# sandialabs/PyNucleus

Measured on AMD Instinct MI355X. Metric: element-pairs/sec assembled (2D P1 fractional s=0.5, dense) + % fp64 roofline, higher is better.
Workload: dtype f64; 1 GPU; 2D unit disc (uniform_disc refined 7x, 98304 cells), P1, 48769 DoFs, fractional s=0.5, horizon=inf, dense getDense incl. zeroExterior; 4831887360 element pairs/step; noRef=7, num_dofs=48769, num_cells=98304, parallelism=block rows of the upper triangle dealt over 1 GPU(s), row-owned one-sided slabs

## Files before the change

include/pnl_hip.h:

```cpp
#ifndef PNL_HIP_H
#define PNL_HIP_H
#include <stdint.h>

#ifdef __cplusplus
extern "C" {
#endif

typedef struct pnl_context pnl_context;

enum pnl_status {
    PNL_OK = 0,
    PNL_ERR_INVALID = -1,
    PNL_ERR_UNSUPPORTED = -2,
    PNL_ERR_HIP = -3,
    PNL_ERR_STATE = -4,
    PNL_ERR_ORDER = -5
};

enum pnl_kernel_type { PNL_FRACTIONAL = 0, PNL_INDICATOR = 1, PNL_PERIDYNAMIC = 2, PNL_GAUSSIAN = 3, PNL_EXPONENTIAL = 4,
                       PNL_GAUSSIAN_BOUNDARY = 5, PNL_EXPONENTIAL_BOUNDARY = 6 };

typedef struct {
    int32_t ktype;
    int32_t interaction;
// ... 85 lines not shown
    const int32_t *d_cell, *d_pair;
    int32_t n_sing[3];
    int32_t n_btouch;
    const int32_t *sing_items[3];
    const int32_t *pair_foff, *fvid;
    const int32_t *bt_slot, *bt_cell, *bt_facet;
} pnl_cluster_plan;
int pnl_assemble_clusters_tiled(pnl_context *ctx, const pnl_cluster_plan *plan, int cluster_boundary, double *data_dev,
                                double *diag_dev);
typedef struct {
    int32_t nnodes, nleaves, nfar, m, nlevels, nq;
    const double *box;
    const int32_t *parent, *level;
    const int32_t *leaf_node, *leaf_dof_off, *leaf_dofs, *leaf_cell_off, *leaf_cells;
    const int32_t *far;
    const double *transfer;
    const double *qbary, *qw, *qphi;
    const int32_t *far_class;
    int32_t partial_leaves;
} pnl_h2_plan;
int pnl_h2_setup(pnl_context *ctx, const pnl_h2_plan *plan);
int pnl_h2_matvec(pnl_context *ctx, const double *x_dev, double *y_dev);
int pnl_h2_upward(pnl_context *ctx, const double *x_dev, double *cup_dev);
int pnl_h2_interact(pnl_context *ctx, const double *cup_dev, double *cdown_dev);
int pnl_h2_downward(pnl_context *ctx, double *cdown_dev, double *y_dev);
int pnl_h2_sizes(pnl_context *ctx, int32_t *out2);
int pnl_h2_get(pnl_context *ctx, int which, double *dst_host);
int pnl_h2_set(pnl_context *ctx, int which, const double *src_host);

int pnl_spmv(pnl_context *ctx, const double *data_dev, const double *diag_dev, const double *x_dev, double *y_dev);

typedef struct pnl_order_function {
    int32_t type, normalized;
    double p[6];
    int32_t scal_n, pad;
    double scal_mid, scal_half;
    double scal_cheb[32];
} pnl_order_function;

int pnl_set_order_function(pnl_context *ctx, const pnl_order_function *f, const double *cell_smax, const double *facet_smax,
                           double c0, double bc0, double sing_fac, double bsing_fac);
int pnl_set_order_vertex_values(pnl_context *ctx, int nv, const double *values_host);
int pnl_upload_pointwise_rules(pnl_context *ctx, int which, int panel, int nkeys, int M, int rows, const double *nodes,
                               const double *w, const double *phi0, const double *phi1);
int pnl_assemble_dense_pointwise(pnl_context *ctx, double *A, int64_t ldA, int zero_exterior, int cell_begin, int cell_end,
                                 int npairs, const int32_t *pairs, int nbpairs, const int32_t *bpairs);
int pnl_assemble_pairs_masked_pointwise(pnl_context *ctx, int np, const int32_t *pairs, const uint64_t *masks, const int32_t *rule,
                                        double *data);
int pnl_assemble_boundary_masked_pointwise(pnl_context *ctx, int ni, const int32_t *cells, const int32_t *facets, const uint32_t *masks,
                                           const int32_t *rule, const double *sv, double fac, double *data, double *diag);

int pnl_get_counters(pnl_context *ctx, int64_t *out, int n);
int pnl_get_phase_ms(pnl_context *ctx, float *out, int n);
enum pnl_kernel_slot { PNL_K_TILE_GENERAL = 0, PNL_K_TILE_UNIFORM2, PNL_K_TILE_UNIFORM3, PNL_K_TILE_UNIFORM4, PNL_K_FOLD_MIRROR,
                       PNL_K_WORKLIST, PNL_NUM_KERNEL_SLOTS };
int pnl_get_kernel_ms(pnl_context *ctx, float *out, int n);

typedef struct pnl_tree pnl_tree;
typedef struct pnl_nfplan pnl_nfplan;
int pnl_tree_build(int N, int dim, const double *boxes, const int64_t *d2c_ptr, const int32_t *d2c_idx, int nc, double eta,
                   int min_size, int max_levels, int do_admissibility, pnl_tree **out);
int pnl_tree_build_blocks(int N, int dim, const double *boxes, const int64_t *d2c_ptr, const int32_t *d2c_idx, int nc, double eta,
                          int min_size, int max_levels, int do_admissibility, const int32_t *dof_block, int mixed_block,
                          pnl_tree **out);
int pnl_tree_build_refined(int N, int dim, const double *boxes, const int64_t *d2c_ptr, const int32_t *d2c_idx, int nc, double eta,
                           int min_size, int max_levels, int do_admissibility, const int32_t *dof_block, int mixed_block, int ref_type,
                           pnl_tree **out);
int pnl_tree_build_horizon(int N, int dim, const double *boxes, const int64_t *d2c_ptr, const int32_t *d2c_idx, int nc, double eta,
                           int min_size, int max_levels, int do_admissibility, const int32_t *dof_block, int mixed_block, int ref_type,
                           double horizon, pnl_tree **out);
int pnl_tree_build_device(int N, int dim, const double *boxes, const int64_t *d2c_ptr, const int32_t *d2c_idx, int nc, double eta,
                          int min_size, int max_levels, int do_admissibility, int ref_type, pnl_tree **out);
void pnl_tree_destroy(pnl_tree *T);
int pnl_tree_sizes(const pnl_tree *T, int64_t *out3);
int pnl_tree_get(const pnl_tree *T, int32_t *range, int32_t *parent, int32_t *children, int32_t *level, double *box, int32_t *perm,
                 int32_t *near, int32_t *far);
int pnl_tree_node_cells(const pnl_tree *T, int n, const int32_t *node_ids, int64_t *off, int32_t *cells);
int pnl_h2_transfer_matrices(int nnodes, int dim, int m, const double *box, const int32_t *parent, double *out);
int pnl_nfplan_build(int dim, int nv, const double *vertices, int nc, const int32_t *cells, int dpe, int N, const int32_t *dofs,
                     int nnodes, const int64_t *node_off, const int32_t *node_dofs, const int64_t *node_cell_off,
                     const int32_t *node_cells, int npairs, const int32_t *pair_nodes, int tile, int max_chunk_dofs,
                     pnl_nfplan **out);
void pnl_nfplan_destroy(pnl_nfplan *P);
int pnl_nfplan_sizes(const pnl_nfplan *P, int64_t *out9);
int pnl_nfplan_get(const pnl_nfplan *P, int which, void *dst);

typedef struct pnl_pattern pnl_pattern;
int pnl_horizon_pattern(int dim, int nv, const double *vertices, int nc, const int32_t *cells, int dpe, int N, const int32_t *dofs,
                        double delta, int strict_lower, pnl_pattern **out);
int pnl_near_pattern(const pnl_tree *T, int npairs, const int32_t *pairs, int strict_lower, pnl_pattern **out);
int64_t pnl_pattern_set_max_nnz(int64_t max_nnz);
int64_t pnl_pattern_nnz(const pnl_pattern *P);
int pnl_pattern_get(const pnl_pattern *P, int32_t *indptr, int32_t *indices);
void pnl_pattern_destroy(pnl_pattern *P);

int pnl_set_row_slab(pnl_context *ctx, int nrows, const int32_t *rowdofs_host, int ncols, const int32_t *coldofs_host);
int pnl_diag_blocks_size(pnl_context *ctx);
int pnl_get_diag_blocks(pnl_context *ctx, double *dst_dev);
int pnl_slab_matvec(pnl_context *ctx, const double *slab_dev, int64_t ld, const double *diag_blocks_dev, const double *x_dev,
                    double *y_dev);
int pnl_slab_diagonal(pnl_context *ctx, const double *slab_dev, int64_t ld, const double *diag_blocks_dev, double *diag_dev);

int pnl_gemv(pnl_context *ctx, const double *A_dev, int64_t ldA, int n, const double *x_dev, double *y_dev,
             int symmetric_half);
int pnl_cg_jacobi(pnl_context *ctx, const double *A_dev, int64_t ldA, int n, const double *b_dev, double *x_dev,
                  double tol, int maxiter, int *iters, double *residual);
// ... 77 lines not shown
```

pynucleus_amd/_lib.py:

```python
import ctypes as C
import os
import numpy as np

_HERE = os.path.dirname(os.path.abspath(__file__))
LIB_PATH = os.environ.get('PNL_LIB', os.path.join(_HERE, 'libpnl_hip.so'))

PNL_OK = 0
PNL_ERR_INVALID = -1
PNL_ERR_UNSUPPORTED = -2
PNL_ERR_HIP = -3
PNL_ERR_STATE = -4
PNL_ERR_ORDER = -5
PNL_INTERIOR = 0
PNL_BOUNDARY = 1
PNL_FLAG_NO_MIRROR = 1
PNL_FLAG_SYMMETRIC_FLUSH = 2
PNL_NUM_COUNTERS = 134

EXPORTS = ['pnl_create', 'pnl_destroy', 'pnl_error_string', 'pnl_version', 'pnl_set_stream', 'pnl_synchronize',
           'pnl_upload_mesh', 'pnl_upload_dofmap', 'pnl_set_kernel', 'pnl_set_order_formula', 'pnl_upload_distant_rules',
           'pnl_upload_singular_rule', 'pnl_upload_boundary', 'pnl_assemble_dense', 'pnl_dense_overwrites', 'pnl_block_row_costs', 'pnl_tile_cells',
           'pnl_assemble_dense_tiles', 'pnl_get_counters', 'pnl_get_phase_ms', 'pnl_get_kernel_ms', 'pnl_tree_build', 'pnl_tree_build_blocks', 'pnl_tree_build_refined', 'pnl_tree_build_horizon', 'pnl_tree_build_device', 'pnl_tree_destroy', 'pnl_tree_sizes', 'pnl_tree_get', 'pnl_tree_node_cells', 'pnl_h2_transfer_matrices', 'pnl_nfplan_build', 'pnl_nfplan_destroy', 'pnl_nfplan_sizes', 'pnl_nfplan_get', 'pnl_horizon_pattern', 'pnl_near_pattern', 'pnl_pattern_set_max_nnz', 'pnl_set_option', 'pnl_set_cell_order', 'pnl_set_interaction_transform', 'pnl_set_order_vertex_values', 'pnl_h2_get', 'pnl_h2_set', 'pnl_pattern_nnz', 'pnl_pattern_get', 'pnl_pattern_destroy', 'pnl_set_row_slab', 'pnl_diag_blocks_size', 'pnl_get_diag_blocks', 'pnl_slab_matvec', 'pnl_slab_diagonal', 'pnl_gemv', 'pnl_cg_jacobi',
           'pnl_inv_diagonal', 'pnl_set_classes', 'pnl_select_class', 'pnl_upload_sparsity', 'pnl_upload_sparsity_device', 'pnl_assemble_pairs_masked', 'pnl_assemble_boundary_masked', 'pnl_assemble_clusters_tiled', 'pnl_h2_setup', 'pnl_h2_matvec', 'pnl_h2_upward', 'pnl_h2_interact', 'pnl_h2_downward', 'pnl_h2_sizes', 'pnl_spmv',
           'pnl_assemble_pairs_in_horizon', 'pnl_assemble_pairs_in_horizon_range', 'pnl_set_nonsymmetric', 'pnl_set_order_function', 'pnl_upload_pointwise_rules', 'pnl_assemble_dense_pointwise',
           'pnl_assemble_pairs_masked_pointwise', 'pnl_assemble_boundary_masked_pointwise',
           'pnl_gemv_axpby', 'pnl_csr_matvec', 'pnl_mg_create', 'pnl_mg_destroy', 'pnl_mg_cycle', 'pnl_mg_solve', 'pnl_mg_cg', 'pnl_theta_step', 'pnl_selftest',
           'pnl_potrf', 'pnl_potrs', 'pnl_getrf', 'pnl_getrs',
           'pnl_csr_cg_jacobi', 'pnl_fe_space_create', 'pnl_fe_space_destroy', 'pnl_assemble_nonlinearity', 'pnl_imex_create',
           'pnl_imex_destroy', 'pnl_imex_sweep']

PNL_FUN_BRUSSELATOR, PNL_FUN_CUBIC = 0, 1
PNL_IMEX_CG_MG, PNL_IMEX_CHOL = 0, 1
PNL_IMEX_MAX_STAGES, PNL_IMEX_MAX_COMP = 4, 2


def source_sha16():
    import glob
    import hashlib
    root = os.path.dirname(_HERE)
    files = sorted(glob.glob(os.path.join(_HERE, 'csrc', '*.h'))+glob.glob(os.path.join(_HERE, 'csrc', '*.hip'))
                   +[os.path.join(root, 'include', 'pnl_hip.h'), os.path.join(_HERE, 'csrc', 'Makefile')])
    h = hashlib.sha256()
    for fn in files:
        with open(fn, 'rb') as f:
            h.update(os.path.basename(fn).encode()+b'\0'+f.read())
    return h.hexdigest()[:16]


class pnl_kernel(C.Structure):
    _fields_ = [('ktype', C.c_int32), ('interaction', C.c_int32), ('exponent', C.c_double), ('scale', C.c_double),
                ('horizon2', C.c_double)]


class pnl_order_formula(C.Structure):
    _fields_ = [('c0', C.c_double), ('a', C.c_double), ('b', C.c_double), ('e', C.c_double), ('den0', C.c_double),
                ('clip_num', C.c_int32), ('pad', C.c_int32)]


class pnl_mg_level_desc(C.Structure):
    _fields_ = [('n', C.c_int32), ('pad', C.c_int32), ('A_dev', C.c_void_p), ('ldA', C.c_int64), ('diag_dev', C.c_void_p),
                ('R_indptr_dev', C.c_void_p), ('R_indices_dev', C.c_void_p), ('R_data_dev', C.c_void_p),
                ('P_indptr_dev', C.c_void_p), ('P_indices_dev', C.c_void_p), ('P_data_dev', C.c_void_p),
                ('kind', C.c_int32), ('pad2', C.c_int32), ('near_indptr_dev', C.c_void_p), ('near_indices_dev', C.c_void_p),
                ('near_data_dev', C.c_void_p)]


class pnl_order_function(C.Structure):
    _fields_ = [('type', C.c_int32), ('normalized', C.c_int32), ('p', C.c_double*6), ('scal_n', C.c_int32), ('pad', C.c_int32),
                ('scal_mid', C.c_double), ('scal_half', C.c_double), ('scal_cheb', C.c_double*32)]


class pnl_cluster_plan(C.Structure):
    _fields_ = ([(n, C.c_int32) for n in ('npairs', 'nnodes', 'nchunks', 'chunk_stride', 'ntiles', 'num_dslots', 'nfacets', 'tile')] +
                [(n, C.c_void_p) for n in ('pair_nodes', 'node_off', 'node_dofs', 'chunk_cells', 'chunk_ndof', 'chunk_dofs', 'chunk_slot',
                                           'tile_chunkA', 'tile_chunkB', 'tile_pair', 'tile_flags', 'tile_dslotA', 'tile_dslotB',
# ... 11 lines not shown

class pnl_imex_desc(C.Structure):
    _fields_ = ([(n, C.c_int32) for n in ('s', 'ncomp', 'n', 'fun', 'nparams', 'solver', 'maxiter', 'mass_maxiter')] +
                [('AE', C.c_double*(PNL_IMEX_MAX_STAGES**2)), ('AI', C.c_double*(PNL_IMEX_MAX_STAGES**2)),
                 ('bE', C.c_double*PNL_IMEX_MAX_STAGES), ('bI', C.c_double*PNL_IMEX_MAX_STAGES),
                 ('mass_scale', C.c_double*PNL_IMEX_MAX_COMP), ('params', C.c_double*4),
                 ('dt', C.c_double), ('tol', C.c_double), ('mass_tol', C.c_double),
                 ('S_dev', C.c_void_p), ('ldS', C.c_int64), ('M_indptr_dev', C.c_void_p), ('M_indices_dev', C.c_void_p),
                 ('M_data_dev', C.c_void_p), ('space', C.c_void_p), ('mg', C.c_void_p*PNL_IMEX_MAX_COMP),
                 ('chol_dev', C.c_void_p*PNL_IMEX_MAX_COMP), ('ldchol', C.c_int64*PNL_IMEX_MAX_COMP)])


class PnlError(RuntimeError):
    pass


_LIB = None


def load():
    global _LIB
    if _LIB is not None:
        return _LIB
    if not os.path.exists(LIB_PATH):
        raise PnlError('{} is missing: the HIP extension has not been built (run __graft_entry__.build()); '
                       'there is no CPU fallback for the assembly path'.format(LIB_PATH))
    import torch
    L = C.CDLL(LIB_PATH)
    vp, i32, i64, dbl = C.c_void_p, C.c_int, C.c_int64, C.c_double
    L.pnl_create.argtypes = [i32, C.POINTER(vp)]
    L.pnl_destroy.argtypes = [vp]
    L.pnl_destroy.restype = None
    L.pnl_error_string.argtypes = [vp]
    L.pnl_error_string.restype = C.c_char_p
    L.pnl_version.restype = C.c_char_p
    L.pnl_set_stream.argtypes = [vp, vp]
    L.pnl_synchronize.argtypes = [vp]
    L.pnl_upload_mesh.argtypes = [vp, i32, i32, vp, i32, vp, vp, vp, dbl]
    L.pnl_upload_dofmap.argtypes = [vp, i32, i32, i32, i32, vp, vp]
    L.pnl_set_kernel.argtypes = [vp, i32, C.POINTER(pnl_kernel)]
    L.pnl_selftest.argtypes = [i32, i32, i32, i32, vp, i32, vp, vp]
    L.pnl_set_order_formula.argtypes = [vp, i32, C.POINTER(pnl_order_formula)]
    L.pnl_upload_distant_rules.argtypes = [vp, i32, vp, vp, vp, vp, vp, vp, vp]
    L.pnl_upload_singular_rule.argtypes = [vp, i32, i32, i32, i32, vp, vp, vp, dbl]
    L.pnl_upload_boundary.argtypes = [vp, i32, vp]
    L.pnl_assemble_dense.argtypes = [vp, vp, i64, i32, i32, i32, i32]
    L.pnl_dense_overwrites.argtypes = [vp, i32, i32, i32]
    L.pnl_block_row_costs.argtypes = [vp, vp, i32]
    L.pnl_tile_cells.argtypes = [vp]
    L.pnl_assemble_dense_tiles.argtypes = [vp, vp, i64, i32, i32, vp, i32, i32, i32]
    L.pnl_get_counters.argtypes = [vp, vp, i32]
    L.pnl_get_phase_ms.argtypes = [vp, vp, i32]
    L.pnl_get_kernel_ms.argtypes = [vp, vp, i32]
    L.pnl_set_row_slab.argtypes = [vp, i32, vp, i32, vp]
    L.pnl_tree_build.argtypes = [i32, i32, vp, vp, vp, i32, dbl, i32, i32, i32, C.POINTER(vp)]
    L.pnl_tree_build_blocks.argtypes = [i32, i32, vp, vp, vp, i32, dbl, i32, i32, i32, vp, i32, C.POINTER(vp)]
    L.pnl_tree_build_refined.argtypes = [i32, i32, vp, vp, vp, i32, dbl, i32, i32, i32, vp, i32, i32, C.POINTER(vp)]
    L.pnl_tree_build_horizon.argtypes = [i32, i32, vp, vp, vp, i32, dbl, i32, i32, i32, vp, i32, i32, dbl, C.POINTER(vp)]
    L.pnl_tree_build_device.argtypes = [i32, i32, vp, vp, vp, i32, dbl, i32, i32, i32, i32, C.POINTER(vp)]
    L.pnl_tree_destroy.argtypes = [vp]
    L.pnl_tree_destroy.restype = None
    L.pnl_tree_sizes.argtypes = [vp, vp]
    L.pnl_tree_get.argtypes = [vp, vp, vp, vp, vp, vp, vp, vp, vp]
    L.pnl_tree_node_cells.argtypes = [vp, i32, vp, vp, vp]
    L.pnl_h2_transfer_matrices.argtypes = [i32, i32, i32, vp, vp, vp]
    L.pnl_nfplan_build.argtypes = [i32, i32, vp, i32, vp, i32, i32, vp, i32, vp, vp, vp, vp, i32, vp, i32, i32, C.POINTER(vp)]
    L.pnl_nfplan_destroy.argtypes = [vp]
    L.pnl_nfplan_destroy.restype = None
    L.pnl_nfplan_sizes.argtypes = [vp, vp]
    L.pnl_nfplan_get.argtypes = [vp, i32, vp]
    L.pnl_horizon_pattern.argtypes = [i32, i32, vp, i32, vp, i32, i32, vp, dbl, i32, C.POINTER(vp)]
    L.pnl_near_pattern.argtypes = [vp, i32, vp, i32, C.POINTER(vp)]
    L.pnl_pattern_nnz.argtypes = [vp]
    L.pnl_pattern_set_max_nnz.argtypes = [i64]
    L.pnl_set_option.argtypes = [C.c_char_p, C.c_char_p]
    L.pnl_set_cell_order.argtypes = [vp, i32, vp]
    L.pnl_set_interaction_transform.argtypes = [vp, i32, vp]
    L.pnl_set_order_vertex_values.argtypes = [vp, i32, vp]
    L.pnl_h2_get.argtypes = [vp, i32, vp]
    L.pnl_h2_set.argtypes = [vp, i32, vp]
    L.pnl_pattern_get.argtypes = [vp, vp, vp]
    L.pnl_pattern_destroy.argtypes = [vp]
    L.pnl_diag_blocks_size.argtypes = [vp]
    L.pnl_get_diag_blocks.argtypes = [vp, vp]
    L.pnl_slab_matvec.argtypes = [vp, vp, i64, vp, vp, vp]
    L.pnl_slab_diagonal.argtypes = [vp, vp, i64, vp, vp]
    L.pnl_gemv.argtypes = [vp, vp, i64, i32, vp, vp, i32]
    L.pnl_cg_jacobi.argtypes = [vp, vp, i64, i32, vp, vp, dbl, i32, C.POINTER(C.c_int), C.POINTER(C.c_double)]
    L.pnl_inv_diagonal.argtypes = [vp, vp, i64, i32, vp]
    L.pnl_gemv_axpby.argtypes = [vp, vp, i64, i32, i32, vp, dbl, dbl, vp, vp]
    L.pnl_csr_matvec.argtypes = [vp, i32, vp, vp, vp, vp, dbl, dbl, vp]
    L.pnl_mg_create.argtypes = [vp, i32, C.POINTER(pnl_mg_level_desc), vp, dbl, i32, i32, C.POINTER(C.c_void_p)]
    L.pnl_mg_destroy.argtypes = [vp]
    L.pnl_mg_cycle.argtypes = [vp, vp, vp, i32]
    L.pnl_mg_solve.argtypes = [vp, vp, vp, dbl, i32, i32, C.POINTER(C.c_int), C.POINTER(C.c_double), i32]
    L.pnl_mg_cg.argtypes = [vp, vp, i64, vp, vp, dbl, i32, i32, C.POINTER(C.c_int), C.POINTER(C.c_double), i32]
    L.pnl_theta_step.argtypes = [vp, vp, i64, vp, vp, vp, dbl, dbl, vp, vp, dbl, i32, C.POINTER(C.c_int), C.POINTER(C.c_double)]
    L.pnl_potrf.argtypes = [vp, vp, i64, i32, C.POINTER(C.c_int)]
    L.pnl_potrs.argtypes = [vp, vp, i64, i32, vp, i64, i32]
    L.pnl_getrf.argtypes = [vp, vp, i64, i32, vp, C.POINTER(C.c_int)]
    L.pnl_getrs.argtypes = [vp, vp, i64, i32, vp, vp, i64, i32]
    L.pnl_csr_cg_jacobi.argtypes = [vp, i32, vp, vp, vp, dbl, vp, vp, dbl, i32, i32, C.POINTER(C.c_int), C.POINTER(C.c_double)]
    L.pnl_fe_space_create.argtypes = [vp, i32, i32, i32, i32, vp, vp, vp, vp, C.POINTER(vp)]
    L.pnl_fe_space_destroy.argtypes = [vp]
    L.pnl_assemble_nonlinearity.argtypes = [vp, i32, vp, i32, i32, vp, i64, i32, dbl, dbl, vp, i64]
    L.pnl_imex_create.argtypes = [vp, C.POINTER(pnl_imex_desc), C.POINTER(vp)]
# ... 307 lines not shown
        P.chunk_slot = ptr(plan.chunk_slot, np.int16)
        for s in range(3):
            P.n_sing[s] = plan.sing_items[s].shape[0]
            P.sing_items[s] = ptr(plan.sing_items[s], np.int32)
        P.n_btouch = plan.bt_cell.shape[0]
        self.check(self.L.pnl_assemble_clusters_tiled(self.h, C.byref(P), int(bool(cluster_boundary)), C.c_void_p(data_ptr),
                                                      C.c_void_p(diag_ptr) if diag_ptr else None))

    def spmv(self, data_ptr, diag_ptr, x_ptr, y_ptr):
        self.check(self.L.pnl_spmv(self.h, C.c_void_p(data_ptr), C.c_void_p(diag_ptr) if diag_ptr else None, C.c_void_p(x_ptr),
                                   C.c_void_p(y_ptr)))

    def counters(self):
        out = np.zeros(PNL_NUM_COUNTERS, dtype=np.int64)
        self.check(self.L.pnl_get_counters(self.h, out.ctypes.data, PNL_NUM_COUNTERS))
        hist = {q: int(out[8+q]) for q in range(120) if out[8+q]}
        sing = {-1-k: int(out[128+k]) for k in range(3)}
        return dict(numCellPairs=int(out[0]), numAssembledCellPairs=int(out[1]), numIntegrations=int(out[2]),
                    numBoundaryPairs=int(out[3]), numBoundaryIntegrations=int(out[4]), orders=hist, singular=sing,
                    uniformTilePairs=int(out[6]), uniformTilePairsByOrder={2+k: int(out[131+k]) for k in range(3)})

    def phase_ms(self):
        out = np.zeros(7, dtype=np.float32)
        self.check(self.L.pnl_get_phase_ms(self.h, out.ctypes.data, 7))
        return dict(tiles=float(out[0]), tiles_uniform=float(out[6]), worklist=float(out[1]), singular=float(out[2]),
                    boundary=float(out[3]), scatter_mirror=float(out[4]), total=float(out[5]))

    def set_row_slab(self, rowdofs, coldofs):
        rd = np.ascontiguousarray(rowdofs, dtype=np.int32)
        cd = np.ascontiguousarray(coldofs, dtype=np.int32)
        self.check(self.L.pnl_set_row_slab(self.h, int(rd.shape[0]), rd.ctypes.data if rd.shape[0] else None, int(cd.shape[0]),
                                           cd.ctypes.data if cd.shape[0] else None))

    def diag_blocks_size(self):
        n = self.L.pnl_diag_blocks_size(self.h)
        self.check(min(n, 0))
        return n

    def get_diag_blocks(self, dst_ptr):
        self.check(self.L.pnl_get_diag_blocks(self.h, C.c_void_p(dst_ptr)))

    def slab_matvec(self, slab_ptr, ld, dblocks_ptr, x_ptr, y_ptr):
        self.check(self.L.pnl_slab_matvec(self.h, C.c_void_p(slab_ptr), int(ld), C.c_void_p(dblocks_ptr), C.c_void_p(x_ptr), C.c_void_p(y_ptr)))

    def slab_diagonal(self, slab_ptr, ld, dblocks_ptr, diag_ptr):
        self.check(self.L.pnl_slab_diagonal(self.h, C.c_void_p(slab_ptr), int(ld), C.c_void_p(dblocks_ptr), C.c_void_p(diag_ptr)))

    def kernel_ms(self):
        out = np.zeros(6, dtype=np.float32)
        self.check(self.L.pnl_get_kernel_ms(self.h, out.ctypes.data, 6))
        return dict(tile_general=float(out[0]), tile_uniform2=float(out[1]), tile_uniform3=float(out[2]), tile_uniform4=float(out[3]),
                    fold_mirror=float(out[4]), worklist=float(out[5]))

    def gemv(self, A_ptr, ldA, n, x_ptr, y_ptr, symmetric_half=False):
        self.check(self.L.pnl_gemv(self.h, C.c_void_p(A_ptr), int(ldA), int(n), C.c_void_p(x_ptr), C.c_void_p(y_ptr),
                                   int(symmetric_half)))

    def cg_jacobi(self, A_ptr, ldA, n, b_ptr, x_ptr, tol, maxiter):
        it, res = C.c_int(0), C.c_double(0.)
        self.check(self.L.pnl_cg_jacobi(self.h, C.c_void_p(A_ptr), int(ldA), int(n), C.c_void_p(b_ptr), C.c_void_p(x_ptr),
                                        float(tol), int(maxiter), C.byref(it), C.byref(res)))
        return it.value, res.value

    def gemv_axpby(self, A_ptr, ldA, nrows, ncols, x_ptr, alpha, beta, b_ptr, y_ptr):
        self.check(self.L.pnl_gemv_axpby(self.h, C.c_void_p(A_ptr), int(ldA), int(nrows), int(ncols), C.c_void_p(x_ptr), float(alpha),
                                         float(beta), C.c_void_p(b_ptr) if b_ptr else None, C.c_void_p(y_ptr)))

    def csr_matvec(self, nrows, indptr_ptr, indices_ptr, data_ptr, x_ptr, alpha, beta, y_ptr):
        self.check(self.L.pnl_csr_matvec(self.h, int(nrows), C.c_void_p(indptr_ptr), C.c_void_p(indices_ptr), C.c_void_p(data_ptr),
                                         C.c_void_p(x_ptr), float(alpha), float(beta), C.c_void_p(y_ptr)))

    def mg_create(self, descs, coarse_inverse_ptr, omega, presmooth, postsmooth):
        arr = (pnl_mg_level_desc*len(descs))(*descs)
        out = C.c_void_p()
        self.check(self.L.pnl_mg_create(self.h, len(descs), arr, C.c_void_p(coarse_inverse_ptr), float(omega), int(presmooth), int(postsmooth),
                                        C.byref(out)))
        return out

    def mg_destroy(self, mg):
        self.L.pnl_mg_destroy(mg)

    def mg_cycle(self, mg, b_ptr, x_ptr, x_is_zero):
        self.check(self.L.pnl_mg_cycle(mg, C.c_void_p(b_ptr), C.c_void_p(x_ptr), int(bool(x_is_zero))))

    def mg_solve(self, mg, b_ptr, x_ptr, tol, maxiter, x_is_zero):
        it = C.c_int(0)
        res = (C.c_double*(maxiter+2))()
        self.check(self.L.pnl_mg_solve(mg, C.c_void_p(b_ptr), C.c_void_p(x_ptr), float(tol), int(maxiter), int(bool(x_is_zero)), C.byref(it),
                                       res, maxiter+2))
        return it.value, list(res[:it.value+1])

    def mg_cg(self, mg, A_ptr, ldA, b_ptr, x_ptr, tol, maxiter, x_is_zero):
        it = C.c_int(0)
        res = (C.c_double*(maxiter+2))(*([float('nan')]*(maxiter+2)))
        self.check(self.L.pnl_mg_cg(mg, C.c_void_p(A_ptr) if A_ptr else None, int(ldA), C.c_void_p(b_ptr), C.c_void_p(x_ptr), float(tol),
                                    int(maxiter), int(bool(x_is_zero)), C.byref(it), res, maxiter+2))
        out = list(res)
        while len(out) > 1 and out[-1] != out[-1]:
            out.pop()
        return it.value, out

    def theta_step(self, mg, S_ptr, ldS, M_indptr_ptr, M_indices_ptr, M_data_ptr, dt, theta, forcing_ptr, u_ptr, tol, maxiter):
        it, res = C.c_int(0), C.c_double(0.)
        self.check(self.L.pnl_theta_step(mg, C.c_void_p(S_ptr), int(ldS), C.c_void_p(M_indptr_ptr), C.c_void_p(M_indices_ptr),
                                         C.c_void_p(M_data_ptr), float(dt), float(theta), C.c_void_p(forcing_ptr) if forcing_ptr else None,
                                         C.c_void_p(u_ptr), float(tol), int(maxiter), C.byref(it), C.byref(res)))
# ... 69 lines not shown
```

pynucleus_amd/csrc/pnl_context.h:

```cpp
#pragma once
#include <hip/hip_runtime.h>
#include <algorithm>
#include <cmath>
#include <cstdarg>
#include <cstdio>
#include <cstring>
#include <string>
#include <vector>
#include "pnl_hip.h"
#include "pnl_device.h"

constexpr int TILE_P1 = 64;
constexpr int TILE_P2 = 32;

struct DevBuf {
    void *p = nullptr;
    size_t bytes = 0;
    ~DevBuf() { release(); }
    void release() { if (p) { (void)hipFree(p); p = nullptr; bytes = 0; } }
};

struct pnl_context {
    int device = 0;
    hipStream_t own_stream = nullptr, stream = nullptr;
    static constexpr int NAUX = 4;
    hipStream_t aux[NAUX] = {};
    hipEvent_t ev_fork = nullptr, ev_join[NAUX] = {};
    hipEvent_t ev_fold = nullptr;
    hipEvent_t ev_bnd = nullptr;
    bool fold_event_set = false;
    std::string err;
    int dim = 0, nv = 0, nc = 0, dpe = 0, dpv = 0, dped = 0, N = 0, nb = 0, qmax = -1;
    int nreal = 0;
    std::vector<int> cell_orig;
    std::vector<int> real_from;
    double H0 = 0.;
    std::vector<double> vertices, vol, h;
    std::vector<int32_t> cells, dofs, perm_table, bcells;
    struct ClassData {
        pnl_kernel kern[2];
        pnl_order_formula form[2];
        bool have_kernel[2] = {false, false}, have_form[2] = {false, false};
        bool have_sing[2][3] = {{false, false, false}, {false, false, false}};
        DevBuf b_sn[3], b_sw[3], b_sp[3], b_bn[2], b_bw[2], b_bp[2], b_spairs[3], b_bpairs[2], b_spairs1[3];
        int sM[3] = {0, 0, 0}, sRows[3] = {0, 0, 0}, bM[2] = {0, 0};
        double sFac = 0., bFac = 0.;
        int n_spairs[3] = {0, 0, 0}, n_bpairs[2] = {0, 0};
        int n_spairs1[3] = {0, 0, 0};
        ClassData() { std::memset(kern, 0, sizeof(kern)); std::memset(form, 0, sizeof(form)); }
    };
    std::vector<ClassData*> cls;
    int cur = 0;
    ClassData &C() { return *cls[cur]; }
    int nlab = 0;
    bool nonsym = false;
    int orient = 0;
    std::vector<int32_t> cell_labels, facet_labels, cls_of;
    bool have_mesh = false, have_dofs = false, have_rules = false, have_boundary = false;
    bool dirty = true;
    DevProblem P;
    DevBuf b_cellv, b_ccen, b_cvol, b_ch, b_clog, b_cvid, b_cdof, b_cslot, b_blk_ndof, b_blk_dofs, b_perm, b_off, b_bary, b_w, b_phi,
        b_foff, b_fbary, b_fw, b_bvid, b_bv, b_bgeo, b_counters, b_D, b_tiles,
        b_vec[6], b_clabel, b_blabel, b_clsof, b_scal, b_wl, b_wlcount, b_tilectr, b_ttn, b_ttoff, b_tttab, b_ttwphi, b_wlsorted, b_wlaux,
        b_vertices, b_sp_indptr, b_sp_indices, b_mp_pairs, b_mp_masks, b_mp_wl, b_mp_sorted, b_mp_aux, b_bi_cells, b_bi_facets,
        b_bi_masks, b_cp[28], b_cpD, b_wlds, b_wlpair, b_h2[20];
    DevBuf b_kcls, b_fcls, b_uni, b_tilecls, b_ttwphif;
    DevBuf b_scolbase, b_srowoff, b_cpoff, b_cpslot, b_cprow, b_foldtab, b_bkcls, b_bfcls, b_bdefer, b_multitiles, b_slotA, b_candtiles, b_candq;
    int slot_S = 0, n_multitiles = 0;
    long long slot_total = 0;
    DevBuf b_rowmap, b_rowdof, b_colmap, b_coldof;
    DevBuf b_cholinfo;
    DevBuf b_luwork, b_lutmp;
    std::vector<int32_t> slab_rowdofs, slab_coldofs;
    int slab_rows = 0, slab_cols = 0;
    bool slot_full_list = false;
    bool slot_used = false;
    std::vector<DevKernel> kcls_host;
    std::vector<DevKernel> bkcls_host;
    std::vector<DevFormula> bfcls_host;
    std::vector<DevFormula> fcls_host;
    int uni_off[5] = {-1, -1, -1, -1, -1}, uni_np[5] = {0, 0, 0, 0, 0};
    bool uni_struct[5] = {false, false, false, false, false};
    H2Dev h2;
    bool have_h2 = false;
    bool have_tile_order = false;
    struct TileOrderJob *tile_job = nullptr;
    DevBuf b_cellv_t, b_cdof_t, b_cslot_t, b_Dt;
    PwDev pw;
    bool have_pw = false, have_pw_rules[2][3] = {{false, false, false}, {false, false, false}};
    int pw_nkeys[2] = {0, 0};
    std::vector<double> pw_cell_smax, pw_facet_smax;
    std::vector<double> pw_vertex_s;
    DevBuf b_pw_cellsv;
    DevBuf b_pw_csm, b_pw_fsm, b_pw_rule[2][3][4], b_pw_pairs, b_pw_bpairs;
    std::vector<std::vector<int>> h2_levels;
    long long h2_vtot = 0;
    std::vector<size_t> h2_level_off;
    std::vector<int32_t> rule_off, frule_off;
    int sp_nnz = -1;
    unsigned wl_cap = 0;
    int tile = TILE_P1, nblocks = 0, ncp = 0, nU = 0;
    std::vector<int2> spairs_host[3];
    std::vector<int2> tiles_cached;
    size_t tiles_cap = 0;
    int n_mixed = 0, n_pure = 0, tile_off = 0, tiles_cb = -1, tiles_ce = -1;
    std::vector<int> cls_tile_off, cls_n_mixed, cls_n_pure;
    std::vector<int> cls_n_uni[3];
    bool single_launch = false;
    int sl_off[4] = {0, 0, 0, 0}, sl_n[4] = {0, 0, 0, 0};
    unsigned wl_cap_each = 0;
    int wl_slots = 1;
    std::vector<pnl_order_formula> tiles_forms;
    pnl_order_formula tiles_form;
    bool tiles_filter = true;
    bool use_pure = true;
    struct PowTab { double exponent, scale; DevBuf buf; };
    std::vector<PowTab*> powtabs;
    struct BlockAgg { double cx, cy, rad, hmax, hmin, Lmin, Lmax; bool full; double tcx, tcy, trad; };
    bool have_xform = false;
    double xform[4] = {1., 0., 0., 1.};
    std::vector<BlockAgg> blocks;
    hipEvent_t ev[8] = {nullptr, nullptr, nullptr, nullptr, nullptr, nullptr, nullptr, nullptr};
    hipEvent_t kev[PNL_NUM_KERNEL_SLOTS][2] = {};
    bool kev_set[PNL_NUM_KERNEL_SLOTS] = {};
    bool pure_launched = false;
    bool symflush = false;
    bool ev_valid = false;
    unsigned long long visited_pairs = 0;
    bool visited_is_assembled = false;
    bool tiles_launched = false;
    int ablate = 0;
    bool tile_cell_filter = true;
    bool wl_lane = true;
};

inline int fail(pnl_context *ctx, int code, const char *fmt, ...) {
    char buf[512];
    va_list ap;
    va_start(ap, fmt);
    vsnprintf(buf, sizeof(buf), fmt, ap);
    va_end(ap);
    if (ctx) ctx->err = buf;
    return code;
}

#define HIPCHK(ctx, call)                                                                            \
    do {                                                                                             \
        hipError_t e_ = (call);                                                                      \
        if (e_ != hipSuccess) return fail(ctx, PNL_ERR_HIP, "%s failed: %s", #call, hipGetErrorString(e_)); \
    } while (0)

template <class T>
int upload(pnl_context *ctx, DevBuf &b, const T *src, size_t n) {
    const size_t bytes = std::max<size_t>(n*sizeof(T), 16);
    if (b.bytes < bytes) {
        b.release();
        HIPCHK(ctx, hipMalloc(&b.p, bytes));
        b.bytes = bytes;
    }
    if (n) HIPCHK(ctx, hipMemcpyAsync(b.p, src, n*sizeof(T), hipMemcpyHostToDevice, ctx->stream));
    HIPCHK(ctx, hipStreamSynchronize(ctx->stream));
    return PNL_OK;
}

inline int ensure(pnl_context *ctx, DevBuf &b, size_t bytes) {
    bytes = std::max<size_t>(bytes, 16);
    if (b.bytes < bytes) {
        b.release();
        HIPCHK(ctx, hipMalloc(&b.p, bytes));
        b.bytes = bytes;
    }
    return PNL_OK;
}

inline DevKernel to_dev(const pnl_kernel &k, int dim) {
    DevKernel d;
    d.ktype = k.ktype;
// ... 31 lines not shown
    W.type = f.type; W.normalized = f.normalized;
    for (int i = 0; i < 6; i++) W.p[i] = f.p[i];
    if (f.scal_n < 0 || f.scal_n > 32 || (f.scal_n > 0 && !(f.scal_half > 0.))) return false;
    W.scal_n = f.scal_n; W.scal_mid = f.scal_mid; W.scal_inv_half = f.scal_n > 0 ? 1./f.scal_half : 0.;
    for (int i = 0; i < 32; i++) W.scal_cheb[i] = i < f.scal_n ? f.scal_cheb[i] : 0.;
    return true;
}

inline DevFormula to_dev(const pnl_order_formula &f) {
    DevFormula d;
    d.c0 = f.c0; d.a = f.a; d.b = f.b; d.e = f.e; d.den0 = f.den0; d.clip = f.clip_num; d.pad = 0;
    return d;
}

const char *pnl_tune(const char *name);
inline int pnl_grid_cap(int grid) {
    const char *e = pnl_tune("PNL_TILE_WGS");
    const int cap = e ? atoi(e) : 0;
    return cap > 0 ? std::max(1, std::min(grid, cap)) : grid;
}

inline int acc_stride_of(int nU, size_t fixed_bytes = 0) {
    int st = nU+1;
    const int m = pnl_tune("PNL_ACC_PAD") ? atoi(pnl_tune("PNL_ACC_PAD")) : 32;
    if (m > 1) {
        int padded = st;
        while (padded % m != 1) padded++;
        if (fixed_bytes+sizeof(double)*(size_t)(nU+1)*padded <= 80*1024) st = padded;
        else if (st % 2 == 0 && fixed_bytes+sizeof(double)*(size_t)(nU+1)*(st+1) <= 80*1024) st++;
    }
    return st;
}

inline DevProblem tile_problem(const pnl_context *ctx) {
    DevProblem Pt = ctx->P;
    if (ctx->have_tile_order) {
        Pt.cellv = (const double*)ctx->b_cellv_t.p; Pt.cdof = (const int*)ctx->b_cdof_t.p; Pt.cslot = (const short*)ctx->b_cslot_t.p;
    }
    return Pt;
}

inline DevProblem with_mixed_rules(const pnl_context *ctx, DevProblem Pt) {
    Pt.uni = (const double*)ctx->b_uni.p;
    Pt.mix_struct = 0;
    const bool generic = pnl_tune("PNL_MIXED_GENERIC") != nullptr;
    for (int q = 0; q < 5; q++) {
        Pt.uni_off[q] = ctx->uni_off[q] >= 0 ? ctx->uni_off[q] : 0;
        if (q >= 2 && q <= ctx->qmax && ctx->dim == 2 && ctx->dpe == 3 && ctx->uni_off[q] >= 0 && ctx->uni_struct[q] && !generic)
            Pt.mix_struct |= 1 << q;
    }
    return Pt;
}

inline void kt_begin(pnl_context *ctx, int slot) { (void)hipEventRecord(ctx->kev[slot][0], ctx->stream); }
inline void kt_end(pnl_context *ctx, int slot) { (void)hipEventRecord(ctx->kev[slot][1], ctx->stream); ctx->kev_set[slot] = true; }

int pnl_tile_order_ready(pnl_context *ctx);

int pnl_assembly_prepare(pnl_context *ctx);
int pnl_assembly_ready(pnl_context *ctx);
void pnl_refresh_tables(pnl_context *ctx);
int pnl_make_tiles(pnl_context *ctx, std::vector<int2> &tiles, int cell_begin, int cell_end);
int pnl_upload_tiles(pnl_context *ctx, std::vector<int2> &tiles, int cell_begin, int cell_end);
int pnl_tile_order_range(pnl_context *ctx, const DevFormula &qo, int ncand, signed char *host_out);
struct WlBins { unsigned *hist, *offs, *coff, *cursor; };
int pnl_wl_sort(pnl_context *ctx, const int4 *wl, const unsigned *count, unsigned cap, unsigned *aux_base, int4 *sorted, WlBins &B);
void pnl_scatter_diag(pnl_context *ctx, const DevProblem &P, const double *D, double *A, int64_t ldA);
int pnl_tile_uniform_order(const pnl_context *ctx, const pnl_order_formula &F, int ta, int tb, int qlimit);
int pnl_sparse_ready(pnl_context *ctx, double *data, double *diag, SparseOut &S);

int pnl_pw_prepare(pnl_context *ctx, int need_boundary);
int pnl_pw_h2_interp(pnl_context *ctx);

int pnl_launch_gemv_symmetric(pnl_context *ctx, const double *A, long long ldA, int n, const double *x, double alpha, double beta,
                              const double *b, double *y);
int pnl_launch_slab_two_sided(pnl_context *ctx, const double *slab, long long ld, int nrows, int ncols, const int *rowdof, const int *coldof,
                              const double *x, double *y);

int pnl2_launch_uniform(pnl_context *ctx, int kt, const DevProblem &Pt, const int2 *tiles, const int *tile_cls, int ntiles, int q,
                        double *A, int64_t ldA, double *Dglob, const SlotOut &SO);
int pnl2_launch_p2(pnl_context *ctx, int kt, const int2 *tiles, const int *tile_cls, int ntiles, double *A, int64_t ldA,
                   int cell_begin, int cell_end, unsigned wl_cap_each, const SlotOut &SO);
int pnl2_zero_slot_tiles(pnl_context *ctx, const SlotOut &SO);
int pnl2_fold_mirror(pnl_context *ctx, const SlotOut &SO, double *A, int64_t ldA);
inline SlotOut slot_out(const pnl_context *ctx) {
    SlotOut SO;
    SO.A2 = (double*)ctx->b_slotA.p; SO.rowoff = (const long long*)ctx->b_srowoff.p; SO.colbase = (const int*)ctx->b_scolbase.p;
    SO.S = ctx->slot_S; SO.nU = ctx->nU;
    return SO;
}
```

pynucleus_amd/csrc/pnl_hip.hip:

```cpp
#include <hip/hip_runtime.h>
#include <algorithm>
#include <cmath>
#include <cstdio>
#include <cstring>
#include <string>
#include <vector>
#include "pnl_hip.h"
#include "pnl_kernels.h"
#include "pnl_bndtile.h"
#include "pnl_context.h"
#include "pnl_launch.h"

namespace {

__global__ void __launch_bounds__(PNL_NTHREADS)
k_mirror(double *__restrict__ A, long long ldA, int N) {
    __shared__ double t1[32][33], t2[32][33];
    const int nb = (N+31)/32;
    int bid = blockIdx.x;
    int bi = 0;
    {
        double fb = ((2.*nb+1.)-sqrt((2.*nb+1.)*(2.*nb+1.)-8.*bid))*0.5;
        bi = (int)fb;
        while (bi > 0 && (long long)bi*nb-(long long)bi*(bi-1)/2 > bid) bi--;
// ... 75 lines not shown
        }
    }
    void use(int k) {
        if (!on) return;
        const int j = k < (int)slot.size() ? slot[k] : k % pnl_context::NAUX;
        if (!used[j]) { (void)hipStreamWaitEvent(ctx->aux[j], start, 0); used[j] = true; }
        ctx->stream = ctx->aux[j];
    }
    void join() {
        if (!on) return;
        ctx->stream = main;
        for (int j = 0; j < pnl_context::NAUX; j++)
            if (used[j]) {
                (void)hipEventRecord(ctx->ev_join[j], ctx->aux[j]);
                (void)hipStreamWaitEvent(main, ctx->ev_join[j], 0);
                used[j] = false;
            }
        on = false;
    }
    ~ClassFork() { join(); }
};

template <int DIM, int DPE, int KT>
int run_worklist(pnl_context *ctx, const int4 *wl, const unsigned *wlc, unsigned cap, double *A, int64_t ldA, bool sym, int region = 0,
                 int nregions = 1) {
    int rc;
    if ((rc = ensure(ctx, ctx->b_wlsorted, (size_t)cap*nregions*sizeof(int4)))) return rc;
    if ((rc = ensure(ctx, ctx->b_wlaux, sizeof(unsigned)*(4*(PNL_WL_BINS+1))*nregions))) return rc;
    const int4 *wlsorted = (const int4*)ctx->b_wlsorted.p+(size_t)region*cap;
    WlBins B;
    if ((rc = pnl_wl_sort(ctx, wl, wlc, cap, (unsigned*)ctx->b_wlaux.p+(size_t)region*4*(PNL_WL_BINS+1), (int4*)wlsorted, B))) return rc;
    int dbg = 0;
#ifdef PNL_DEBUG_ABLATE
    dbg = pnl_tune("PNL_WL_DBG") ? atoi(pnl_tune("PNL_WL_DBG")) : 0;
#endif
    const int nmin = ctx->wl_lane ? PNL_WL_LANE_MAXPTS+1 : 0;
    return worklist_eval<DIM, DPE, KT, false>(ctx, "PNL_WL_LDS_KB", 18, wlsorted, B, A, ldA, (double*)ctx->b_D.p, SparseOut{}, ClusterTiles{},
                                              PNL_WL_BINS-1, nmin | (sym ? 1 << 16 : 0), ctx->wl_lane, dbg | (sym ? 8 : 0));
}

int ensure_worklist(pnl_context *ctx, double pairs, int regions) {
    const double frac = pnl_tune("PNL_WL_FRAC") ? atof(pnl_tune("PNL_WL_FRAC")) : 0.05;
    const double floor_entries = pnl_tune("PNL_WL_FRAC") ? 64. : (double)(1 << 20);
    const size_t each = (size_t)std::min<double>(std::max<double>(pairs*frac, floor_entries), 400e6);
    int rc;
    if ((rc = ensure(ctx, ctx->b_wl, each*(size_t)regions*sizeof(int4)))) return rc;
    ctx->wl_cap = (unsigned)std::min<size_t>(ctx->b_wl.bytes/sizeof(int4), 0xffffffffu);
    ctx->wl_cap_each = (unsigned)each;
    if ((rc = ensure(ctx, ctx->b_tilectr, sizeof(unsigned)))) return rc;
    return PNL_OK;
}

template <int DIM, int DPE, int TILE, int KT>
int launch_tiles(pnl_context *ctx, int wl_slot, double *A, int64_t ldA, int cell_begin, int cell_end, const SlotOut &SO = SlotOut{}) {
    using S = TileSmem<DIM, DPE, TILE, KT == 0>;
    HIPCHK(ctx, hipEventRecord(ctx->ev[7], ctx->stream));
    ctx->pure_launched = false;
    if (TILE == 64 && DPE <= 3) {
        int rc;
        if (DIM == 2 && DPE == 3 && !pnl_tune("PNL_PURE_V1") && ctx->uni_off[2] >= 0 && ctx->uni_np[2] == 3)
            rc = pnl2_launch_uniform(ctx, KT, tile_problem(ctx), (const int2*)ctx->b_tiles.p+ctx->tile_off+ctx->n_mixed, nullptr, ctx->n_pure, 2,
                                     A, ldA, (double*)(ctx->have_tile_order ? ctx->b_Dt.p : ctx->b_D.p), SO);
        else rc = launch_pure<DIM, (DPE <= 3 ? DPE : 3), KT>(ctx, A, ldA, SO);
        if (rc) return rc;
        ctx->pure_launched = ctx->n_pure > 0;
        if (DIM == 2 && DPE == 3) {
            int off = ctx->tile_off+ctx->n_mixed+ctx->n_pure;
            for (int q = 3; q <= 4; q++) {
                const int n = ctx->cls_n_uni[q-2][ctx->cur];
                if ((rc = pnl2_launch_uniform(ctx, KT, tile_problem(ctx), (const int2*)ctx->b_tiles.p+off, nullptr, n, q, A, ldA,
                                              (double*)(ctx->have_tile_order ? ctx->b_Dt.p : ctx->b_D.p), SO))) return rc;
                ctx->pure_launched = ctx->pure_launched || n > 0;
                off += n;
            }
        }
        HIPCHK(ctx, hipEventRecord(ctx->ev[7], ctx->stream));
    }
    const int ntiles = ctx->n_mixed;
    const int acc_stride = acc_stride_of(ctx->nU, S::fixed_bytes);
    const size_t lds = S::fixed_bytes+sizeof(double)*(size_t)(ctx->nU+1)*acc_stride;
    if (lds > 160*1024)
        return fail(ctx, PNL_ERR_UNSUPPORTED, "a block of %d cells touches %d DoFs: LDS sub-block of %zu bytes exceeds 160 KiB "
                    "(cells must be numbered with spatial locality)", TILE, ctx->nU, lds);
    unsigned *wlc = (unsigned*)ctx->b_wlcount.p+wl_slot;
    HIPCHK(ctx, hipMemsetAsync(ctx->b_tilectr.p, 0, sizeof(unsigned), ctx->stream));
    auto kfun = k_tile_distant<DIM, DPE, TILE, KT, false>;
    const int grid_mult = pnl_tune("PNL_GRID_MULT") ? atoi(pnl_tune("PNL_GRID_MULT")) : 1;
    const PersistentGrid g = persistent_grid(ctx, kfun, tile_threads(DPE, KT), lds, ntiles, 2, grid_mult);
    if (g.rc) return g.rc;
    if (pnl_tune("PNL_VERBOSE")) fprintf(stderr, "[pnl] tiles=%d nU=%d lds=%zu bytes, occupancy API: %d blocks/CU\n", ntiles, ctx->nU, lds, g.per_cu);
    SlotOut SOk = SO;
    SOk.nU = ctx->nU;
    kt_begin(ctx, PNL_K_TILE_GENERAL);
    if (g.grid > 0)
        hipLaunchKernelGGL(kfun, dim3(g.grid), dim3(tile_threads(DPE, KT)), lds, ctx->stream, with_mixed_rules(ctx, tile_problem(ctx)), (const int2*)ctx->b_tiles.p+ctx->tile_off, A,
                           (long long)ldA, (double*)(ctx->have_tile_order ? ctx->b_Dt.p : ctx->b_D.p), cell_begin, cell_end, acc_stride, (int4*)ctx->b_wl.p,
                           wlc, ctx->wl_cap_each, ctx->ablate | (ctx->symflush ? 256 : 0), ntiles, ClusterTiles{},
                           (unsigned*)ctx->b_tilectr.p, SOk);
    kt_end(ctx, PNL_K_TILE_GENERAL);
    HIPCHK(ctx, hipGetLastError());
    HIPCHK(ctx, hipEventRecord(ctx->ev[6], ctx->stream));
    if (SO.A2) {
        int rc = pnl2_fold_mirror(ctx, SO, A, ldA);
        if (rc) return rc;
        HIPCHK(ctx, hipEventRecord(ctx->ev_fold, ctx->stream));
        ctx->fold_event_set = true;
    }
    return run_worklist<DIM, DPE, KT>(ctx, (const int4*)ctx->b_wl.p, wlc, ctx->wl_cap_each, A, ldA, ctx->symflush || SO.A2 != nullptr);
}

template <int DIM, int DPE, int KT>
int launch_singular(pnl_context *ctx, double *A, int64_t ldA, int cell_begin, int cell_end) {
    for (int s = 0; s < DIM+1; s++) {
        const int np = ctx->orient ? ctx->C().n_spairs1[s] : ctx->C().n_spairs[s];
        if (!np) continue;
        if (!ctx->C().have_sing[0][s]) return fail(ctx, PNL_ERR_STATE, "singular rule for %d common vertices not uploaded", s+1);
        const int wpb = PNL_SING_THREADS/64;
        int rc = with_slot<DIM>(s, [&](auto slot) {
            constexpr int SLOT = decltype(slot)::value;
            const int2 *pairs = (const int2*)(ctx->orient ? ctx->C().b_spairs1[SLOT].p : ctx->C().b_spairs[SLOT].p);
            return launch_singular_pairs<DIM, DPE, SLOT, KT, false>(ctx, (np+wpb-1)/wpb, pairs, np, A, ldA, cell_begin, cell_end, SparseOut{},
                                                                    nullptr, nullptr, ClusterTiles{});
        });
        if (rc) return rc;
    }
    return PNL_OK;
}

template <int DIM, int DPE, int KT>
int launch_boundary(pnl_context *ctx, int cell_begin, int cell_end, int what = 3, const DevKernel *bkcls = nullptr,
                    const DevFormula *bfcls = nullptr, bool all_fast = false) {
    if (ctx->nb == 0 || cell_end <= cell_begin) return PNL_OK;
    const int ncell = cell_end-cell_begin;
    const int gx = (ncell+PNL_NTHREADS-1)/PNL_NTHREADS;
    int per = pnl_tune("PNL_BND_PER") ? atoi(pnl_tune("PNL_BND_PER")) : 32;
    while (per > 1 && (long long)gx*((ctx->nb+per-1)/per) < 4096) per >>= 1;
    const int chunks = (ctx->nb+per-1)/per;
    if (what & 1) {
        const int defer = pnl_tune("PNL_BND_DEFER") ? atoi(pnl_tune("PNL_BND_DEFER")) : 48;
        const bool use_list = defer > 0;
        const unsigned cap = (unsigned)std::min<long long>(std::max<long long>(65536, 64ll*ctx->nb), 1ll << 24);
        int *dcells = nullptr, *dfacets = nullptr, *dcls = nullptr;
        unsigned *dslots = nullptr, *dcount = nullptr;
        if (use_list) {
            int rc;
            if ((rc = ensure(ctx, ctx->b_bdefer, sizeof(int)*(size_t)cap*(3+DIM)+sizeof(unsigned)))) return rc;
            dcells = (int*)ctx->b_bdefer.p; dfacets = dcells+cap; dslots = (unsigned*)(dfacets+(size_t)cap*DIM); dcls = (int*)(dslots+cap);
            dcount = (unsigned*)(dcls+cap);
            HIPCHK(ctx, hipMemsetAsync(dcount, 0, sizeof(unsigned), ctx->stream));
        }
        const bool fast = bkcls ? all_fast : (ctx->P.bkn.fast != 0);
        bool tiled = false;
        if constexpr (DIM == 2) {
// ... 95 lines not shown
        if (var && (rc = pnl2_zero_slot_tiles(ctx, SO))) return rc;
    }
    HIPCHK(ctx, hipEventRecord(ctx->ev[7], ctx->stream));
    ctx->pure_launched = false;
    for (int q = 2; q <= 4; q++) {
        const int n = ctx->sl_n[q-1];
        if ((rc = pnl2_launch_uniform(ctx, kt, ctx->P, tiles+ctx->sl_off[q-1], tcls ? tcls+ctx->sl_off[q-1] : nullptr, n, q, A, ldA,
                                      (double*)ctx->b_D.p, SO))) return rc;
        ctx->pure_launched = ctx->pure_launched || n > 0;
    }
    if (ctx->pure_launched) HIPCHK(ctx, hipEventRecord(ctx->ev[7], ctx->stream));
    if ((rc = pnl2_launch_p2(ctx, kt, tiles+ctx->sl_off[0], tcls ? tcls+ctx->sl_off[0] : nullptr, ctx->sl_n[0], A, ldA, cell_begin, cell_end,
                             ctx->wl_cap_each, SO))) return rc;
    HIPCHK(ctx, hipEventRecord(ctx->ev[6], ctx->stream));
    if (ctx->slot_used) {
        if ((rc = pnl2_fold_mirror(ctx, SO, A, ldA))) return rc;
        HIPCHK(ctx, hipEventRecord(ctx->ev_fold, ctx->stream));
        ctx->fold_event_set = true;
    }
    const bool sym = ctx->symflush || ctx->slot_used;
    {
        ClassFork fork(ctx, ncls);
        if (ncls > pnl_context::NAUX && (int)ctx->cls_n_mixed.size() == ncls) fork.plan(ctx->cls_n_mixed);
        for (int k = 0; k < ncls; k++) {
            ctx->cur = k;
            pnl_refresh_tables(ctx);
            fork.use(k);
            const int4 *wl = (const int4*)ctx->b_wl.p+(size_t)k*ctx->wl_cap_each;
            const unsigned *wlc = (const unsigned*)ctx->b_wlcount.p+k;
            rc = with_kt(ctx->P.k.fast, [&](auto kt) {
                return run_worklist<DIM, DPE, decltype(kt)::value>(ctx, wl, wlc, ctx->wl_cap_each, A, ldA, sym, k, ncls);
            });
            if (rc) { ctx->cur = 0; return rc; }
        }
    }
    ctx->cur = 0;
    return PNL_OK;
}

bool slot_eligible(const pnl_context *ctx, int cell_begin, int cell_end, int flags) {
    const bool elem = ctx->dpe == 6 || (ctx->dpe == 3 && ctx->cls.size() == 1 && !ctx->nonsym && ctx->use_pure && !pnl_tune("PNL_NO_SLOT_P1"));
    return ctx->dim == 2 && elem && ctx->slot_full_list && ctx->slab_rows == 0 && cell_begin == 0 && cell_end == ctx->nc &&
           !(flags & (PNL_FLAG_NO_MIRROR | PNL_FLAG_SYMMETRIC_FLUSH));
}

#ifndef PNL_BND_MODE_DEFAULT
#define PNL_BND_MODE_DEFAULT 3
#endif
template <int DIM, int DPE, int TILE>
int assemble_impl(pnl_context *ctx, double *A, int64_t ldA, int zero_exterior, int ntiles, int cell_begin, int cell_end, int flags) {
    int rc;
    const int ncls = (int)ctx->cls.size();
    ctx->symflush = (flags & PNL_FLAG_SYMMETRIC_FLUSH) != 0;
    for (bool &b : ctx->kev_set) b = false;
    HIPCHK(ctx, hipMemsetAsync(ctx->b_counters.p, 0, sizeof(unsigned long long)*PNL_NCOUNTERS, ctx->stream));
    HIPCHK(ctx, hipMemsetAsync(ctx->b_D.p, 0, sizeof(double)*(size_t)ctx->ncp*(DPE*(DPE+1)/2), ctx->stream));
    if (ctx->have_tile_order) HIPCHK(ctx, hipMemsetAsync(ctx->b_Dt.p, 0, sizeof(double)*(size_t)ctx->ncp*(DPE*(DPE+1)/2), ctx->stream));
    HIPCHK(ctx, hipEventRecord(ctx->ev[0], ctx->stream));
    ctx->tiles_launched = ntiles > 0;
    ctx->fold_event_set = false;
    const bool bnd_one_pass = zero_exterior && ncls > 1 && ctx->nlab > 0 && !pnl_tune("PNL_BND_PER_CLASS");
    bool bnd_all_fast = true;
    if (bnd_one_pass) {
        std::vector<DevKernel> &bk = ctx->bkcls_host;
        std::vector<DevFormula> &bf = ctx->bfcls_host;
        bk.resize(ncls); bf.resize(ncls);
        for (int k = 0; k < ncls; k++) {
            ctx->cur = k;
            pnl_refresh_tables(ctx);
            bk[k] = ctx->P.bkn; bf[k] = ctx->P.bqo;
            bnd_all_fast = bnd_all_fast && ctx->P.bkn.fast;
        }
        ctx->cur = 0;
        if ((rc = ensure(ctx, ctx->b_bkcls, sizeof(DevKernel)*ncls))) return rc;
        if ((rc = ensure(ctx, ctx->b_bfcls, sizeof(DevFormula)*ncls))) return rc;
        HIPCHK(ctx, hipMemcpyAsync(ctx->b_bkcls.p, bk.data(), sizeof(DevKernel)*ncls, hipMemcpyHostToDevice, ctx->stream));
        HIPCHK(ctx, hipMemcpyAsync(ctx->b_bfcls.p, bf.data(), sizeof(DevFormula)*ncls, hipMemcpyHostToDevice, ctx->stream));
    }
    auto boundary_term = [&](hipEvent_t chain) -> int {
        int rcb;
        ClassFork fork(ctx, chain ? ncls : 1, chain);
        if (chain && ncls > pnl_context::NAUX && (int)ctx->cls_n_mixed.size() == ncls) fork.plan(ctx->cls_n_mixed);
        for (int k = 0; k < ncls; k++) {
            ctx->cur = k;
            pnl_refresh_tables(ctx);
            if (!ctx->have_boundary || !ctx->C().have_kernel[1] || !ctx->C().have_form[1]) {
                ctx->cur = 0;
                return fail(ctx, PNL_ERR_STATE, "zero_exterior needs boundary facets, boundary kernel and order formula");
            }
            if (chain) fork.use(k);
            if (bnd_one_pass && k == 0 &&
                (rcb = launch_boundary<DIM, DPE, 0>(ctx, cell_begin, cell_end, 1, (const DevKernel*)ctx->b_bkcls.p, (const DevFormula*)ctx->b_bfcls.p,
                                                    bnd_all_fast))) { ctx->cur = 0; return rcb; }
            if (chain) fork.use(k);
            if ((rcb = launch_boundary<DIM, DPE, 0>(ctx, cell_begin, cell_end, bnd_one_pass ? 2 : 3))) { ctx->cur = 0; return rcb; }
        }
        ctx->cur = 0;
        return PNL_OK;
    };
    const int bnd_mode = !zero_exterior ? -1 : pnl_tune("PNL_BND_MODE") ? atoi(pnl_tune("PNL_BND_MODE")) : PNL_BND_MODE_DEFAULT;
    bool bnd_side = false;
    auto boundary_side = [&](hipEvent_t after) -> int {
        hipStream_t const caller = ctx->stream;
        hipStream_t const side = ctx->aux[1];
        HIPCHK(ctx, hipStreamWaitEvent(side, after, 0));
        ctx->stream = side;
        const int rcb = boundary_term(nullptr);
        ctx->stream = caller;
        if (rcb) return rcb;
        HIPCHK(ctx, hipEventRecord(ctx->ev_join[1], side));
        bnd_side = true;
        return PNL_OK;
    };
// ... 16 lines not shown
                { ctx->cur = 0; ctx->orient = 0; return rc; }
        } else {
        SlotOut SO{};
        ctx->slot_used = false;
        if (slot_eligible(ctx, cell_begin, cell_end, flags) && slot_storage_ready(ctx)) { SO = slot_out(ctx); ctx->slot_used = true; }
        for (int ko = 0; ko < ncls*norient; ko++) {
            const int k = ko/norient;
            ctx->cur = k; ctx->orient = ko%norient;
            pnl_refresh_tables(ctx);
            ctx->tile_off = ctx->cls_tile_off[k]; ctx->n_mixed = ctx->cls_n_mixed[k]; ctx->n_pure = ctx->cls_n_pure[k];
            if (ctx->n_mixed+ctx->n_pure+ctx->cls_n_uni[1][k]+ctx->cls_n_uni[2][k] == 0) continue;
            const int tb0 = ctx->tile_cell_filter ? cell_begin : 0, tb1 = ctx->tile_cell_filter ? cell_end : ctx->nc;
            if (ctx->P.k.fast && ctx->P.k.qm == 6 && DPE == 3 && !pnl_tune("PNL_NO_KT2")) rc = launch_tiles<DIM, DPE, TILE, (DPE == 3 ? 2 : 1)>(ctx, ko, A, ldA, tb0, tb1, SO);
            else rc = with_kt(ctx->P.k.fast, [&](auto kt) { return launch_tiles<DIM, DPE, TILE, decltype(kt)::value>(ctx, ko, A, ldA, tb0, tb1, SO); });
            if (rc) { ctx->cur = 0; ctx->orient = 0; return rc; }
        }
        }
    }
    ctx->orient = 0;
    HIPCHK(ctx, hipEventRecord(ctx->ev[1], ctx->stream));
    if (ntiles > 0 && ctx->slot_used) {
    } else if (!(flags & (PNL_FLAG_NO_MIRROR | PNL_FLAG_SYMMETRIC_FLUSH))) {
        const long long nb = (ctx->N+31)/32;
        hipLaunchKernelGGL(k_mirror, dim3((unsigned)(nb*(nb+1)/2)), dim3(PNL_NTHREADS), 0, ctx->stream, A, (long long)ldA, ctx->N);
        HIPCHK(ctx, hipGetLastError());
    }
    HIPCHK(ctx, hipEventRecord(ctx->ev[2], ctx->stream));
    hipStream_t const main_stream = ctx->stream;
    bool fold_like = ctx->fold_event_set;
    if (!fold_like && ncls*norient == 1 && zero_exterior && !pnl_tune("PNL_NO_OVERLAP")) {
        HIPCHK(ctx, hipEventRecord(ctx->ev_fold, ctx->stream));
        fold_like = true;
    }
    const bool overlap = fold_like && ncls*norient == 1 && !pnl_tune("PNL_NO_OVERLAP");
    struct StreamGuard { pnl_context *c; hipStream_t s; ~StreamGuard() { c->stream = s; } } stream_guard{ctx, main_stream};
    if (overlap) { HIPCHK(ctx, hipStreamWaitEvent(ctx->aux[0], ctx->ev_fold, 0)); ctx->stream = ctx->aux[0]; }
    hipEvent_t const chain = (ctx->fold_event_set && !overlap && !pnl_tune("PNL_NO_OVERLAP")) ? ctx->ev_fold : nullptr;
    {
        ClassFork fork(ctx, ncls*norient, chain);
        if (norient == 1 && ncls > pnl_context::NAUX && (int)ctx->cls_n_mixed.size() == ncls) fork.plan(ctx->cls_n_mixed);
        for (int ko = 0; ko < ncls*norient; ko++) {
            ctx->cur = ko/norient; ctx->orient = ko%norient;
            pnl_refresh_tables(ctx);
            fork.use(ko);
            rc = with_kt(ctx->P.k.fast, [&](auto kt) { return launch_singular<DIM, DPE, decltype(kt)::value>(ctx, A, ldA, cell_begin, cell_end); });
            if (rc) { ctx->cur = 0; ctx->orient = 0; return rc; }
        }
    }
    ctx->orient = 0;
    if (overlap) {
        HIPCHK(ctx, hipEventRecord(ctx->ev_join[0], ctx->aux[0]));
        ctx->stream = main_stream;
    } else HIPCHK(ctx, hipEventRecord(ctx->ev[3], ctx->stream));
    if (bnd_mode == 3 && ctx->fold_event_set) rc = boundary_side(ctx->ev[6]);
    else if (bnd_mode == 1 || ((bnd_mode == 0 || bnd_mode == 3) && overlap)) rc = boundary_side(bnd_mode == 1 ? ctx->ev_bnd : ctx->ev_fold);
    else if (bnd_mode == 0 || bnd_mode == 3) rc = boundary_term(chain);
    if (rc) return rc;
    ctx->cur = 0;
    if (overlap) {
        HIPCHK(ctx, hipStreamWaitEvent(main_stream, ctx->ev_join[0], 0));
        ctx->stream = main_stream;
        HIPCHK(ctx, hipEventRecord(ctx->ev[3], ctx->stream));
    }
    if (bnd_side) HIPCHK(ctx, hipStreamWaitEvent(main_stream, ctx->ev_join[1], 0));
    HIPCHK(ctx, hipEventRecord(ctx->ev[4], ctx->stream));
    if (ctx->slab_rows == 0) {
        scatter_diag<DPE>(ctx, ctx->P, (const double*)ctx->b_D.p, A, ldA);
        if (ctx->have_tile_order) scatter_diag<DPE>(ctx, tile_problem(ctx), (const double*)ctx->b_Dt.p, A, ldA);
        HIPCHK(ctx, hipGetLastError());
    }
    HIPCHK(ctx, hipEventRecord(ctx->ev[5], ctx->stream));
    ctx->ev_valid = true;
    return PNL_OK;
}

template <int DIM, int DPE>
int boundary_masked_impl(pnl_context *ctx, int ni, double fac, const SparseOut &S) {
    const int grid = std::min((ni+3)/4, 256*8);
    const int *cells = (const int*)ctx->b_bi_cells.p, *facets = (const int*)ctx->b_bi_facets.p;
    const unsigned *masks = (const unsigned*)ctx->b_bi_masks.p;
    with_kt(ctx->P.bkn.fast, [&](auto kt) {
        hipLaunchKernelGGL((k_boundary_items<DIM, DPE, decltype(kt)::value>), dim3(grid), dim3(PNL_NTHREADS), 0, ctx->stream, ctx->P,
                           (const double*)ctx->b_vertices.p, cells, facets, masks, ni, fac, S, (double*)nullptr, (const unsigned*)nullptr,
                           (const int*)nullptr, (const DevKernel*)nullptr, (const DevFormula*)nullptr);
        return PNL_OK;
    });
    HIPCHK(ctx, hipGetLastError());
    return PNL_OK;
}

template <int DIM, int DPE, int TILE, int KT>
int clusters_tiled_impl(pnl_context *ctx, const pnl_cluster_plan *pl, ClusterTiles CT, int cluster_boundary, const int *d_cell,
                        const int *d_pair, const int2 *sing_dev[3], const int *sing_pair_dev[3], const int *pair_foff, const int *fvid,
                        const double *fgeo, int maxf, const int *bt_cell, const int *bt_facet, const unsigned *bt_slot) {
    using S = TileSmem<DIM, DPE, TILE, KT == 0>;
    constexpr int ND = DPE*(DPE+1)/2;
    int rc;
    const int acc_stride = pl->chunk_stride+1;
    const size_t lds = S::fixed_bytes+sizeof(double)*(size_t)(pl->chunk_stride+1)*acc_stride;
    if (lds > 160*1024) return fail(ctx, PNL_ERR_UNSUPPORTED, "cluster chunk with %d DoFs: LDS sub-block of %zu bytes exceeds 160 KiB", pl->chunk_stride, lds);
    HIPCHK(ctx, hipMemsetAsync(ctx->b_counters.p, 0, sizeof(unsigned long long)*PNL_NCOUNTERS, ctx->stream));
    HIPCHK(ctx, hipMemsetAsync(CT.D, 0, sizeof(double)*(size_t)std::max(pl->num_dslots, 1)*ND, ctx->stream));
    HIPCHK(ctx, hipEventRecord(ctx->ev[0], ctx->stream));
    HIPCHK(ctx, hipEventRecord(ctx->ev[7], ctx->stream));
    ctx->pure_launched = false;
    {
        const double pairs = (double)pl->ntiles*TILE*TILE;
        const size_t want = (size_t)std::min<double>(std::max<double>(pairs*0.25, 1<<20), 400e6);
        if (ctx->wl_cap < want) {
// ... 444 lines not shown
```

pynucleus_amd/csrc/pnl_setup.hip:

```cpp
#include <hip/hip_runtime.h>
#include <algorithm>
#include <cmath>
#include <cstdio>
#include <cstring>
#include <deque>
#include <map>
#include <mutex>
#include <string>
#include <thread>
#include <vector>
#include "pnl_hip.h"
#include "pnl_context.h"

template <class F>
static void host_threads(F body) {
    const int nthr = (int)std::max(1u, std::min(8u, std::thread::hardware_concurrency()));
    std::vector<std::thread> pool;
    for (int th = 0; th < nthr; th++) pool.emplace_back([&body, th, nthr]() { body(th, nthr); });
    for (auto &t : pool) t.join();
}

struct TileOrderJob {
    std::vector<int> cells, lperm;
    int nc = 0, T = 0, nblocks = 0, ncp = 0, dim = 0, dpe = 0;
// ... 367 lines not shown
        block_aggregates(ctx, F, clog);
    }
    if ((rc = upload(ctx, ctx->b_cvid, F.cvid.data(), F.cvid.size()))) return rc;
    if ((rc = upload(ctx, ctx->b_cdof, F.cdof.data(), F.cdof.size()))) return rc;
    if ((rc = upload(ctx, ctx->b_cslot, F.cslot.data(), F.cslot.size()))) return rc;
    if ((rc = upload(ctx, ctx->b_blk_ndof, F.blk_ndof.data(), F.blk_ndof.size()))) return rc;
    if ((rc = upload(ctx, ctx->b_blk_dofs, F.blk_dofs.data(), F.blk_dofs.size()))) return rc;
    return PNL_OK;
}

static int upload_slot_tables(pnl_context *ctx, const CellTables &F) {
    int rc;
    const int nblocks = F.nblocks;
    const std::vector<std::vector<int>> &lists = F.lists;
    const std::vector<int32_t> &blk_ndof = F.blk_ndof;
    std::vector<int32_t> colbase(nblocks+1, 0);
    for (int b = 0; b < nblocks; b++) colbase[b+1] = colbase[b]+((blk_ndof[b]+7) & ~7);
    const int S = colbase[nblocks];
    std::vector<long long> rowoff(nblocks, 0);
    long long run = 0;
    for (int a = 0; a < nblocks; a++) { rowoff[a] = run; run += (long long)blk_ndof[a]*(S-colbase[a]); }
    ctx->slot_S = S; ctx->slot_total = run;
    std::vector<int32_t> cpoff(ctx->N+1, 0);
    for (int b = 0; b < nblocks; b++) for (int g : lists[b]) cpoff[g+1]++;
    for (int g = 0; g < ctx->N; g++) cpoff[g+1] += cpoff[g];
    std::vector<int2> cp(cpoff[ctx->N]);
    std::vector<int32_t> fillp(cpoff.begin(), cpoff.end()-1);
    std::vector<long long> cprow(cp.size());
    for (int b = 0; b < nblocks; b++)
        for (size_t r = 0; r < lists[b].size(); r++) {
            const int k = fillp[lists[b][r]]++;
            cp[k] = make_int2(b, colbase[b]+(int)r);
            cprow[k] = rowoff[b]+(long long)r*(S-colbase[b])-colbase[b];
        }
    if ((rc = upload(ctx, ctx->b_cprow, cprow.data(), cprow.size()))) return rc;
    if ((rc = upload(ctx, ctx->b_scolbase, colbase.data(), colbase.size()))) return rc;
    if ((rc = upload(ctx, ctx->b_srowoff, rowoff.data(), rowoff.size()))) return rc;
    if ((rc = upload(ctx, ctx->b_cpoff, cpoff.data(), cpoff.size()))) return rc;
    if ((rc = upload(ctx, ctx->b_cpslot, cp.data(), cp.size()))) return rc;
    const int nranges = (ctx->N+31)/32;
    std::vector<FoldEntry> tab((size_t)nranges*(PNL_FOLD_TAB+1));
    for (int q = 0; q < nranges; q++) {
        FoldEntry *e = &tab[(size_t)q*(PNL_FOLD_TAB+1)];
        const int g0 = cpoff[q*32], g1 = cpoff[std::min(ctx->N, q*32+32)];
        e[0].off = g1-g0; e[0].ar = 0; e[0].cy = 0;
        if (g1-g0 > PNL_FOLD_TAB) continue;
        for (int I = q*32; I < std::min(ctx->N, q*32+32); I++)
            for (int g = cpoff[I]; g < cpoff[I+1]; g++) {
                FoldEntry &x = e[1+g-g0];
                x.off = cprow[g]; x.ar = (cp[g].x << 5) | (I-q*32); x.cy = cp[g].y;
            }
    }
    if ((rc = upload(ctx, ctx->b_foldtab, tab.data(), tab.size()))) return rc;
    return PNL_OK;
}

static void fill_problem(pnl_context *ctx, const CellTables &F) {
    const int dim = F.dim, dpe = F.dpe, nc = F.nc, ncp = F.ncp, nblocks = F.nblocks, nU = ctx->nU, nlab = ctx->nlab;
    DevProblem &P = ctx->P;
    P.dim = dim; P.dpe = dpe; P.nc = nc; P.ncp = ncp; P.N = ctx->N; P.dpv = ctx->dpv; P.dped = ctx->dped; P.nb = ctx->nb;
    P.H0 = ctx->H0;
    P.cellv = (const double*)ctx->b_cellv.p; P.ccen = (const double*)ctx->b_ccen.p;
    P.cvol = (const double*)ctx->b_cvol.p; P.ch = (const double*)ctx->b_ch.p; P.clog = (const double*)ctx->b_clog.p;
    P.cvid = (const int*)ctx->b_cvid.p; P.cdof = (const int*)ctx->b_cdof.p; P.cslot = (const short*)ctx->b_cslot.p;
    P.blk_ndof = (const int*)ctx->b_blk_ndof.p; P.blk_dofs = (const int*)ctx->b_blk_dofs.p;
    P.blk_stride = nU; P.nblocks = nblocks;
    P.perm_table = (const int*)ctx->b_perm.p;
    P.bvid = (const int*)ctx->b_bvid.p; P.bv = (const double*)ctx->b_bv.p; P.bgeo = (const double*)ctx->b_bgeo.p;
    P.counters = (unsigned long long*)ctx->b_counters.p;
    P.nlab = nlab; P.cur_class = -1; P.orient = 0; P.pad2 = 0; P.idfac = 1.;
    P.clabel = (const int*)ctx->b_clabel.p; P.blabel = (const int*)ctx->b_blabel.p; P.cls_of = (const int*)ctx->b_clsof.p;
}

static int finalize(pnl_context *ctx) {
    if (!ctx->dirty) return PNL_OK;
    if (!ctx->have_mesh || !ctx->have_dofs) return fail(ctx, PNL_ERR_STATE, "mesh and DoF map must be uploaded first");
    const int dim = ctx->dim, nV = dim+1, nc = ctx->nc, dpe = ctx->dpe;
    if (!((dim == 2 && (dpe == 1 || dpe == 3 || dpe == 6)) || (dim == 1 && dpe >= 1 && dpe <= 4)))
        return fail(ctx, PNL_ERR_UNSUPPORTED, "unsupported (dim=%d, dofs_per_element=%d)", dim, dpe);
    const int T = ctx->tile = (dpe == 6 || (dim == 1 && dpe >= 3)) ? TILE_P2 : TILE_P1;
    const int nblocks = ctx->nblocks = (nc+T-1)/T;
    const int ncp = ctx->ncp = nblocks*T;
    CellTables F;
    F.dim = dim; F.nV = nV; F.nc = nc; F.dpe = dpe; F.T = T; F.nblocks = nblocks; F.ncp = ncp;
    const bool reorder = dpe == nV && dim == 2 && !pnl_tune("PNL_NO_REORDER");
    tile_order_drop(ctx);
    if (reorder) start_tile_order_search(ctx, F);
    int rc;
    if ((rc = padded_cell_tables(ctx, F))) return rc;
    block_dofs(ctx, F);
    ctx->have_tile_order = false;
    if (reorder) { ctx->tile_job->cellv = F.cellv; ctx->tile_job->cdof = F.cdof; ctx->tile_job->cslot = F.cslot; }
    if ((rc = touching_cell_pairs(ctx, F))) return rc;
    if (ctx->nlab > 0 && (int)ctx->cell_labels.size() != nc) return fail(ctx, PNL_ERR_STATE, "cell labels do not match the mesh");
    if ((rc = upload_touching_pairs(ctx))) return rc;
    if ((rc = boundary_facets(ctx, F))) return rc;
    if ((rc = upload_cell_tables(ctx, F))) return rc;
    if ((rc = upload_slot_tables(ctx, F))) return rc;
    if ((rc = upload(ctx, ctx->b_perm, ctx->perm_table.data(), ctx->perm_table.size()))) return rc;
    const bool fresh_counters = !ctx->b_counters.p;
    if ((rc = ensure(ctx, ctx->b_counters, sizeof(unsigned long long)*PNL_NCOUNTERS))) return rc;
    if (fresh_counters) HIPCHK(ctx, hipMemset(ctx->b_counters.p, 0, sizeof(unsigned long long)*PNL_NCOUNTERS));
    if ((rc = ensure(ctx, ctx->b_D, sizeof(double)*(size_t)ncp*(dpe*(dpe+1)/2)))) return rc;
    fill_problem(ctx, F);
    ctx->dirty = false;
    return PNL_OK;
// ... 59 lines not shown
        if (!c->have_kernel[0] || !c->have_form[0] || !ctx->have_rules)
            return fail(ctx, PNL_ERR_STATE, "kernel, order formula and distant rules must be set (for every class) before assembling");
    return PNL_OK;
}

int pnl_assembly_ready(pnl_context *ctx) {
    int rc;
    if ((rc = check_ready(ctx))) return rc;
    return finalize(ctx);
}
int pnl_assembly_prepare(pnl_context *ctx) {
    int rc;
    if ((rc = pnl_assembly_ready(ctx))) return rc;
    pnl_refresh_tables(ctx);
    return PNL_OK;
}

int pnl_tile_uniform_order(const pnl_context *ctx, const pnl_order_formula &F, int ta, int tb, int qlimit) {
    if (ta == tb) return 0;
    const auto &A = ctx->blocks[ta], &B = ctx->blocks[tb];
    if (!A.full || !B.full || !(F.e >= 0.) || !(F.den0 > 0.)) return 0;
    const double dx = A.cx-B.cx, dy = A.cy-B.cy, dc = std::sqrt(dx*dx+dy*dy);
    const double dmin = dc-A.rad-B.rad, dmax = dc+A.rad+B.rad;
    if (!(dmin > A.hmax+B.hmax)) return 0;
    typedef pnl_context::BlockAgg Agg;
    auto upper = [&](const Agg &S, const Agg &O, double q) {
        const double l_self = std::log(dmin/S.hmax), n_other = std::log(dmin/O.hmax);
        const double aL = std::max(F.a*O.Lmin, F.a*O.Lmax);
        const double bL = std::max(F.b*std::max(S.Lmin, O.Lmin), F.b*std::max(S.Lmax, O.Lmax));
        const double num = F.c0+aL+bL-F.e*n_other, den = l_self+F.den0;
        return num <= q*den*(1.-1e-9)-1e-9;
    };
    auto lower = [&](const Agg &S, const Agg &O, double q) {
        const double l_self = std::log(dmax/S.hmin), n_other = std::log(dmax/O.hmin);
        const double aL = std::min(F.a*O.Lmin, F.a*O.Lmax);
        const double bL = std::min(F.b*std::max(S.Lmin, O.Lmin), F.b*std::max(S.Lmax, O.Lmax));
        const double num = F.c0+aL+bL-F.e*n_other, den = l_self+F.den0;
        return den > 0. && num >= q*den*(1.+1e-9)+1e-9;
    };
    for (int q = 2; q <= qlimit; q++)
        if (upper(A, B, q) && upper(B, A, q)) {
            if (q == 2) return 2;
            return (lower(A, B, q-1) || lower(B, A, q-1)) ? q : 0;
        }
    return 0;
}

namespace {
std::mutex g_opt_mutex;
std::map<std::string, const std::string*> g_options;
std::deque<std::string> g_option_values;
const char *const k_product_options[] = {"PNL_WL_FRAC", "PNL_FH_NOTILES", "PNL_NO_POWTAB", "PNL_VERBOSE", "PNL_PLAN_TIMING", "PNL_PLAN_THREADS", "PNL_BND_OLD",
                                         "PNL_NO_OVERLAP", "PNL_NO_FORK",
                                         "PNL_TILE_WGS", "PNL_UNI_GENERIC", "PNL_MIXED_GENERIC"};
}

const char *pnl_tune(const char *name) {
    {
        std::lock_guard<std::mutex> lk(g_opt_mutex);
        auto it = g_options.find(name);
        if (it != g_options.end()) return it->second->c_str();
    }
#ifdef PNL_TUNING
    return getenv(name);
#else
    return nullptr;
#endif
}

extern "C" {

const char *pnl_version(void) {
#ifdef PNL_TUNING
    return "pnl_hip 0.1 (gfx950, tuning build)";
#else
    return "pnl_hip 0.1 (gfx950)";
#endif
}

int pnl_set_option(const char *name, const char *value) {
    if (!name) return PNL_ERR_INVALID;
#ifndef PNL_TUNING
    bool known = false;
    for (const char *k : k_product_options) known = known || std::strcmp(k, name) == 0;
    if (!known) return PNL_ERR_UNSUPPORTED;
#endif
    std::lock_guard<std::mutex> lk(g_opt_mutex);
    if (value) {
        const std::string *v = nullptr;
        for (const std::string &have : g_option_values) if (have == value) { v = &have; break; }
        if (!v) { g_option_values.emplace_back(value); v = &g_option_values.back(); }
        g_options[name] = v;
    } else g_options.erase(name);
    return PNL_OK;
}

int pnl_create(int device_id, pnl_context **out) {
    if (!out) return PNL_ERR_INVALID;
    *out = nullptr;
    int ndev = 0;
    hipError_t e0;
    auto hiperr = [](const char *what, hipError_t e) { fprintf(stderr, "[pnl] pnl_create: %s failed: %s\n", what, hipGetErrorString(e)); return PNL_ERR_HIP; };
    if ((e0 = hipGetDeviceCount(&ndev)) != hipSuccess || ndev <= 0) return hiperr("hipGetDeviceCount", e0);
    if (device_id < 0 || device_id >= ndev) return PNL_ERR_INVALID;
    if ((e0 = hipSetDevice(device_id)) != hipSuccess) return hiperr("hipSetDevice", e0);
    pnl_context *ctx = new pnl_context();
    ctx->device = device_id;
    if ((e0 = hipStreamCreate(&ctx->own_stream)) != hipSuccess) { delete ctx; return hiperr("hipStreamCreate", e0); }
    ctx->stream = ctx->own_stream;
    for (auto &st : ctx->aux)
        if ((e0 = hipStreamCreateWithFlags(&st, hipStreamNonBlocking)) != hipSuccess) { delete ctx; return hiperr("hipStreamCreateWithFlags", e0); }
    if (hipEventCreateWithFlags(&ctx->ev_fork, hipEventDisableTiming) != hipSuccess) { delete ctx; return PNL_ERR_HIP; }
    if (hipEventCreateWithFlags(&ctx->ev_fold, hipEventDisableTiming) != hipSuccess) { delete ctx; return PNL_ERR_HIP; }
    if (hipEventCreateWithFlags(&ctx->ev_bnd, hipEventDisableTiming) != hipSuccess) { delete ctx; return PNL_ERR_HIP; }
    for (auto &e : ctx->ev_join)
        if (hipEventCreateWithFlags(&e, hipEventDisableTiming) != hipSuccess) { delete ctx; return PNL_ERR_HIP; }
    for (auto &e : ctx->ev)
        if (hipEventCreate(&e) != hipSuccess) { delete ctx; return PNL_ERR_HIP; }
    for (auto &pr : ctx->kev)
        for (auto &e : pr)
            if (hipEventCreate(&e) != hipSuccess) { delete ctx; return PNL_ERR_HIP; }
    std::memset(&ctx->P, 0, sizeof(ctx->P));
#ifdef PNL_DEBUG_ABLATE
    if (const char *e = pnl_tune("PNL_ABLATE")) ctx->ablate = atoi(e);
#endif
    if (const char *e = pnl_tune("PNL_WL_LANE")) ctx->wl_lane = atoi(e) != 0;
    if (const char *e = pnl_tune("PNL_PURE")) ctx->use_pure = atoi(e) != 0;
    ctx->cls.push_back(new pnl_context::ClassData());
    *out = ctx;
    return PNL_OK;
}

void pnl_destroy(pnl_context *ctx) {
    if (!ctx) return;
    (void)hipSetDevice(ctx->device);
    (void)hipStreamSynchronize(ctx->stream);
    for (auto &e : ctx->ev)
        if (e) (void)hipEventDestroy(e);
    for (auto &pr : ctx->kev)
        for (auto &e : pr)
            if (e) (void)hipEventDestroy(e);
    tile_order_drop(ctx);
    for (auto &st : ctx->aux) if (st) { (void)hipStreamSynchronize(st); (void)hipStreamDestroy(st); }
    if (ctx->ev_fork) (void)hipEventDestroy(ctx->ev_fork);
    if (ctx->ev_fold) (void)hipEventDestroy(ctx->ev_fold);
    if (ctx->ev_bnd) (void)hipEventDestroy(ctx->ev_bnd);
    for (auto *t : ctx->powtabs) delete t;
    ctx->powtabs.clear();
    for (auto &e : ctx->ev_join) if (e) (void)hipEventDestroy(e);
    if (ctx->own_stream) (void)hipStreamDestroy(ctx->own_stream);
    for (auto *c : ctx->cls) delete c;
    delete ctx;
}

const char *pnl_error_string(pnl_context *ctx) { return ctx ? ctx->err.c_str() : "null context"; }

int pnl_set_stream(pnl_context *ctx, void *hip_stream) {
    if (!ctx) return PNL_ERR_INVALID;
    ctx->stream = hip_stream ? (hipStream_t)hip_stream : ctx->own_stream;
    return PNL_OK;
}

static int check_overflow(pnl_context *ctx) {
    if (ctx->b_wlcount.p && ctx->wl_cap_each > 0) {
        unsigned wl[PNL_WL_SLOTS];
        const int n = std::max(1, std::min(ctx->wl_slots, PNL_WL_SLOTS));
        HIPCHK(ctx, hipMemcpy(wl, ctx->b_wlcount.p, sizeof(unsigned)*n, hipMemcpyDeviceToHost));
        for (int i = 0; i < n; i++)
            if (wl[i] > ctx->wl_cap_each)
                return fail(ctx, PNL_ERR_STATE, "work list overflow (pass %d): %u entries needed, capacity %u; the assembled operator is "
                            "incomplete", i, wl[i], ctx->wl_cap_each);
    }
    if (ctx->b_counters.p) {
        unsigned long long ov = 0;
        HIPCHK(ctx, hipMemcpy(&ov, (const unsigned long long*)ctx->b_counters.p+5, sizeof(ov), hipMemcpyDeviceToHost));
        if (ov) return fail(ctx, PNL_ERR_ORDER, "%llu pairs need a quadrature order beyond the uploaded tables (qmax=%d); the assembled "
                            "operator is incomplete", ov, ctx->qmax);
        HIPCHK(ctx, hipMemcpy(&ov, (const unsigned long long*)ctx->b_counters.p+7, sizeof(ov), hipMemcpyDeviceToHost));
        if (ov) return fail(ctx, PNL_ERR_STATE, "%llu entries of touching pairs have no row in the slab (pnl_set_row_slab needs the DoFs of the "
                            "cells touching the rank's cells)", ov);
    }
    return PNL_OK;
}

int pnl_synchronize(pnl_context *ctx) {
    if (!ctx) return PNL_ERR_INVALID;
    HIPCHK(ctx, hipStreamSynchronize(ctx->stream));
    return check_overflow(ctx);
}

int pnl_upload_mesh(pnl_context *ctx, int dim, int nv, const double *vertices, int nc, const int32_t *cells,
                    const double *vol, const double *h, double H0) {
    if (!ctx) return PNL_ERR_INVALID;
    if (dim != 1 && dim != 2) return fail(ctx, PNL_ERR_UNSUPPORTED, "dim=%d is not implemented", dim);
// ... 241 lines not shown
    if (!ctx->have_dofs) return fail(ctx, PNL_ERR_STATE, "upload the DoF map first");
    const int slot = -panel-1;
    const int nslots = which == PNL_INTERIOR ? ctx->dim+1 : ctx->dim;
    if (which < 0 || which > 1 || slot < 0 || slot >= nslots || M <= 0 || rows <= 0 || !nodes || !w || !psi)
        return fail(ctx, PNL_ERR_INVALID, "bad singular-rule arguments");
    const int dim = ctx->dim, dpe = ctx->dpe, dpv = ctx->dpv, dped = ctx->dped, nV = dim+1;
    int rc;
    if (which == PNL_INTERIOR) {
        const int common = slot+1;
        const int expect = common == nV ? dpe : (common == 1 ? 2*dpe-dpv : 2*dpe-2*dpv-dped);
        if (rows != expect) return fail(ctx, PNL_ERR_INVALID, "singular rule has %d rows, expected %d", rows, expect);
        if ((rc = upload(ctx, ctx->C().b_sn[slot], nodes, (size_t)2*nV*M))) return rc;
        if ((rc = upload(ctx, ctx->C().b_sw[slot], w, (size_t)M))) return rc;
        if ((rc = upload(ctx, ctx->C().b_sp[slot], psi, (size_t)rows*M))) return rc;
        ctx->C().sM[slot] = M; ctx->C().sRows[slot] = rows; ctx->C().sFac = facv;
    } else {
        if (rows != dpe) return fail(ctx, PNL_ERR_INVALID, "boundary singular rule has %d rows, expected %d", rows, dpe);
        if ((rc = upload(ctx, ctx->C().b_bn[slot], nodes, (size_t)(nV+dim)*M))) return rc;
        if ((rc = upload(ctx, ctx->C().b_bw[slot], w, (size_t)M))) return rc;
        if ((rc = upload(ctx, ctx->C().b_bp[slot], psi, (size_t)rows*M))) return rc;
        ctx->C().bM[slot] = M; ctx->C().bFac = facv;
    }
    ctx->C().have_sing[which][slot] = true;
    return PNL_OK;
}

int pnl_upload_boundary(pnl_context *ctx, int nb, const int32_t *bcells) {
    if (!ctx) return PNL_ERR_INVALID;
    if (!ctx->have_mesh) return fail(ctx, PNL_ERR_STATE, "upload the mesh first");
    if (nb < 0 || (nb > 0 && !bcells)) return fail(ctx, PNL_ERR_INVALID, "bad boundary arguments");
    ctx->nb = nb;
    ctx->bcells.assign(bcells, bcells+(size_t)nb*ctx->dim);
    ctx->have_boundary = true;
    ctx->dirty = true;
    return PNL_OK;
}

int pnl_tile_cells(pnl_context *ctx) {
    if (!ctx) return PNL_ERR_INVALID;
    int rc = finalize(ctx);
    return rc ? rc : ctx->tile;
}

}

struct TilePlan {
    int T, ncls, L, qlimit, cell_begin, cell_end;
    bool filter, p1, p2, allow, q2ok;
    std::vector<pnl_order_formula> forms;
    std::vector<std::vector<int>> blk_labels;
    std::vector<std::vector<int2>> mixed, uni[3];
};

static bool tiles_resident(const pnl_context *ctx, const std::vector<int2> &tiles, const TilePlan &R) {
    const std::vector<pnl_order_formula> &forms = R.forms;
    return tiles.size() == ctx->tiles_cached.size() && ctx->b_tiles.p && ctx->tiles_cb == R.cell_begin && ctx->tiles_ce == R.cell_end &&
        forms.size() == ctx->tiles_forms.size() && std::memcmp(forms.data(), ctx->tiles_forms.data(), sizeof(pnl_order_formula)*R.ncls) == 0 &&
        ctx->tiles_filter == ctx->tile_cell_filter &&
        (tiles.empty() || std::memcmp(tiles.data(), ctx->tiles_cached.data(), tiles.size()*sizeof(int2)) == 0);
}

static int tile_orders(pnl_context *ctx, const TilePlan &R, const std::vector<int2> &tiles, int k, std::vector<signed char> &qof) {
    const int T = R.T, L = R.L, qlimit = R.qlimit, cell_begin = R.cell_begin, cell_end = R.cell_end;
    const bool filter = R.filter, allow = R.allow, q2ok = R.q2ok;
    const std::vector<std::vector<int>> &blk_labels = R.blk_labels;
    host_threads([&](int th, int nthr) {
        const size_t i0 = tiles.size()*th/nthr, i1 = tiles.size()*(th+1)/nthr;
        for (size_t i = i0; i < i1; i++) {
            const int2 &t = tiles[i];
            bool single = true;
            if (L > 0) {
                bool has = false;
                for (int la : blk_labels[t.x]) for (int lb : blk_labels[t.y])
                    has = has || ctx->cls_of[(size_t)la*L+lb] == k || ctx->cls_of[(size_t)lb*L+la] == k;
                if (!has) { qof[i] = -1; continue; }
                single = blk_labels[t.x].size() == 1 && blk_labels[t.y].size() == 1;
            }
            int q = (allow && single) ? pnl_tile_uniform_order(ctx, R.forms[k], t.x, t.y, qlimit) : 0;
            if (q == 2 && !q2ok) q = 0;
            if (q && filter && !(t.x*T >= cell_begin && (t.x+1)*T <= cell_end)) q = 0;
            qof[i] = (signed char)q;
        }
    });
    if (!(allow && ctx->dim == 2 && (T == 64 || T == 32) && !pnl_tune("PNL_NO_EXACT_TILES"))) return PNL_OK;
    std::vector<int2> cand;
    std::vector<size_t> cand_idx;
    for (size_t i = 0; i < tiles.size(); i++) {
        const int2 &t = tiles[i];
        if (qof[i] != 0 || t.x == t.y || !ctx->blocks[t.x].full || !ctx->blocks[t.y].full) continue;
        if (L > 0 && !(blk_labels[t.x].size() == 1 && blk_labels[t.y].size() == 1)) continue;
        if (filter && !(t.x*T >= cell_begin && (t.x+1)*T <= cell_end)) continue;
        cand.push_back(t); cand_idx.push_back(i);
    }
    if (cand.empty()) return PNL_OK;
    int rc;
    if ((rc = upload(ctx, ctx->b_candtiles, cand.data(), cand.size()))) return rc;
    if ((rc = ensure(ctx, ctx->b_candq, cand.size()))) return rc;
    std::vector<signed char> cq(cand.size());
    if ((rc = pnl_tile_order_range(ctx, to_dev(R.forms[k]), (int)cand.size(), cq.data()))) return rc;
    size_t moved = 0;
    for (size_t c = 0; c < cand.size(); c++) {
        const int q = cq[c];
        if (q < 2 || q > qlimit || (q == 2 && !q2ok)) continue;
        qof[cand_idx[c]] = (signed char)q; moved++;
    }
    if (pnl_tune("PNL_VERBOSE")) fprintf(stderr, "[pnl] exact order range: %zu of %zu open tiles are uniform\n", moved, cand.size());
    return PNL_OK;
}

static void tile_lists_per_class(pnl_context *ctx, const TilePlan &R, std::vector<int2> &all) {
    const std::vector<std::vector<int2>> &mixed = R.mixed, *uni = R.uni;
    for (int k = 0; k < R.ncls; k++) {
        ctx->cls_tile_off[k] = (int)all.size(); ctx->cls_n_mixed[k] = (int)mixed[k].size();
        all.insert(all.end(), mixed[k].begin(), mixed[k].end());
        for (int u = 0; u < 3; u++) { ctx->cls_n_uni[u][k] = (int)uni[u][k].size(); all.insert(all.end(), uni[u][k].begin(), uni[u][k].end()); }
        ctx->cls_n_pure[k] = ctx->cls_n_uni[0][k];
    }
}

static int tile_lists_single_launch(pnl_context *ctx, const TilePlan &R, const std::vector<int2> &tiles, std::vector<int2> &all) {
    const int ncls = R.ncls;
    const std::vector<std::vector<int2>> &mixed = R.mixed, *uni = R.uni;
    std::vector<int32_t> allcls;
    const int norient = ctx->nonsym ? 2 : 1;
    ctx->sl_off[0] = 0;
    const bool one_visit = norient == 1 && ncls > 1 && ncls <= 28 && !pnl_tune("PNL_P2_VISIT_PER_CLASS");
    std::vector<unsigned> tile_mask;
    if (one_visit) {
        tile_mask.assign((size_t)ctx->nblocks*ctx->nblocks, 0u);
        for (int k = 0; k < ncls; k++)
            for (const int2 &t : mixed[k]) tile_mask[(size_t)t.x*ctx->nblocks+t.y] |= 1u << k;
        for (const int2 &t : tiles) {
            const unsigned m = tile_mask[(size_t)t.x*ctx->nblocks+t.y];
            if (m & (m-1u)) { all.push_back(t); allcls.push_back((int)((1u << 29) | m)); }
        }
    }
    for (int k = 0; k < ncls; k++) {
        ctx->cls_n_mixed[k] = (int)mixed[k].size();
        for (int o = 0; o < norient; o++)
            for (const int2 &t : mixed[k]) {
                if (one_visit) { const unsigned m = tile_mask[(size_t)t.x*ctx->nblocks+t.y]; if (m & (m-1u)) continue; }
                all.push_back(t); allcls.push_back(2*k+o);
            }
    }
    ctx->sl_n[0] = (int)all.size();
    for (int u = 0; u < 3; u++) {
        ctx->sl_off[u+1] = (int)all.size();
        for (int k = 0; k < ncls; k++) {
            ctx->cls_n_uni[u][k] = (int)uni[u][k].size();
            for (const int2 &t : uni[u][k]) { all.push_back(t); allcls.push_back(2*k); }
        }
        ctx->sl_n[u+1] = (int)all.size()-ctx->sl_off[u+1];
    }
    for (int k = 0; k < ncls; k++) ctx->cls_n_pure[k] = ctx->cls_n_uni[0][k];
    std::vector<long long> keys(all.size());
    for (size_t i = 0; i < all.size(); i++) keys[i] = (long long)all[i].x*ctx->nblocks+all[i].y;
    std::vector<long long> sorted(keys);
    std::sort(sorted.begin(), sorted.end());
    std::vector<int2> multi;
// ... 4 lines not shown
    for (size_t i = 0; i < multi.size(); i++) mk[i] = (long long)multi[i].x*ctx->nblocks+multi[i].y;
    for (size_t i = 0; i < all.size(); i++)
        if (std::binary_search(mk.begin(), mk.end(), keys[i])) allcls[i] |= (1 << 30);
    ctx->n_multitiles = (int)multi.size();
    int rc;
    if ((rc = upload(ctx, ctx->b_multitiles, multi.data(), multi.size()))) return rc;
    return upload(ctx, ctx->b_tilecls, allcls.data(), allcls.size());
}

int pnl_upload_tiles(pnl_context *ctx, std::vector<int2> &tiles, int cell_begin, int cell_end) {
    TilePlan R;
    const int ncls = R.ncls = (int)ctx->cls.size();
    R.cell_begin = cell_begin; R.cell_end = cell_end;
    R.forms = std::vector<pnl_order_formula>(ncls);
    for (int k = 0; k < ncls; k++) R.forms[k] = ctx->cls[k]->form[0];
    if (tiles_resident(ctx, tiles, R)) return PNL_OK;
    const int T = R.T = ctx->tile;
    R.filter = ctx->tile_cell_filter;
    R.p1 = T == 64 && (ctx->dpe == 3 || ctx->dpe == 2); R.p2 = ctx->dim == 2 && ctx->dpe == 6;
    R.allow = ctx->use_pure && (R.p1 || R.p2) && ctx->qmax >= 2 && !ctx->nonsym;
    int qlimit = 2;
    if (ctx->dim == 2) for (int q = 3; q <= 4 && ctx->uni_off[q] >= 0 && ctx->uni_np[q] == 6 && q <= ctx->qmax; q++) qlimit = q;
    R.q2ok = R.p1 ? true : (ctx->uni_off[2] >= 0 && ctx->uni_np[2] == 3);
    if (pnl_tune("PNL_UNI_QMAX")) qlimit = std::min(qlimit, std::max(2, atoi(pnl_tune("PNL_UNI_QMAX"))));
    R.qlimit = qlimit;
    const int L = R.L = ctx->nlab;
    std::vector<std::vector<int>> &blk_labels = R.blk_labels;
    if (L > 0) {
        blk_labels.resize(ctx->nblocks);
        for (int b = 0; b < ctx->nblocks; b++) {
            auto &v = blk_labels[b];
            for (int c = b*T; c < std::min((b+1)*T, ctx->nc); c++) v.push_back(ctx->cell_labels[c]);
            std::sort(v.begin(), v.end());
            v.erase(std::unique(v.begin(), v.end()), v.end());
        }
    }
    ctx->cls_tile_off.assign(ncls, 0); ctx->cls_n_mixed.assign(ncls, 0); ctx->cls_n_pure.assign(ncls, 0);
    for (int u = 0; u < 3; u++) ctx->cls_n_uni[u].assign(ncls, 0);
    std::vector<std::vector<int2>> &mixed = R.mixed, *uni = R.uni;
    mixed.resize(ncls);
    for (int u = 0; u < 3; u++) uni[u].resize(ncls);
    std::vector<signed char> qof(tiles.size());
    int rc;
    for (int k = 0; k < ncls; k++) {
        if ((rc = tile_orders(ctx, R, tiles, k, qof))) return rc;
        for (size_t i = 0; i < tiles.size(); i++) {
            const int q = qof[i];
            if (q < 0) continue;
            (q ? uni[q-2][k] : mixed[k]).push_back(tiles[i]);
        }
    }
    std::vector<int2> all;
    ctx->single_launch = R.p2;
    if (!R.p2) tile_lists_per_class(ctx, R, all);
    else if ((rc = tile_lists_single_launch(ctx, R, tiles, all))) return rc;
    if (pnl_tune("PNL_VERBOSE")) {
        size_t nm = 0, nu[3] = {0, 0, 0};
        for (int k = 0; k < ncls; k++) { nm += mixed[k].size(); for (int u = 0; u < 3; u++) nu[u] += uni[u][k].size(); }
        fprintf(stderr, "[pnl] tiles: %zu mixed, uniform order 2/3/4: %zu / %zu / %zu (qlimit %d)\n", nm, nu[0], nu[1], nu[2], qlimit);
    }
    if ((rc = upload(ctx, ctx->b_tiles, all.data(), all.size()))) return rc;
    ctx->tile_off = 0; ctx->n_mixed = ctx->cls_n_mixed[0]; ctx->n_pure = ctx->cls_n_pure[0];
    ctx->tiles_cached = tiles; ctx->tiles_cb = cell_begin; ctx->tiles_ce = cell_end; ctx->tiles_forms = R.forms;
    ctx->tiles_filter = ctx->tile_cell_filter;
    return PNL_OK;
}

int pnl_make_tiles(pnl_context *ctx, std::vector<int2> &tiles, int cell_begin, int cell_end) {
    const int T = ctx->tile, nbk = ctx->nblocks;
    const int a0 = cell_begin/T, a1 = (cell_end+T-1)/T;
    for (int d = 0; d < nbk; d++)
        for (int a = a0; a < a1 && a+d < nbk; a++) tiles.push_back(make_int2(a, a+d));
    return PNL_OK;
}

extern "C" {

int pnl_block_row_costs(pnl_context *ctx, double *out, int n) {
    if (!ctx || !out) return PNL_ERR_INVALID;
    int rc;
    if ((rc = check_ready(ctx))) return rc;
    if ((rc = finalize(ctx))) return rc;
    if (n != ctx->nblocks) return fail(ctx, PNL_ERR_INVALID, "pnl_block_row_costs: %d blocks expected", ctx->nblocks);
    const int T = ctx->tile, nb = ctx->nblocks;
    const bool p1 = T == 64 && (ctx->dpe == 3 || ctx->dpe == 2), p2 = ctx->dim == 2 && ctx->dpe == 6;
    const bool allow = ctx->use_pure && (p1 || p2) && ctx->qmax >= 2 && !ctx->nonsym && ctx->cls.size() == 1;
    int qlimit = 2;
    if (ctx->dim == 2) for (int q = 3; q <= 4 && ctx->uni_off[q] >= 0 && ctx->uni_np[q] == 6 && q <= ctx->qmax; q++) qlimit = q;
    const pnl_order_formula F = ctx->cls[0]->form[0];
    const double w_uni3 = p2 ? 1.75 : 2.7, w_mixed = p2 ? 2.5 : 4.0, w_cells = p2 ? 30. : 57.;
    host_threads([&](int t, int nthreads) {
        for (int a = t; a < nb; a += nthreads) {
            double c = w_cells;
            for (int b = a; b < nb; b++) {
                const int q = allow ? pnl_tile_uniform_order(ctx, F, a, b, qlimit) : 0;
                c += q == 2 ? 1. : (q ? w_uni3 : w_mixed);
            }
            out[a] = c;
        }
    });
    return PNL_OK;
}

int pnl_set_order_function(pnl_context *ctx, const pnl_order_function *f, const double *cell_smax, const double *facet_smax,
                           double c0, double bc0, double sing_fac, double bsing_fac) {
    if (!ctx || !f || !cell_smax) return fail(ctx, PNL_ERR_INVALID, "bad order-function arguments");
    if (!ctx->have_mesh) return fail(ctx, PNL_ERR_STATE, "upload the mesh first");
    if (f->type < 1 || f->type > 5) return fail(ctx, PNL_ERR_UNSUPPORTED, "order function type %d is not implemented", f->type);
    if (ctx->have_dofs && !(ctx->dpe == ctx->dim+1 || (ctx->dim == 2 && ctx->dpe == 6) || (ctx->dim == 1 && ctx->dpe == 3)))
        return fail(ctx, PNL_ERR_UNSUPPORTED, "pointwise variable orders: P1 and P2 elements");
    if (!pw_set_function(ctx->pw, *f)) return fail(ctx, PNL_ERR_INVALID, "bad Chebyshev series of the scaling");
    ctx->pw.c0 = c0; ctx->pw.bc0 = bc0; ctx->pw.sfac = sing_fac; ctx->pw.bfac = bsing_fac;
    ctx->pw_cell_smax.assign(cell_smax, cell_smax+ctx->nc);
    ctx->pw_facet_smax.clear();
    if (facet_smax && ctx->have_boundary) ctx->pw_facet_smax.assign(facet_smax, facet_smax+ctx->nb);
    for (int w = 0; w < 2; w++) for (int s = 0; s < 3; s++) ctx->have_pw_rules[w][s] = false;
    ctx->pw_vertex_s.clear();
// ... 69 lines not shown
        for (int s = 0; s < ctx->dim; s++)
            if (!ctx->have_pw_rules[1][s]) return fail(ctx, PNL_ERR_STATE, "pointwise boundary rule for %d common vertices not uploaded", s+1);
    }
    std::vector<double> sm(ctx->ncp, 0.);
    std::copy(ctx->pw_cell_smax.begin(), ctx->pw_cell_smax.end(), sm.begin());
    if ((rc = upload(ctx, ctx->b_pw_csm, sm.data(), sm.size()))) return rc;
    if ((rc = upload(ctx, ctx->b_pw_fsm, ctx->pw_facet_smax.data(), ctx->pw_facet_smax.size()))) return rc;
    ctx->pw.cell_smax = (const double*)ctx->b_pw_csm.p; ctx->pw.facet_smax = (const double*)ctx->b_pw_fsm.p;
    DevProblem &P = ctx->P;
    P.qmax = ctx->qmax;
    P.off = (const int*)ctx->b_off.p; P.bary = (const double*)ctx->b_bary.p; P.w = (const double*)ctx->b_w.p;
    P.phi = (const double*)ctx->b_phi.p; P.foff = (const int*)ctx->b_foff.p; P.fbary = (const double*)ctx->b_fbary.p;
    P.fw = (const double*)ctx->b_fw.p;
    P.cur_class = -1;
    return PNL_OK;
}

extern "C" {

int pnl_get_counters(pnl_context *ctx, int64_t *out, int n) {
    if (!ctx || !out || n <= 0) return PNL_ERR_INVALID;
    if (!ctx->b_counters.p) return fail(ctx, PNL_ERR_STATE, "nothing assembled yet");
    unsigned long long tmp[PNL_NCOUNTERS];
    HIPCHK(ctx, hipStreamSynchronize(ctx->stream));
    HIPCHK(ctx, hipMemcpy(tmp, ctx->b_counters.p, sizeof(tmp), hipMemcpyDeviceToHost));
    tmp[0] = ctx->visited_is_assembled ? tmp[1] : ctx->visited_pairs;
    for (int i = 0; i < n && i < PNL_NCOUNTERS; i++) out[i] = (int64_t)tmp[i];
    return check_overflow(ctx);
}

int pnl_get_phase_ms(pnl_context *ctx, float *out, int n) {
    if (!ctx || !out || n <= 0) return PNL_ERR_INVALID;
    if (!ctx->ev_valid) return fail(ctx, PNL_ERR_STATE, "nothing assembled yet");
    HIPCHK(ctx, hipEventSynchronize(ctx->ev[5]));
    float t[7] = {0, 0, 0, 0, 0, 0, 0}, tmp;
    if (ctx->tiles_launched) {
        HIPCHK(ctx, hipEventElapsedTime(&t[0], ctx->ev[0], ctx->ev[6]));
        HIPCHK(ctx, hipEventElapsedTime(&t[1], ctx->ev[6], ctx->ev[1]));
        if (ctx->pure_launched && ctx->cls.size() == 1) {
            HIPCHK(ctx, hipEventElapsedTime(&t[6], ctx->ev[0], ctx->ev[7]));
            t[0] -= t[6];
        }
    }
    HIPCHK(ctx, hipEventElapsedTime(&tmp, ctx->ev[1], ctx->ev[2]));
    HIPCHK(ctx, hipEventElapsedTime(&t[2], ctx->ev[2], ctx->ev[3]));
    HIPCHK(ctx, hipEventElapsedTime(&t[3], ctx->ev[3], ctx->ev[4]));
    HIPCHK(ctx, hipEventElapsedTime(&t[4], ctx->ev[4], ctx->ev[5]));
    t[4] += tmp;
    HIPCHK(ctx, hipEventElapsedTime(&t[5], ctx->ev[0], ctx->ev[5]));
    for (int i = 0; i < n && i < 7; i++) out[i] = t[i];
    return PNL_OK;
}

int pnl_get_kernel_ms(pnl_context *ctx, float *out, int n) {
    if (!ctx || !out || n <= 0) return PNL_ERR_INVALID;
    if (!ctx->ev_valid) return fail(ctx, PNL_ERR_STATE, "nothing assembled yet");
    HIPCHK(ctx, hipEventSynchronize(ctx->ev[5]));
    for (int s = 0; s < n && s < PNL_NUM_KERNEL_SLOTS; s++) {
        out[s] = 0.f;
        if (ctx->kev_set[s]) HIPCHK(ctx, hipEventElapsedTime(&out[s], ctx->kev[s][0], ctx->kev[s][1]));
    }
    return PNL_OK;
}

}
```

pynucleus_amd/csrc/pnl_tile2.h:

```cpp
#pragma once
#include "pnl_common.h"

__host__ __device__ constexpr int uni_rule_size(int dpe, int np) { return 3*np+np+np*dpe+(dpe*(dpe+1)/2)*np; }


#ifndef PNL_FOLD_FLAT
#define PNL_FOLD_FLAT 1
#endif
template <bool NT>
__global__ void __launch_bounds__(256)
k_fold_mirror(const double *__restrict__ A2, const FoldEntry *__restrict__ tab, const int *__restrict__ cpoff, const int2 *__restrict__ cp,
              const long long *__restrict__ cprow, double *__restrict__ A, long long ldA, int N) {
    __shared__ double t1[32][33], t2[32][33];
    __shared__ FoldEntry s_tab[2][PNL_FOLD_TAB+1];
    const unsigned nb = (unsigned)(N+31)/32;
    const unsigned nbs = (nb+7)/8;
    const unsigned sbid = blockIdx.x >> 6, inner = blockIdx.x & 63;
    unsigned I;
    {
        const float t = 2.f*(float)nbs+1.f;
        const float fb = (t-sqrtf(fmaxf(t*t-8.f*(float)sbid, 0.f)))*0.5f;
        I = (unsigned)fmaxf(fb, 0.f);
        if (I >= nbs) I = nbs-1;
        while (I > 0 && I*nbs-I*(I-1)/2 > sbid) I--;
        while (I+1 < nbs && (I+1)*nbs-(I+1)*I/2 <= sbid) I++;
    }
    const unsigned J = I+(sbid-(I*nbs-I*(I-1)/2));
    const unsigned bi = 8*I+(inner >> 3), bj = 8*J+(inner & 7);
    if (bi > bj || bj >= nb) return;
    const int tid = threadIdx.x, tx = tid & 31, ty = tid >> 5;
    if (tid < 2*(PNL_FOLD_TAB+1)) {
        const int side = tid >= PNL_FOLD_TAB+1, k = tid-side*(PNL_FOLD_TAB+1);
        s_tab[side][k] = tab[(size_t)(side ? bj : bi)*(PNL_FOLD_TAB+1)+k];
    }
    for (int k = tid; k < 32*33; k += 256) { (&t1[0][0])[k] = 0.; (&t2[0][0])[k] = 0.; }
    __syncthreads();
    const int n0 = (int)s_tab[0][0].off, n1 = (int)s_tab[1][0].off;
    if (n0 <= PNL_FOLD_TAB && n1 <= PNL_FOLD_TAB) {
#if PNL_FOLD_FLAT
#pragma unroll
        for (int g = 0; g < 2; g++) {
            if (g && bi == bj) break;
            const int nr = g ? n1 : n0, nc = g ? n0 : n1;
            double *__restrict__ tf = g ? &t2[0][0] : &t1[0][0];
            const unsigned total = (unsigned)(nr*nc), inv = ((1u << 20)+(unsigned)nc-1u)/(unsigned)nc;
            for (unsigned base = 0; base < total; base += 8*256) {
                double v[8];
                int dst[8];
#pragma unroll
                for (int u = 0; u < 8; u++) {
                    const unsigned idx = base+256u*u+(unsigned)tid;
                    dst[u] = -1;
                    v[u] = 0.;
                    if (idx < total) {
                        const unsigned ci = (idx*inv) >> 20, cj = idx-ci*(unsigned)nc;
                        const FoldEntry rw = s_tab[g][1+ci], col = s_tab[1-g][1+cj];
                        if ((col.ar >> 5) >= (rw.ar >> 5)) { v[u] = A2[rw.off+col.cy]; dst[u] = (rw.ar & 31)*33+(col.ar & 31); }
                    }
                }
#pragma unroll
                for (int u = 0; u < 8; u++) if (dst[u] >= 0) lds_add_f64(tf+dst[u], v[u]);
            }
        }
#else
#pragma unroll
        for (int g = 0; g < 2; g++) {
            if (g && bi == bj) break;
            const int nr = g ? n1 : n0, nc = g ? n0 : n1;
            double *__restrict__ tf = g ? &t2[0][0] : &t1[0][0];
            for (int cj = tx; cj < nc; cj += 32) {
                const FoldEntry col = s_tab[1-g][1+cj];
                const int cb = col.ar >> 5, c = col.ar & 31;
                for (int ci0 = ty; ci0 < nr; ci0 += 48) {
                    double v[6];
                    int dst[6];
#pragma unroll
                    for (int u = 0; u < 6; u++) {
                        const int ci = ci0+8*u;
                        dst[u] = -1;
                        v[u] = 0.;
                        if (ci < nr) {
// ... 6 lines not shown
                }
            }
        }
#endif
    } else {
        auto gather = [&](int br, int bc, double (*t)[33]) {
            const int J = min(bc*32+tx, N), j0 = cpoff[J], j1 = cpoff[min(J+1, N)];
#pragma unroll 1
            for (int rr = 0; rr < 4; rr++) {
                const int r = ty+8*rr, I = min(br*32+r, N);
                double s = 0.;
                for (int ci = cpoff[I]; ci < cpoff[min(I+1, N)]; ci++) {
                    const int a = cp[ci].x;
                    const double *__restrict__ rowp = A2+cprow[ci];
                    for (int cj = j0; cj < j1; cj++) {
                        const int2 c2 = cp[cj];
                        if (c2.x >= a) s += rowp[c2.y];
                    }
                }
                t[r][tx] = s;
            }
        };
        gather((int)bi, (int)bj, t1);
        if (bi != bj) gather((int)bj, (int)bi, t2);
    }
    __syncthreads();
    for (int r = ty; r < 32; r += 8) {
        const int I = bi*32+r, J = bj*32+tx;
        if (I < N && J < N) {
            const double v = (bi != bj) ? t1[r][tx]+t2[tx][r] : ((r != tx) ? t1[r][tx]+t1[tx][r] : t1[r][tx]);
            if (NT) __builtin_nontemporal_store(v, A+(long long)I*ldA+J); else A[(long long)I*ldA+J] = v;
        }
        const int I2 = bj*32+r, J2 = bi*32+tx;
        if (bi != bj && I2 < N && J2 < N) {
            const double v = t2[r][tx]+t1[tx][r];
            if (NT) __builtin_nontemporal_store(v, A+(long long)I2*ldA+J2); else A[(long long)I2*ldA+J2] = v;
        }
    }
}

__global__ void __launch_bounds__(256)
k_zero_slot_tiles(const SlotOut SO, const int2 *__restrict__ tiles, const int *__restrict__ blk_ndof) {
    const int a = tiles[blockIdx.x].x, b = tiles[blockIdx.x].y;
    const int nA = blk_ndof[a], nBp = SO.colbase[b+1]-SO.colbase[b], W = SO.S-SO.colbase[a];
    double *__restrict__ base = SO.A2+SO.rowoff[a]+(SO.colbase[b]-SO.colbase[a]);
    for (int t = threadIdx.x; t < nA*nBp; t += 256) {
        const int r = t/nBp, c = t-r*nBp;
        base[(long long)r*W+c] = 0.;
    }
}

__host__ __device__ constexpr size_t uniform_fixed_lds(int dpe, int np, int tile, int nUe, bool dof_lists = true) {
    return dpe == 3 ? sizeof(double)*(size_t)(2*tile*(np*2+1)+2*tile+2*tile*(np|1)+(dpe*(dpe+1)/2)*np)
                      +sizeof(int)*(size_t)(2*tile*(dpe|1)+2*tile+(dof_lists ? 4*nUe : 0))
                    : sizeof(double)*(size_t)(tile*np*2+tile*6+2*tile+2*tile*np+(dpe*(dpe+1)/2)*np)
                      +sizeof(int)*(size_t)(2*tile*dpe+2*tile+(dof_lists ? 4*nUe : 0));
}

#ifndef PNL_U33K0_WAVES
#define PNL_U33K0_WAVES 3
#endif
template <int DPE, int NP, int KT, bool STRUCT = false>
__global__ void __launch_bounds__(256, (DPE == 3 && NP == 3) ? (KT == 0 ? PNL_U33K0_WAVES : (KT == 2 ? 4 : 2)) : ((DPE == 3 && NP == 6) ? 3 : 2))
k_tile_uniform(const DevProblem P, const int2 *__restrict__ tiles, const int *__restrict__ tile_cls, const DevKernel *__restrict__ kcls,
               int ntiles, double *__restrict__ A, long long ldA, double *__restrict__ Dglob, int acc_stride, int q_uniform,
               int flags, const double *__restrict__ rule_g, int nUe, const SlotOut SO) {
    const int flags_in = flags;
    constexpr int DIM = 2, NV = 3, NC = 6, ND = DPE*(DPE+1)/2, NT = 256, NW = NT/64;
    constexpr int TILE = DPE == 6 ? 32 : 64, HALVES = 64/TILE, JW = TILE/NW, ITER = JW/HALVES;
    constexpr int R_BARY = 0, R_W = 3*NP, R_WPH = R_W+NP, R_PP = R_WPH+NP*DPE;
    constexpr bool XPTS = DPE == 3;
    constexpr int PS = XPTS ? NP*DIM+1 : NP*DIM, RS = XPTS ? (NP|1) : NP, SS = XPTS ? (DPE|1) : DPE, XS = XPTS ? PS : NC;
    constexpr bool TRAVEL = (TILE == 64);
    const pnl_const_f64_ptr rule = (pnl_const_f64_ptr)(unsigned long long)rule_g;
#ifndef PNL_DEBUG_ABLATE
    flags &= 1;
#endif
    extern __shared__ double smem[];
    double *s_y = smem;
    double *s_x = s_y+TILE*PS;
    double *s_vola = s_x+TILE*XS;
    double *s_volb = s_vola+TILE;
    double *s_Ra = s_volb+TILE;
    double *s_Rb = s_Ra+TILE*RS;
    double *s_PP = s_Rb+TILE*RS;
    int *s_slotb = (int*)(s_PP+ND*NP);
    int *s_sa = s_slotb+TILE*SS;
    int *s_ha = s_sa+TILE*SS;
    int *s_hb = s_ha+TILE;
    int *s_dof = s_hb+TILE;
    const bool dof_lists = SO.A2 == nullptr;
    double *s_acc = (double*)(s_dof+(dof_lists ? 4*nUe : 0));
    const bool have_pow = KT == 0 && (flags_in & 8) != 0;
    double *s_pow = s_acc+(size_t)(nUe+1)*acc_stride;
    const int tid = threadIdx.x, lane = tid & 63, wave = tid >> 6;
    const int li = lane%TILE, half = lane/TILE;
    const int wv = __builtin_amdgcn_readfirstlane(wave);
    unsigned long long npairs = 0;
    const double *cur_ptab = nullptr;

    auto stage = [&](int t, int buf) {
        const int2 tl = tiles[t];
        const int nA = P.blk_ndof[tl.x], nB = P.blk_ndof[tl.y];
        if (tid < 2*TILE) {
            const bool bside = tid < TILE;
            const int l = bside ? tid : tid-TILE, c = (bside ? tl.y : tl.x)*TILE+l;
            double v[NC];
#pragma unroll
            for (int k = 0; k < NC; k++) v[k] = P.cellv[(size_t)k*P.ncp+c];
            const double vol = P.cvol[c];
            int sl[DPE], any = 0;
#pragma unroll
            for (int k = 0; k < DPE; k++) { sl[k] = P.cslot[(size_t)k*P.ncp+c]; any |= (sl[k] >= 0); }
            any |= (P.cvid[c] >= 0) ? 2 : 0;
            double *__restrict__ pts = (bside ? s_y : s_x)+l*PS;
            if (bside || XPTS) {
#pragma unroll
                for (int jp = 0; jp < NP; jp++)
#pragma unroll
                    for (int d = 0; d < DIM; d++) {
                        double sy = 0.;
#pragma unroll
                        for (int k = 0; k < NV; k++) sy = __builtin_fma(rule[R_BARY+3*jp+k], v[k*DIM+d], sy);
                        pts[jp*DIM+d] = sy;
                    }
            } else {
#pragma unroll
                for (int k = 0; k < NC; k++) s_x[l*XS+k] = v[k];
            }
            if (bside) {
                s_volb[l] = vol; s_hb[l] = any;
#pragma unroll
                for (int k = 0; k < DPE; k++) s_slotb[l*SS+k] = sl[k] >= 0 ? sl[k] : nUe;
            } else {
                s_vola[l] = vol; s_ha[l] = any;
#pragma unroll
                for (int k = 0; k < DPE; k++) s_sa[l*SS+k] = (sl[k] >= 0 ? sl[k] : nUe)*acc_stride;
            }
        }
        const int *__restrict__ dofA = P.blk_dofs+(size_t)tl.x*P.blk_stride;
        const int *__restrict__ dofB = P.blk_dofs+(size_t)tl.y*P.blk_stride;
        if (dof_lists) {
            for (int k = tid; k < nA; k += NT) s_dof[(buf*2+0)*nUe+k] = P.rowmap ? P.rowmap[dofA[k]] : dofA[k];
            for (int k = tid; k < nB; k += NT) s_dof[(buf*2+1)*nUe+k] = P.colmap ? P.colmap[dofB[k]] : dofB[k];
        }
        if (have_pow && tile_cls) {
            const double *pt = kcls[(tile_cls[t] & 0xffff) >> 1].ptab;
            if (pt != cur_ptab) { cur_ptab = pt; pnl_pow_tab_fill(s_pow, pt, tid, NT); }
        }
    };

    int tile_idx = blockIdx.x, buf = 0;
    if (tile_idx >= ntiles) return;
    for (int t = tid; t < ND*NP; t += NT) s_PP[t] = rule_g[R_PP+t];
    if (have_pow && !tile_cls) { cur_ptab = P.k.ptab; pnl_pow_tab_fill(s_pow, cur_ptab, tid, NT); }
    for (int t = tid; t < (nUe+1)*acc_stride; t += NT) s_acc[t] = 0.;
    for (int t = tid; t < 2*TILE*RS; t += NT) s_Ra[t] = 0.;
    stage(tile_idx, 0);
    lds_barrier();
#pragma unroll 1
    while (true) {
        const int2 tl = tiles[tile_idx];
        const int ta = tl.x, tb = tl.y;
        const int nA = P.blk_ndof[ta], nB = P.blk_ndof[tb];
        DevKernel kk = P.k;
        if (tile_cls) kk = kcls[(tile_cls[tile_idx] & 0xffff) >> 1];
        const double scale2 = 2.*kern_scale<KT>(kk);
        const double *__restrict__ ptab = (have_pow && kk.ptab) ? s_pow : nullptr;
        double *__restrict__ Ra = s_Ra;
        double xa[NP == 3 ? 3 : 1][DIM];
        double av[XPTS ? 1 : NC];
        if (XPTS && NP == 3) {
#pragma unroll
            for (int ip = 0; ip < (NP == 3 ? 3 : 1); ip++)
#pragma unroll
                for (int d = 0; d < DIM; d++) xa[ip][d] = s_x[li*XS+ip*DIM+d];
        }
        if (!XPTS) {
#pragma unroll
            for (int k = 0; k < NC; k++) av[XPTS ? 0 : k] = s_x[li*XS+k];
        }
        int sa[DPE];
#pragma unroll
        for (int k = 0; k < DPE; k++) sa[k] = s_sa[li*SS+k];
        const int fa = s_ha[li];
        const double vola = s_vola[li];
        kern_dispatch<KT>(kk, ptab, [&](auto ktag) {
        constexpr int KTE = decltype(ktag)::value;
        double racc[NP == 3 ? 3 : 1] = {};
        int j = (wave*JW+half+li) & (TILE-1);
        double y[NP][DIM], volb_j, cacc[TRAVEL ? NP : 1] = {};
        int fb, sbj[DPE];
        auto load_b = [&]() {
#pragma unroll
            for (int jp = 0; jp < NP; jp++)
#pragma unroll
                for (int d = 0; d < DIM; d++) y[jp][d] = s_y[j*PS+jp*DIM+d];
            fb = s_hb[j];
            volb_j = s_volb[j];
#pragma unroll
            for (int b = 0; b < DPE; b++) sbj[b] = s_slotb[j*SS+b];
        };
        if (TRAVEL) load_b();
#pragma unroll 1
        for (int jj = 0; jj < ITER; jj++) {
            if (!TRAVEL) { j = (wave*JW+jj*HALVES+half+li) & (TILE-1); load_b(); }
            else if (jj) {
                constexpr int ROT = 0x134;
                j = __builtin_amdgcn_update_dpp(0, j, ROT, 0xf, 0xf, true);
                fb = __builtin_amdgcn_update_dpp(0, fb, ROT, 0xf, 0xf, true);
// ... 81 lines not shown
                    }
                    const double s0 = (g[0]+g[1])+g[2], s1 = (g[3]+g[4])+g[NP-1];
                    const double A0 = rule[R_WPH+1], B0 = rule[R_WPH]-rule[R_WPH+1];
                    const double A1 = rule[R_WPH+3*DPE+1], B1 = rule[R_WPH+3*DPE]-rule[R_WPH+3*DPE+1];
                    r = __builtin_fma(rule[R_W], s0, rule[R_W+3]*s1);
                    const double base = __builtin_fma(A0, s0, A1*s1);
#pragma unroll
                    for (int b = 0; b < DPE; b++) u[b] = __builtin_fma(B0, g[b], __builtin_fma(B1, g[NP == 6 ? 3+b : 0], base));
                } else {
#pragma unroll
                for (int jp = 0; jp < NP; jp++) {
                    double d2 = 0.;
#pragma unroll
                    for (int d = 0; d < DIM; d++) { const double t = x[d]-y[jp][d]; d2 = __builtin_fma(t, t, d2); }
                    const double g = kern_eval<KTE>(kk, d2, ptab);
                    r = __builtin_fma(rule[R_W+jp], g, r);
                    c[jp] = __builtin_fma(wi, g, c[jp]);
#pragma unroll
                    for (int b = 0; b < DPE; b++) u[b] = __builtin_fma(g, rule[R_WPH+jp*DPE+b], u[b]);
                }
                }
                if (NP == 3) racc[NP == 3 ? ip : 0] = __builtin_fma(vv, r, racc[NP == 3 ? ip : 0]);
                else lds_add_f64(&Ra[li*RS+ip], vv*r);
#pragma unroll
                for (int a = 0; a < DPE; a++) {
                    const double pa = rule[R_WPH+ip*DPE+a];
#pragma unroll
                    for (int b = 0; b < DPE; b++) G[a][b] = __builtin_fma(pa, u[b], G[a][b]);
                }
            }
            if (!(flags & 4)) {
#pragma unroll
                for (int b = 0; b < DPE; b++) {
                    const int sb = sbj[b];
#pragma unroll
                    for (int a = 0; a < DPE; a++) lds_add_f64(&s_acc[sa[a]+sb], -vv*G[a][b]);
                }
            } else if (G[0][0]+G[1][2]+G[DPE-1][DPE-1] == 1.2345e300) s_acc[0] = vv;
#pragma unroll
            for (int jp = 0; jp < NP; jp++) {
                if (TRAVEL) cacc[TRAVEL ? jp : 0] = __builtin_fma(vv, c[jp], cacc[TRAVEL ? jp : 0]);
                else lds_add_f64(&s_Rb[j*RS+jp], vv*c[jp]);
            }
        }
        if (TRAVEL) {
#pragma unroll
            for (int jp = 0; jp < NP; jp++) lds_add_f64(&s_Rb[j*RS+jp], cacc[TRAVEL ? jp : 0]);
        }
        if (NP == 3) {
#pragma unroll
            for (int ip = 0; ip < (NP == 3 ? 3 : 1); ip++) lds_add_f64(&Ra[li*RS+ip], racc[ip]);
        }
        });
        lds_barrier();
        const int nxt = tile_idx+(int)gridDim.x;
        const bool more = nxt < ntiles;
        if (more) stage(nxt, buf^1);
        const int *__restrict__ dA = s_dof+(buf*2+0)*nUe, *__restrict__ dB = s_dof+(buf*2+1)*nUe;
        const bool sym = (flags & 1) != 0 && dof_lists;
        if (SO.A2) {
            const int ca = SO.colbase[ta], W = SO.S-ca;
            double *__restrict__ base = SO.A2+SO.rowoff[ta]+(SO.colbase[tb]-ca);
#pragma unroll 1
            for (int r = wv; r < nA; r += NW) {
                double *__restrict__ row = base+(long long)r*W;
                for (int cc = 2*lane; cc < nB; cc += 128) {
                    double2 v = make_double2(0., 0.);
                    if (cc < nB) { v.x = s_acc[r*acc_stride+cc]; s_acc[r*acc_stride+cc] = 0.; }
                    if (cc+1 < nB) { v.y = s_acc[r*acc_stride+cc+1]; s_acc[r*acc_stride+cc+1] = 0.; }
                    slot_store2(row+cc, v.x, v.y);
                }
            }
        } else if (!(flags & 2))
#pragma unroll 1
        for (int r = wv; r < nA; r += NW) {
            double *__restrict__ row = A+(long long)__builtin_amdgcn_readfirstlane(dA[r])*ldA;
            for (int cc = lane; cc < nB; cc += 64) {
                const double v = s_acc[r*acc_stride+cc];
                if (v != 0.) {
                    if (!sym) s_acc[r*acc_stride+cc] = 0.;
                    atomic_add_f64(&row[dB[cc]], v);
                }
            }
        }
        if (sym) lds_barrier();
        if (sym)
#pragma unroll 1
            for (int cc = wv; cc < nB; cc += NW) {
                double *__restrict__ row = A+(long long)__builtin_amdgcn_readfirstlane(dB[cc])*ldA;
                for (int r = lane; r < nA; r += 64) {
                    const double v = s_acc[r*acc_stride+cc];
                    if (v != 0.) {
                        s_acc[r*acc_stride+cc] = 0.;
                        atomic_add_f64(&row[dA[r]], v);
                    }
                }
            }
        if (flags & 2) for (int t = tid; t < (nUe+1)*acc_stride; t += NT) s_acc[t] = 0.;
        {
            constexpr int PARTS = NT/(2*TILE);
            static_assert(PARTS*2*TILE == NT && 64%PARTS == 0, "one (side, cell) per group of PARTS lanes");
            const int item = tid/PARTS, part = tid-item*PARTS, side = item/TILE, cl = item-side*TILE;
            double *__restrict__ R = (side ? s_Rb : s_Ra)+cl*RS;
            double Rv[NP];
#pragma unroll
            for (int ip = 0; ip < NP; ip++) Rv[ip] = R[ip];
#pragma unroll
            for (int ip = 0; ip < NP; ip++) if (ip%PARTS == part) R[ip] = 0.;
// ... 635 lines not shown
```

pynucleus_amd/csrc/pnl_tile2.hip:

```cpp
#include "pnl_context.h"
#include "pnl_tile2.h"

namespace {

template <int DPE, int NP, int KT, bool STRUCT = false>
int launch_uniform_t(pnl_context *ctx, const DevProblem &Pt, const int2 *tiles, const int *tile_cls, int ntiles, int q, double *A,
                     int64_t ldA, double *Dglob, const SlotOut &SO) {
    constexpr int TILE = DPE == 6 ? 32 : 64;
    const int nUe = (ctx->nU+1) & ~1;
    const size_t fixed = uniform_fixed_lds(DPE, NP, TILE, nUe, SO.A2 == nullptr);
    int acc_stride = nUe+1;
    while (acc_stride % 32 != 1) acc_stride++;
    if (fixed+sizeof(double)*(size_t)(nUe+1)*acc_stride > 80*1024) acc_stride = (nUe+1) | 1;
    size_t lds = fixed+sizeof(double)*(size_t)(nUe+1)*acc_stride;
    if (lds > 160*1024)
        return fail(ctx, PNL_ERR_UNSUPPORTED, "a block of %d cells touches %d DoFs: LDS sub-block of %zu bytes exceeds 160 KiB", TILE, ctx->nU, lds);
    const size_t cap_cu = (size_t)std::max(1, pnl_tune("PNL_UNI_PER_CU") ? atoi(pnl_tune("PNL_UNI_PER_CU")) : 4);
    auto kfun = k_tile_uniform<DPE, NP, KT, STRUCT>;
    HIPCHK(ctx, hipFuncSetAttribute((const void*)kfun, hipFuncAttributeMaxDynamicSharedMemorySize, (int)std::min<size_t>(160*1024, lds+sizeof(double)*PNL_POW_TAB_DOUBLES)));
    auto resident = [&](size_t bytes) -> int {
        int occ = 0;
        if (hipOccupancyMaxActiveBlocksPerMultiprocessor(&occ, (const void*)kfun, 256, bytes) != hipSuccess || occ < 1) {
            (void)hipGetLastError();
            occ = (int)std::min<size_t>(2, (160*1024)/bytes);
        }
        return std::max(1, std::min((int)cap_cu, occ));
    };
    int pow_flag = 0;
    if (KT == 0) {
        const size_t tab = sizeof(double)*PNL_POW_TAB_DOUBLES;
        const int per_cu0 = resident(lds);
        if (lds+tab <= 160*1024 && resident(lds+tab) == per_cu0) { lds += tab; pow_flag = 8; }
        else if (!pnl_tune("PNL_UNI_KEEP_STRIDE")) {
            const int odd = (nUe+1) | 1;
            const size_t alt = fixed+sizeof(double)*(size_t)(nUe+1)*odd+tab;
            if (alt <= 160*1024 && resident(alt) == per_cu0) { acc_stride = odd; lds = alt; pow_flag = 8; }
        }
    }
    HIPCHK(ctx, hipFuncSetAttribute((const void*)kfun, hipFuncAttributeMaxDynamicSharedMemorySize, (int)lds));
    const int per_cu = resident(lds);
    const int grid = pnl_grid_cap(std::min(ntiles, 256*per_cu));
    if (pnl_tune("PNL_VERBOSE"))
        fprintf(stderr, "[pnl] uniform tiles of order %d: %d, dpe=%d np=%d kt=%d struct=%d lds=%zu bytes (%d per CU), acc_stride=%d\n", q, ntiles, DPE,
                NP, KT, (int)STRUCT, lds, per_cu, acc_stride);
    int uni_abl = 0;
#ifdef PNL_DEBUG_ABLATE
    uni_abl = pnl_tune("PNL_UNI_ABL") ? atoi(pnl_tune("PNL_UNI_ABL")) : 0;
#endif
    kt_begin(ctx, PNL_K_TILE_UNIFORM2+(q-2));
    hipLaunchKernelGGL(kfun, dim3(grid), dim3(256), lds, ctx->stream, Pt, tiles, tile_cls, (const DevKernel*)ctx->b_kcls.p, ntiles, A,
                       (long long)ldA, Dglob, acc_stride, q, (ctx->symflush ? 1 : 0) | uni_abl | pow_flag, (const double*)ctx->b_uni.p+ctx->uni_off[q],
                       nUe, SO);
    kt_end(ctx, PNL_K_TILE_UNIFORM2+(q-2));
    HIPCHK(ctx, hipGetLastError());
    return PNL_OK;
}

template <int DPE, int NP>
int launch_uniform_kt(pnl_context *ctx, int kt, const DevProblem &Pt, const int2 *tiles, const int *tile_cls, int ntiles, int q,
                      double *A, int64_t ldA, double *Dglob, const SlotOut &SO) {
    if constexpr (DPE == 3) {
        if (ctx->uni_struct[q] && !pnl_tune("PNL_UNI_GENERIC")) {
            if (kt == 2) return launch_uniform_t<DPE, NP, 2, true>(ctx, Pt, tiles, tile_cls, ntiles, q, A, ldA, Dglob, SO);
            if (kt == 1) return launch_uniform_t<DPE, NP, 1, true>(ctx, Pt, tiles, tile_cls, ntiles, q, A, ldA, Dglob, SO);
            return launch_uniform_t<DPE, NP, 0, true>(ctx, Pt, tiles, tile_cls, ntiles, q, A, ldA, Dglob, SO);
        }
    }
    if (kt == 2) return launch_uniform_t<DPE, NP, 2>(ctx, Pt, tiles, tile_cls, ntiles, q, A, ldA, Dglob, SO);
    if (kt == 1) return launch_uniform_t<DPE, NP, 1>(ctx, Pt, tiles, tile_cls, ntiles, q, A, ldA, Dglob, SO);
    return launch_uniform_t<DPE, NP, 0>(ctx, Pt, tiles, tile_cls, ntiles, q, A, ldA, Dglob, SO);
}

template <int KT>
int launch_p2_t(pnl_context *ctx, const int2 *tiles, const int *tile_cls, int ntiles, double *A, int64_t ldA, int cell_begin,
                int cell_end, unsigned wl_cap_each, const SlotOut &SO) {
    using S = P2Smem;
    const int nUe = (ctx->nU+1) & ~1;
    int stride = nUe+1;
    while (stride % 32 != 1) stride++;
    size_t lds = S::fixed_bytes(nUe)+sizeof(double)*(size_t)(nUe+1)*stride;
    if (lds > 160*1024) { stride = (nUe+1) | 1; lds = S::fixed_bytes(nUe)+sizeof(double)*(size_t)(nUe+1)*stride; }
    if (lds > 160*1024)
        return fail(ctx, PNL_ERR_UNSUPPORTED, "a block of %d cells touches %d DoFs: LDS sub-block of %zu bytes exceeds 160 KiB "
                    "(cells must be numbered with spatial locality)", P2_TILE, ctx->nU, lds);
    auto kfun = k_tile_p2<KT>;
    HIPCHK(ctx, hipFuncSetAttribute((const void*)kfun, hipFuncAttributeMaxDynamicSharedMemorySize, (int)lds));
    const int grid = pnl_grid_cap(std::max(1, std::min((ntiles+1)/2, 256)));
    if (pnl_tune("PNL_VERBOSE")) fprintf(stderr, "[pnl] P2 general tiles=%d nU=%d kt=%d lds=%zu bytes acc_stride=%d\n", ntiles, ctx->nU, KT, lds, stride);
    kt_begin(ctx, PNL_K_TILE_GENERAL);
    hipLaunchKernelGGL(kfun, dim3(grid), dim3(P2_NT), lds, ctx->stream, ctx->P, tiles, tile_cls, (const DevKernel*)ctx->b_kcls.p,
                       (const DevFormula*)ctx->b_fcls.p, A, (long long)ldA, (double*)ctx->b_D.p, cell_begin, cell_end, stride,
                       (int4*)ctx->b_wl.p, (unsigned*)ctx->b_wlcount.p, wl_cap_each, ctx->symflush ? 256 : 0, ntiles,
                       (unsigned*)ctx->b_tilectr.p, nUe, SO);
    kt_end(ctx, PNL_K_TILE_GENERAL);
    HIPCHK(ctx, hipGetLastError());
    return PNL_OK;
}

}

int pnl2_launch_uniform(pnl_context *ctx, int kt, const DevProblem &Pt, const int2 *tiles, const int *tile_cls, int ntiles, int q,
                        double *A, int64_t ldA, double *Dglob, const SlotOut &SO) {
    if (ntiles <= 0) return PNL_OK;
    if (q < 2 || q > 4 || ctx->uni_off[q] < 0) return fail(ctx, PNL_ERR_STATE, "no uniform-tile rule for order %d", q);
    const int np = ctx->uni_np[q];
    if (ctx->dpe == 6 && np == 3) return launch_uniform_kt<6, 3>(ctx, kt, Pt, tiles, tile_cls, ntiles, q, A, ldA, Dglob, SO);
    if (ctx->dpe == 6 && np == 6) return launch_uniform_kt<6, 6>(ctx, kt, Pt, tiles, tile_cls, ntiles, q, A, ldA, Dglob, SO);
    if (ctx->dpe == 3 && np == 6) return launch_uniform_kt<3, 6>(ctx, kt, Pt, tiles, tile_cls, ntiles, q, A, ldA, Dglob, SO);
    if (ctx->dpe == 3 && np == 3) return launch_uniform_kt<3, 3>(ctx, kt, Pt, tiles, tile_cls, ntiles, q, A, ldA, Dglob, SO);
    return fail(ctx, PNL_ERR_UNSUPPORTED, "uniform tiles: dpe=%d with %d points", ctx->dpe, np);
}

int pnl2_launch_p2(pnl_context *ctx, int kt, const int2 *tiles, const int *tile_cls, int ntiles, double *A, int64_t ldA,
                   int cell_begin, int cell_end, unsigned wl_cap_each, const SlotOut &SO) {
    if (ntiles <= 0) return PNL_OK;
    if (kt == 2) return launch_p2_t<2>(ctx, tiles, tile_cls, ntiles, A, ldA, cell_begin, cell_end, wl_cap_each, SO);
    if (kt == 1) return launch_p2_t<1>(ctx, tiles, tile_cls, ntiles, A, ldA, cell_begin, cell_end, wl_cap_each, SO);
    return launch_p2_t<0>(ctx, tiles, tile_cls, ntiles, A, ldA, cell_begin, cell_end, wl_cap_each, SO);
}

int pnl2_zero_slot_tiles(pnl_context *ctx, const SlotOut &SO) {
    if (ctx->n_multitiles <= 0) return PNL_OK;
    hipLaunchKernelGGL(k_zero_slot_tiles, dim3(ctx->n_multitiles), dim3(256), 0, ctx->stream, SO, (const int2*)ctx->b_multitiles.p,
                       (const int*)ctx->b_blk_ndof.p);
    HIPCHK(ctx, hipGetLastError());
    return PNL_OK;
}

int pnl2_fold_mirror(pnl_context *ctx, const SlotOut &SO, double *A, int64_t ldA) {
    const long long nb = (ctx->N+31)/32, nbs = (nb+7)/8;
    if (nbs*(nbs+1)/2*64 >= (1ll << 31)) return fail(ctx, PNL_ERR_UNSUPPORTED, "fold pass: %d DoFs exceed the grid size", ctx->N);
    kt_begin(ctx, PNL_K_FOLD_MIRROR);
    hipLaunchKernelGGL(k_fold_mirror<true>, dim3((unsigned)(nbs*(nbs+1)/2*64)), dim3(256), 0, ctx->stream, (const double*)SO.A2, (const FoldEntry*)ctx->b_foldtab.p, (const int*)ctx->b_cpoff.p,
                       (const int2*)ctx->b_cpslot.p, (const long long*)ctx->b_cprow.p, A, (long long)ldA, ctx->N);
    kt_end(ctx, PNL_K_FOLD_MIRROR);
    HIPCHK(ctx, hipGetLastError());
    return PNL_OK;
}
```

Measured before the change: 55.00 billion element-pairs/s.

## Stage uniform tiles and overlap per-stage mirror folds on side streams

Splits the uniform-tile work into K stages and launches the mirror-fold kernel per stage on an auxiliary stream, limited to the images that stage completed. The worklist pass also moves to its own stream, so folding and worklist processing can overlap with later tile computation instead of running serially at the end. Uniform and general tile kernels now take tiles from an atomic ticket counter instead of a fixed stride, and the uniform grid can leave spare slots per CU for the concurrent streams. This adds event and stream synchronisation complexity, per-stage launch overhead, and risks contention between the overlapped kernels.

```diff
diff --git a/include/pnl_hip.h b/include/pnl_hip.h
--- a/include/pnl_hip.h
+++ b/include/pnl_hip.h
@@ -161,6 +161,8 @@
 
 int pnl_get_counters(pnl_context *ctx, int64_t *out, int n);
 int pnl_get_phase_ms(pnl_context *ctx, float *out, int n);
+int pnl_get_fold_stages(pnl_context *ctx, int64_t *out, int n);
+int pnl_get_fold_plan(pnl_context *ctx, int32_t *images, int64_t nimages, int8_t *tile_stage, int8_t *tile_order, int64_t ntiles);
 enum pnl_kernel_slot { PNL_K_TILE_GENERAL = 0, PNL_K_TILE_UNIFORM2, PNL_K_TILE_UNIFORM3, PNL_K_TILE_UNIFORM4, PNL_K_FOLD_MIRROR,
                        PNL_K_WORKLIST, PNL_NUM_KERNEL_SLOTS };
 int pnl_get_kernel_ms(pnl_context *ctx, float *out, int n);
diff --git a/pynucleus_amd/_lib.py b/pynucleus_amd/_lib.py
--- a/pynucleus_amd/_lib.py
+++ b/pynucleus_amd/_lib.py
@@ -20,7 +20,7 @@
 EXPORTS = ['pnl_create', 'pnl_destroy', 'pnl_error_string', 'pnl_version', 'pnl_set_stream', 'pnl_synchronize',
            'pnl_upload_mesh', 'pnl_upload_dofmap', 'pnl_set_kernel', 'pnl_set_order_formula', 'pnl_upload_distant_rules',
            'pnl_upload_singular_rule', 'pnl_upload_boundary', 'pnl_assemble_dense', 'pnl_dense_overwrites', 'pnl_block_row_costs', 'pnl_tile_cells',
-           'pnl_assemble_dense_tiles', 'pnl_get_counters', 'pnl_get_phase_ms', 'pnl_get_kernel_ms', 'pnl_tree_build', 'pnl_tree_build_blocks', 'pnl_tree_build_refined', 'pnl_tree_build_horizon', 'pnl_tree_build_device', 'pnl_tree_destroy', 'pnl_tree_sizes', 'pnl_tree_get', 'pnl_tree_node_cells', 'pnl_h2_transfer_matrices', 'pnl_nfplan_build', 'pnl_nfplan_destroy', 'pnl_nfplan_sizes', 'pnl_nfplan_get', 'pnl_horizon_pattern', 'pnl_near_pattern', 'pnl_pattern_set_max_nnz', 'pnl_set_option', 'pnl_set_cell_order', 'pnl_set_interaction_transform', 'pnl_set_order_vertex_values', 'pnl_h2_get', 'pnl_h2_set', 'pnl_pattern_nnz', 'pnl_pattern_get', 'pnl_pattern_destroy', 'pnl_set_row_slab', 'pnl_diag_blocks_size', 'pnl_get_diag_blocks', 'pnl_slab_matvec', 'pnl_slab_diagonal', 'pnl_gemv', 'pnl_cg_jacobi',
+           'pnl_assemble_dense_tiles', 'pnl_get_counters', 'pnl_get_phase_ms', 'pnl_get_kernel_ms', 'pnl_get_fold_stages', 'pnl_get_fold_plan', 'pnl_tree_build', 'pnl_tree_build_blocks', 'pnl_tree_build_refined', 'pnl_tree_build_horizon', 'pnl_tree_build_device', 'pnl_tree_destroy', 'pnl_tree_sizes', 'pnl_tree_get', 'pnl_tree_node_cells', 'pnl_h2_transfer_matrices', 'pnl_nfplan_build', 'pnl_nfplan_destroy', 'pnl_nfplan_sizes', 'pnl_nfplan_get', 'pnl_horizon_pattern', 'pnl_near_pattern', 'pnl_pattern_set_max_nnz', 'pnl_set_option', 'pnl_set_cell_order', 'pnl_set_interaction_transform', 'pnl_set_order_vertex_values', 'pnl_h2_get', 'pnl_h2_set', 'pnl_pattern_nnz', 'pnl_pattern_get', 'pnl_pattern_destroy', 'pnl_set_row_slab', 'pnl_diag_blocks_size', 'pnl_get_diag_blocks', 'pnl_slab_matvec', 'pnl_slab_diagonal', 'pnl_gemv', 'pnl_cg_jacobi',
            'pnl_inv_diagonal', 'pnl_set_classes', 'pnl_select_class', 'pnl_upload_sparsity', 'pnl_upload_sparsity_device', 'pnl_assemble_pairs_masked', 'pnl_assemble_boundary_masked', 'pnl_assemble_clusters_tiled', 'pnl_h2_setup', 'pnl_h2_matvec', 'pnl_h2_upward', 'pnl_h2_interact', 'pnl_h2_downward', 'pnl_h2_sizes', 'pnl_spmv',
            'pnl_assemble_pairs_in_horizon', 'pnl_assemble_pairs_in_horizon_range', 'pnl_set_nonsymmetric', 'pnl_set_order_function', 'pnl_upload_pointwise_rules', 'pnl_assemble_dense_pointwise',
            'pnl_assemble_pairs_masked_pointwise', 'pnl_assemble_boundary_masked_pointwise',
@@ -138,6 +138,8 @@
     L.pnl_get_counters.argtypes = [vp, vp, i32]
     L.pnl_get_phase_ms.argtypes = [vp, vp, i32]
     L.pnl_get_kernel_ms.argtypes = [vp, vp, i32]
+    L.pnl_get_fold_stages.argtypes = [vp, vp, i32]
+    L.pnl_get_fold_plan.argtypes = [vp, vp, C.c_int64, vp, vp, C.c_int64]
     L.pnl_set_row_slab.argtypes = [vp, i32, vp, i32, vp]
     L.pnl_tree_build.argtypes = [i32, i32, vp, vp, vp, i32, dbl, i32, i32, i32, C.POINTER(vp)]
     L.pnl_tree_build_blocks.argtypes = [i32, i32, vp, vp, vp, i32, dbl, i32, i32, i32, vp, i32, C.POINTER(vp)]
@@ -551,6 +553,20 @@
         return dict(tile_general=float(out[0]), tile_uniform2=float(out[1]), tile_uniform3=float(out[2]), tile_uniform4=float(out[3]),
                     fold_mirror=float(out[4]), worklist=float(out[5]))
 
+    def fold_stages(self):
+        out = np.zeros((17, 5), dtype=np.int64)
+        n = self.L.pnl_get_fold_stages(self.h, out.ctypes.data, 17)
+        self.check(min(n, 0))
+        return [dict(images=int(r[0]), uniform={2: int(r[1]), 3: int(r[2]), 4: int(r[3])}, mixed=int(r[4])) for r in out[:n]]
+
+    def fold_plan(self, nblocks):
+        nimg = sum(s['images'] for s in self.fold_stages())
+        images = np.zeros((nimg, 3), dtype=np.int32)
+        stage = np.zeros((nblocks, nblocks), dtype=np.int8)
+        order = np.zeros((nblocks, nblocks), dtype=np.int8)
+        self.check(self.L.pnl_get_fold_plan(self.h, images.ctypes.data, nimg, stage.ctypes.data, order.ctypes.data, nblocks*nblocks))
+        return images, stage, order
+
     def gemv(self, A_ptr, ldA, n, x_ptr, y_ptr, symmetric_half=False):
         self.check(self.L.pnl_gemv(self.h, C.c_void_p(A_ptr), int(ldA), int(n), C.c_void_p(x_ptr), C.c_void_p(y_ptr),
                                    int(symmetric_half)))
diff --git a/pynucleus_amd/csrc/pnl_context.h b/pynucleus_amd/csrc/pnl_context.h
--- a/pynucleus_amd/csrc/pnl_context.h
+++ b/pynucleus_amd/csrc/pnl_context.h
@@ -27,6 +27,8 @@
     hipStream_t aux[NAUX] = {};
     hipEvent_t ev_fork = nullptr, ev_join[NAUX] = {};
     hipEvent_t ev_fold = nullptr;
+    static constexpr int MAX_STAGES = 16;
+    hipEvent_t ev_stage[MAX_STAGES+1] = {};
     hipEvent_t ev_bnd = nullptr;
     bool fold_event_set = false;
     std::string err;
@@ -67,6 +69,17 @@
     DevBuf b_kcls, b_fcls, b_uni, b_tilecls, b_ttwphif;
     DevBuf b_scolbase, b_srowoff, b_cpoff, b_cpslot, b_cprow, b_foldtab, b_bkcls, b_bfcls, b_bdefer, b_multitiles, b_slotA, b_candtiles, b_candq;
     int slot_S = 0, n_multitiles = 0;
+    std::vector<int32_t> rng_blk_off, rng_blk;
+    DevBuf b_foldimg, b_unictr;
+    int stg_K = 0, stg_want = -1;
+    std::vector<int> stg_img_off;
+    std::vector<int> stg_uni_off[3];
+    std::vector<unsigned> stg_img;
+    std::vector<signed char> stg_tile_stage;
+    std::vector<unsigned char> stg_tile_q;
+    static constexpr int UNI_CTRS = 64;
+    int uni_ctr_next = 0, uni_ctr_fresh = 0;
+    bool stg_active = false;
     long long slot_total = 0;
     DevBuf b_rowmap, b_rowdof, b_colmap, b_coldof;
     DevBuf b_cholinfo;
@@ -121,8 +134,9 @@
     double xform[4] = {1., 0., 0., 1.};
     std::vector<BlockAgg> blocks;
     hipEvent_t ev[8] = {nullptr, nullptr, nullptr, nullptr, nullptr, nullptr, nullptr, nullptr};
-    hipEvent_t kev[PNL_NUM_KERNEL_SLOTS][2] = {};
-    bool kev_set[PNL_NUM_KERNEL_SLOTS] = {};
+    std::vector<hipEvent_t> kev[PNL_NUM_KERNEL_SLOTS];
+    int kev_n[PNL_NUM_KERNEL_SLOTS] = {};
+    bool kev_open[PNL_NUM_KERNEL_SLOTS] = {};
     bool pure_launched = false;
     bool symflush = false;
     bool ev_valid = false;
@@ -260,8 +274,22 @@
     return Pt;
 }
 
-inline void kt_begin(pnl_context *ctx, int slot) { (void)hipEventRecord(ctx->kev[slot][0], ctx->stream); }
-inline void kt_end(pnl_context *ctx, int slot) { (void)hipEventRecord(ctx->kev[slot][1], ctx->stream); ctx->kev_set[slot] = true; }
+inline void kt_begin(pnl_context *ctx, int slot) {
+    std::vector<hipEvent_t> &v = ctx->kev[slot];
+    const size_t k = 2*(size_t)ctx->kev_n[slot];
+    ctx->kev_open[slot] = false;
+    while (v.size() < k+2) {
+        hipEvent_t e = nullptr;
+        if (hipEventCreate(&e) != hipSuccess) { (void)hipGetLastError(); return; }
+        v.push_back(e);
+    }
+    ctx->kev_open[slot] = hipEventRecord(v[k], ctx->stream) == hipSuccess;
+}
+inline void kt_end(pnl_context *ctx, int slot) {
+    if (!ctx->kev_open[slot]) return;
+    ctx->kev_open[slot] = false;
+    if (hipEventRecord(ctx->kev[slot][2*(size_t)ctx->kev_n[slot]+1], ctx->stream) == hipSuccess) ctx->kev_n[slot]++;
+}
 
 int pnl_tile_order_ready(pnl_context *ctx);
 
@@ -286,11 +314,11 @@
                               const double *x, double *y);
 
 int pnl2_launch_uniform(pnl_context *ctx, int kt, const DevProblem &Pt, const int2 *tiles, const int *tile_cls, int ntiles, int q,
-                        double *A, int64_t ldA, double *Dglob, const SlotOut &SO);
+                        double *A, int64_t ldA, double *Dglob, const SlotOut &SO, int spare = 0);
 int pnl2_launch_p2(pnl_context *ctx, int kt, const int2 *tiles, const int *tile_cls, int ntiles, double *A, int64_t ldA,
                    int cell_begin, int cell_end, unsigned wl_cap_each, const SlotOut &SO);
 int pnl2_zero_slot_tiles(pnl_context *ctx, const SlotOut &SO);
-int pnl2_fold_mirror(pnl_context *ctx, const SlotOut &SO, double *A, int64_t ldA);
+int pnl2_fold_mirror(pnl_context *ctx, const SlotOut &SO, double *A, int64_t ldA, const unsigned *images = nullptr, int nimages = 0);
 inline SlotOut slot_out(const pnl_context *ctx) {
     SlotOut SO;
     SO.A2 = (double*)ctx->b_slotA.p; SO.rowoff = (const long long*)ctx->b_srowoff.p; SO.colbase = (const int*)ctx->b_scolbase.p;
diff --git a/pynucleus_amd/csrc/pnl_hip.hip b/pynucleus_amd/csrc/pnl_hip.hip
--- a/pynucleus_amd/csrc/pnl_hip.hip
+++ b/pynucleus_amd/csrc/pnl_hip.hip
@@ -151,10 +151,100 @@
 }
 
 template <int DIM, int DPE, int TILE, int KT>
+int launch_mixed_tiles(pnl_context *ctx, unsigned *wlc, double *A, int64_t ldA, int cell_begin, int cell_end, const SlotOut &SO) {
+    using S = TileSmem<DIM, DPE, TILE, KT == 0>;
+    const int ntiles = ctx->n_mixed;
+    const int acc_stride = acc_stride_of(ctx->nU, S::fixed_bytes);
+    const size_t lds = S::fixed_bytes+sizeof(double)*(size_t)(ctx->nU+1)*acc_stride;
+    if (lds > 160*1024)
+        return fail(ctx, PNL_ERR_UNSUPPORTED, "a block of %d cells touches %d DoFs: LDS sub-block of %zu bytes exceeds 160 KiB "
+                    "(cells must be numbered with spatial locality)", TILE, ctx->nU, lds);
+    HIPCHK(ctx, hipMemsetAsync(ctx->b_tilectr.p, 0, sizeof(unsigned), ctx->stream));
+    auto kfun = k_tile_distant<DIM, DPE, TILE, KT, false>;
+    const int grid_mult = pnl_tune("PNL_GRID_MULT") ? atoi(pnl_tune("PNL_GRID_MULT")) : 1;
+    const PersistentGrid g = persistent_grid(ctx, kfun, tile_threads(DPE, KT), lds, ntiles, 2, grid_mult);
+    if (g.rc) return g.rc;
+    if (pnl_tune("PNL_VERBOSE")) fprintf(stderr, "[pnl] tiles=%d nU=%d lds=%zu bytes, occupancy API: %d blocks/CU\n", ntiles, ctx->nU, lds, g.per_cu);
+    SlotOut SOk = SO;
+    SOk.nU = ctx->nU;
+    kt_begin(ctx, PNL_K_TILE_GENERAL);
+    if (g.grid > 0)
+        hipLaunchKernelGGL(kfun, dim3(g.grid), dim3(tile_threads(DPE, KT)), lds, ctx->stream, with_mixed_rules(ctx, tile_problem(ctx)), (const int2*)ctx->b_tiles.p+ctx->tile_off, A,
+                           (long long)ldA, (double*)(ctx->have_tile_order ? ctx->b_Dt.p : ctx->b_D.p), cell_begin, cell_end, acc_stride, (int4*)ctx->b_wl.p,
+                           wlc, ctx->wl_cap_each, ctx->ablate | (ctx->symflush ? 256 : 0), ntiles, ClusterTiles{},
+                           (unsigned*)ctx->b_tilectr.p, SOk);
+    kt_end(ctx, PNL_K_TILE_GENERAL);
+    HIPCHK(ctx, hipGetLastError());
+    return PNL_OK;
+}
+
+#ifndef PNL_UNI_SPARE_DEFAULT
+#define PNL_UNI_SPARE_DEFAULT 1
+#endif
+template <int DIM, int DPE, int TILE, int KT>
 int launch_tiles(pnl_context *ctx, int wl_slot, double *A, int64_t ldA, int cell_begin, int cell_end, const SlotOut &SO = SlotOut{}) {
-    using S = TileSmem<DIM, DPE, TILE, KT == 0>;
     HIPCHK(ctx, hipEventRecord(ctx->ev[7], ctx->stream));
     ctx->pure_launched = false;
+    const bool staged = DIM == 2 && DPE == 3 && SO.A2 && ctx->stg_K > 0 && ctx->cls.size() == 1 && !ctx->nonsym;
+    ctx->stg_active = staged;
+    if (staged) {
+        int rc;
+        const int K = ctx->stg_K;
+        const int spare = pnl_tune("PNL_UNI_SPARE") ? atoi(pnl_tune("PNL_UNI_SPARE")) : PNL_UNI_SPARE_DEFAULT;
+        const bool side = !pnl_tune("PNL_NO_OVERLAP");
+        hipStream_t const caller = ctx->stream;
+        hipStream_t const folds = side ? ctx->aux[2] : caller;
+        constexpr int wl_aux = 3;
+        hipStream_t const wls = side ? ctx->aux[wl_aux] : caller;
+        struct StreamGuard { pnl_context *c; hipStream_t s; ~StreamGuard() { c->stream = s; } } stream_guard{ctx, caller};
+        const int2 *tiles = (const int2*)ctx->b_tiles.p+ctx->tile_off;
+        double *Dt = (double*)(ctx->have_tile_order ? ctx->b_Dt.p : ctx->b_D.p);
+        unsigned *wlc = (unsigned*)ctx->b_wlcount.p+wl_slot;
+        auto uniform_stage = [&](int s, int spare_s) -> int {
+            int off = ctx->n_mixed;
+            for (int q = 2; q <= 4; q++) {
+                const std::vector<int> &so = ctx->stg_uni_off[q-2];
+                const int n = so[s+1]-so[s];
+                int rcu = pnl2_launch_uniform(ctx, KT, tile_problem(ctx), tiles+off+so[s], nullptr, n, q, A, ldA, Dt, SO, spare_s);
+                if (rcu) return rcu;
+                ctx->pure_launched = ctx->pure_launched || n > 0;
+                off += so[K+1];
+            }
+            return PNL_OK;
+        };
+        auto fold_stage = [&](int s) -> int {
+            if (side) HIPCHK(ctx, hipStreamWaitEvent(folds, ctx->ev_stage[s], 0));
+            ctx->stream = folds;
+            const int rcf = pnl2_fold_mirror(ctx, SO, A, ldA, (const unsigned*)ctx->b_foldimg.p+ctx->stg_img_off[s], ctx->stg_img_off[s+1]-ctx->stg_img_off[s]);
+            ctx->stream = caller;
+            return rcf;
+        };
+        if ((rc = uniform_stage(0, 0))) return rc;
+        HIPCHK(ctx, hipEventRecord(ctx->ev[7], ctx->stream));
+        if ((rc = launch_mixed_tiles<DIM, DPE, TILE, KT>(ctx, wlc, A, ldA, cell_begin, cell_end, SO))) return rc;
+        HIPCHK(ctx, hipEventRecord(ctx->ev_stage[0], caller));
+        if ((rc = fold_stage(0))) return rc;
+        HIPCHK(ctx, hipEventRecord(ctx->ev_fold, folds));
+        ctx->fold_event_set = true;
+        if (side && wls != folds) HIPCHK(ctx, hipStreamWaitEvent(wls, ctx->ev_fold, 0));
+        ctx->stream = wls;
+        rc = run_worklist<DIM, DPE, KT>(ctx, (const int4*)ctx->b_wl.p, wlc, ctx->wl_cap_each, A, ldA, true);
+        ctx->stream = caller;
+        if (rc) return rc;
+        if (side && wls != folds) HIPCHK(ctx, hipEventRecord(ctx->ev_join[wl_aux], wls));
+        for (int s = 1; s <= K; s++) {
+            if ((rc = uniform_stage(s, spare))) return rc;
+            HIPCHK(ctx, hipEventRecord(ctx->ev_stage[s], caller));
+            if ((rc = fold_stage(s))) return rc;
+        }
+        HIPCHK(ctx, hipEventRecord(ctx->ev[6], caller));
+        if (side) {
+            HIPCHK(ctx, hipEventRecord(ctx->ev_join[2], folds));
+            HIPCHK(ctx, hipStreamWaitEvent(caller, ctx->ev_join[2], 0));
+            if (wls != folds) HIPCHK(ctx, hipStreamWaitEvent(caller, ctx->ev_join[wl_aux], 0));
+        }
+        return PNL_OK;
+    }
     if (TILE == 64 && DPE <= 3) {
         int rc;
         if (DIM == 2 && DPE == 3 && !pnl_tune("PNL_PURE_V1") && ctx->uni_off[2] >= 0 && ctx->uni_np[2] == 3)
@@ -175,29 +265,11 @@
         }
         HIPCHK(ctx, hipEventRecord(ctx->ev[7], ctx->stream));
     }
-    const int ntiles = ctx->n_mixed;
-    const int acc_stride = acc_stride_of(ctx->nU, S::fixed_bytes);
-    const size_t lds = S::fixed_bytes+sizeof(double)*(size_t)(ctx->nU+1)*acc_stride;
-    if (lds > 160*1024)
-        return fail(ctx, PNL_ERR_UNSUPPORTED, "a block of %d cells touches %d DoFs: LDS sub-block of %zu bytes exceeds 160 KiB "
-                    "(cells must be numbered with spatial locality)", TILE, ctx->nU, lds);
     unsigned *wlc = (unsigned*)ctx->b_wlcount.p+wl_slot;
-    HIPCHK(ctx, hipMemsetAsync(ctx->b_tilectr.p, 0, sizeof(unsigned), ctx->stream));
-    auto kfun = k_tile_distant<DIM, DPE, TILE, KT, false>;
-    const int grid_mult = pnl_tune("PNL_GRID_MULT") ? atoi(pnl_tune("PNL_GRID_MULT")) : 1;
-    const PersistentGrid g = persistent_grid(ctx, kfun, tile_threads(DPE, KT), lds, ntiles, 2, grid_mult);
-    if (g.rc) return g.rc;
-    if (pnl_tune("PNL_VERBOSE")) fprintf(stderr, "[pnl] tiles=%d nU=%d lds=%zu bytes, occupancy API: %d blocks/CU\n", ntiles, ctx->nU, lds, g.per_cu);
-    SlotOut SOk = SO;
-    SOk.nU = ctx->nU;
-    kt_begin(ctx, PNL_K_TILE_GENERAL);
-    if (g.grid > 0)
-        hipLaunchKernelGGL(kfun, dim3(g.grid), dim3(tile_threads(DPE, KT)), lds, ctx->stream, with_mixed_rules(ctx, tile_problem(ctx)), (const int2*)ctx->b_tiles.p+ctx->tile_off, A,
-                           (long long)ldA, (double*)(ctx->have_tile_order ? ctx->b_Dt.p : ctx->b_D.p), cell_begin, cell_end, acc_stride, (int4*)ctx->b_wl.p,
-                           wlc, ctx->wl_cap_each, ctx->ablate | (ctx->symflush ? 256 : 0), ntiles, ClusterTiles{},
-                           (unsigned*)ctx->b_tilectr.p, SOk);
-    kt_end(ctx, PNL_K_TILE_GENERAL);
-    HIPCHK(ctx, hipGetLastError());
+    {
+        int rc = launch_mixed_tiles<DIM, DPE, TILE, KT>(ctx, wlc, A, ldA, cell_begin, cell_end, SO);
+        if (rc) return rc;
+    }
     HIPCHK(ctx, hipEventRecord(ctx->ev[6], ctx->stream));
     if (SO.A2) {
         int rc = pnl2_fold_mirror(ctx, SO, A, ldA);
@@ -399,13 +471,19 @@
     int rc;
     const int ncls = (int)ctx->cls.size();
     ctx->symflush = (flags & PNL_FLAG_SYMMETRIC_FLUSH) != 0;
-    for (bool &b : ctx->kev_set) b = false;
+    for (int &k : ctx->kev_n) k = 0;
     HIPCHK(ctx, hipMemsetAsync(ctx->b_counters.p, 0, sizeof(unsigned long long)*PNL_NCOUNTERS, ctx->stream));
     HIPCHK(ctx, hipMemsetAsync(ctx->b_D.p, 0, sizeof(double)*(size_t)ctx->ncp*(DPE*(DPE+1)/2), ctx->stream));
     if (ctx->have_tile_order) HIPCHK(ctx, hipMemsetAsync(ctx->b_Dt.p, 0, sizeof(double)*(size_t)ctx->ncp*(DPE*(DPE+1)/2), ctx->stream));
+    if (DIM == 2 && DPE == 3) {
+        if ((rc = ensure(ctx, ctx->b_unictr, sizeof(unsigned)*pnl_context::UNI_CTRS))) return rc;
+        HIPCHK(ctx, hipMemsetAsync(ctx->b_unictr.p, 0, sizeof(unsigned)*pnl_context::UNI_CTRS, ctx->stream));
+        ctx->uni_ctr_next = 0; ctx->uni_ctr_fresh = pnl_context::UNI_CTRS;
+    }
     HIPCHK(ctx, hipEventRecord(ctx->ev[0], ctx->stream));
     ctx->tiles_launched = ntiles > 0;
     ctx->fold_event_set = false;
+    ctx->stg_active = false;
     const bool bnd_one_pass = zero_exterior && ncls > 1 && ctx->nlab > 0 && !pnl_tune("PNL_BND_PER_CLASS");
     bool bnd_all_fast = true;
     if (bnd_one_pass) {
@@ -528,9 +606,10 @@
         HIPCHK(ctx, hipEventRecord(ctx->ev_join[0], ctx->aux[0]));
         ctx->stream = main_stream;
     } else HIPCHK(ctx, hipEventRecord(ctx->ev[3], ctx->stream));
-    if (bnd_mode == 3 && ctx->fold_event_set) rc = boundary_side(ctx->ev[6]);
-    else if (bnd_mode == 1 || ((bnd_mode == 0 || bnd_mode == 3) && overlap)) rc = boundary_side(bnd_mode == 1 ? ctx->ev_bnd : ctx->ev_fold);
-    else if (bnd_mode == 0 || bnd_mode == 3) rc = boundary_term(chain);
+    if ((bnd_mode == 3 || bnd_mode == 4) && ctx->fold_event_set)
+        rc = boundary_side(bnd_mode == 4 && ctx->stg_active && !pnl_tune("PNL_NO_OVERLAP") ? ctx->ev_stage[0] : ctx->ev[6]);
+    else if (bnd_mode == 1 || ((bnd_mode == 0 || bnd_mode >= 3) && overlap)) rc = boundary_side(bnd_mode == 1 ? ctx->ev_bnd : ctx->ev_fold);
+    else if (bnd_mode == 0 || bnd_mode >= 3) rc = boundary_term(chain);
     if (rc) return rc;
     ctx->cur = 0;
     if (overlap) {
diff --git a/pynucleus_amd/csrc/pnl_setup.hip b/pynucleus_amd/csrc/pnl_setup.hip
--- a/pynucleus_amd/csrc/pnl_setup.hip
+++ b/pynucleus_amd/csrc/pnl_setup.hip
@@ -443,6 +443,18 @@
             }
     }
     if ((rc = upload(ctx, ctx->b_foldtab, tab.data(), tab.size()))) return rc;
+    ctx->rng_blk_off.assign(nranges+1, 0);
+    ctx->rng_blk.clear();
+    std::vector<int> bl;
+    for (int q = 0; q < nranges; q++) {
+        bl.clear();
+        for (int g = cpoff[q*32]; g < cpoff[std::min(ctx->N, q*32+32)]; g++) bl.push_back(cp[g].x);
+        std::sort(bl.begin(), bl.end());
+        bl.erase(std::unique(bl.begin(), bl.end()), bl.end());
+        ctx->rng_blk.insert(ctx->rng_blk.end(), bl.begin(), bl.end());
+        ctx->rng_blk_off[q+1] = (int)ctx->rng_blk.size();
+    }
+    ctx->stg_want = -1;
     return PNL_OK;
 }
 
@@ -608,7 +620,8 @@
 std::deque<std::string> g_option_values;
 const char *const k_product_options[] = {"PNL_WL_FRAC", "PNL_FH_NOTILES", "PNL_NO_POWTAB", "PNL_VERBOSE", "PNL_PLAN_TIMING", "PNL_PLAN_THREADS", "PNL_BND_OLD",
                                          "PNL_NO_OVERLAP", "PNL_NO_FORK",
-                                         "PNL_TILE_WGS", "PNL_UNI_GENERIC", "PNL_MIXED_GENERIC"};
+                                         "PNL_TILE_WGS", "PNL_UNI_GENERIC", "PNL_MIXED_GENERIC",
+                                         "PNL_FOLD_STAGES", "PNL_UNI_SPARE", "PNL_BND_MODE"};
 }
 
 const char *pnl_tune(const char *name) {
@@ -673,9 +686,8 @@
         if (hipEventCreateWithFlags(&e, hipEventDisableTiming) != hipSuccess) { delete ctx; return PNL_ERR_HIP; }
     for (auto &e : ctx->ev)
         if (hipEventCreate(&e) != hipSuccess) { delete ctx; return PNL_ERR_HIP; }
-    for (auto &pr : ctx->kev)
-        for (auto &e : pr)
-            if (hipEventCreate(&e) != hipSuccess) { delete ctx; return PNL_ERR_HIP; }
+    for (auto &e : ctx->ev_stage)
+        if (hipEventCreateWithFlags(&e, hipEventDisableTiming) != hipSuccess) { delete ctx; return PNL_ERR_HIP; }
     std::memset(&ctx->P, 0, sizeof(ctx->P));
 #ifdef PNL_DEBUG_ABLATE
     if (const char *e = pnl_tune("PNL_ABLATE")) ctx->ablate = atoi(e);
@@ -693,9 +705,10 @@
     (void)hipStreamSynchronize(ctx->stream);
     for (auto &e : ctx->ev)
         if (e) (void)hipEventDestroy(e);
-    for (auto &pr : ctx->kev)
-        for (auto &e : pr)
+    for (auto &v : ctx->kev)
+        for (auto &e : v)
             if (e) (void)hipEventDestroy(e);
+    for (auto &e : ctx->ev_stage) if (e) (void)hipEventDestroy(e);
     tile_order_drop(ctx);
     for (auto &st : ctx->aux) if (st) { (void)hipStreamSynchronize(st); (void)hipStreamDestroy(st); }
     if (ctx->ev_fork) (void)hipEventDestroy(ctx->ev_fork);
@@ -1043,11 +1056,13 @@
     std::vector<std::vector<int2>> mixed, uni[3];
 };
 
+static int fold_stages_wanted();
+
 static bool tiles_resident(const pnl_context *ctx, const std::vector<int2> &tiles, const TilePlan &R) {
     const std::vector<pnl_order_formula> &forms = R.forms;
     return tiles.size() == ctx->tiles_cached.size() && ctx->b_tiles.p && ctx->tiles_cb == R.cell_begin && ctx->tiles_ce == R.cell_end &&
         forms.size() == ctx->tiles_forms.size() && std::memcmp(forms.data(), ctx->tiles_forms.data(), sizeof(pnl_order_formula)*R.ncls) == 0 &&
-        ctx->tiles_filter == ctx->tile_cell_filter &&
+        ctx->tiles_filter == ctx->tile_cell_filter && ctx->stg_want == fold_stages_wanted() &&
         (tiles.empty() || std::memcmp(tiles.data(), ctx->tiles_cached.data(), tiles.size()*sizeof(int2)) == 0);
 }
 
@@ -1096,6 +1111,127 @@
         qof[cand_idx[c]] = (signed char)q; moved++;
     }
     if (pnl_tune("PNL_VERBOSE")) fprintf(stderr, "[pnl] exact order range: %zu of %zu open tiles are uniform\n", moved, cand.size());
+    return PNL_OK;
+}
+
+#ifndef PNL_FOLD_STAGES_DEFAULT
+#define PNL_FOLD_STAGES_DEFAULT 0
+#endif
+static int fold_stages_wanted() {
+    const char *e = pnl_tune("PNL_FOLD_STAGES");
+    return std::max(0, std::min(e ? atoi(e) : PNL_FOLD_STAGES_DEFAULT, (int)pnl_context::MAX_STAGES));
+}
+
+static void stage_plan_drop(pnl_context *ctx) {
+    ctx->stg_K = 0;
+    ctx->stg_img_off.clear(); ctx->stg_img.clear(); ctx->stg_tile_stage.clear(); ctx->stg_tile_q.clear();
+    for (auto &v : ctx->stg_uni_off) v.clear();
+}
+
+static int stage_plan(pnl_context *ctx, TilePlan &R, const std::vector<int2> &tiles, int K) {
+    stage_plan_drop(ctx);
+    const int nb = ctx->nblocks, nr = (ctx->N+31)/32;
+    const size_t nuni = R.ncls == 1 ? R.uni[0][0].size()+R.uni[1][0].size()+R.uni[2][0].size() : 0;
+    if (K <= 0 || !(R.p1 && ctx->dim == 2 && ctx->dpe == 3 && R.ncls == 1 && !ctx->nonsym) || nuni == 0 || nr > 65535 ||
+        (int)ctx->rng_blk_off.size() != nr+1 || tiles.size() != (size_t)nb*(nb+1)/2) return PNL_OK;
+    std::vector<signed char> &tst = ctx->stg_tile_stage;
+    std::vector<unsigned char> &tq = ctx->stg_tile_q;
+    tst.assign((size_t)nb*nb, (signed char)-1);
+    tq.assign((size_t)nb*nb, 0);
+    size_t seen = 0;
+    for (const int2 &t : tiles)
+        if (t.x >= 0 && t.x <= t.y && t.y < nb && tst[(size_t)t.x*nb+t.y] < 0) { tst[(size_t)t.x*nb+t.y] = 0; seen++; }
+    if (seen != tiles.size()) { stage_plan_drop(ctx); return PNL_OK; }
+    for (int u = 0; u < 3; u++)
+        for (const int2 &t : R.uni[u][0]) { tst[(size_t)t.x*nb+t.y] = 1; tq[(size_t)t.x*nb+t.y] = (unsigned char)(2+u); }
+    const int32_t *boff = ctx->rng_blk_off.data(), *blk = ctx->rng_blk.data();
+    auto img_index = [nr](int bi, int bj) { return (size_t)bi*nr-(size_t)bi*(bi-1)/2+(size_t)(bj-bi); };
+    const size_t nimg = (size_t)nr*(nr+1)/2;
+    std::vector<signed char> ist(nimg, 1);
+    auto over_tiles = [&](int bi, int bj, auto &&f) {
+        for (int x = boff[bi]; x < boff[bi+1]; x++)
+            for (int y = boff[bj]; y < boff[bj+1]; y++) {
+                const int a = std::min(blk[x], blk[y]), b = std::max(blk[x], blk[y]);
+                f((size_t)a*nb+b);
+            }
+    };
+    host_threads([&](int th, int nthr) {
+        for (int bi = th; bi < nr; bi += nthr)
+            for (int bj = bi; bj < nr; bj++) {
+                bool plain = true;
+                over_tiles(bi, bj, [&](size_t t) { plain = plain && tq[t] != 0; });
+                if (!plain) ist[img_index(bi, bj)] = 0;
+            }
+    });
+    for (int bi = 0; bi < nr; bi++)
+        for (int bj = bi; bj < nr; bj++)
+            if (ist[img_index(bi, bj)] == 0) over_tiles(bi, bj, [&](size_t t) { tst[t] = 0; });
+    std::vector<long long> row_n(nb, 0);
+    long long far = 0;
+    for (int a = 0; a < nb; a++) {
+        for (int b = a; b < nb; b++) row_n[a] += tst[(size_t)a*nb+b] == 1;
+        far += row_n[a];
+    }
+    if (far == 0) { stage_plan_drop(ctx); return PNL_OK; }
+    K = (int)std::min<long long>(K, far);
+    long long before = 0;
+    for (int a = 0; a < nb; a++) {
+        const int band = (int)std::min<long long>(K-1, before*K/far);
+        for (int b = a; b < nb; b++) if (tst[(size_t)a*nb+b] == 1) tst[(size_t)a*nb+b] = (signed char)(1+band);
+        before += row_n[a];
+    }
+    host_threads([&](int th, int nthr) {
+        for (int bi = th; bi < nr; bi += nthr)
+            for (int bj = bi; bj < nr; bj++) {
+                signed char &s = ist[img_index(bi, bj)];
+                if (s == 0) continue;
+                int m = 0;
+                over_tiles(bi, bj, [&](size_t t) { m = std::max(m, (int)tst[t]); });
+                s = (signed char)m;
+            }
+    });
+#ifdef PNL_DEBUG_ABLATE
+    for (int bi = 0; bi < nr; bi++)
+        for (int bj = bi; bj < nr; bj++) {
+            const int s = ist[img_index(bi, bj)];
+            over_tiles(bi, bj, [&](size_t t) {
+                if (tst[t] < 0 || tst[t] > s || (s >= 1 && tq[t] == 0)) { fprintf(stderr, "[pnl] stage plan: image (%d, %d) of stage %d against tile stage %d\n", bi, bj, s, (int)tst[t]); abort(); }
+            });
+        }
+#endif
+    std::vector<int> &ioff = ctx->stg_img_off;
+    ioff.assign(K+2, 0);
+    for (size_t i = 0; i < nimg; i++) ioff[ist[i]+1]++;
+    for (int s = 0; s <= K; s++) ioff[s+1] += ioff[s];
+    std::vector<int> fill(ioff.begin(), ioff.end()-1);
+    ctx->stg_img.assign(nimg, 0u);
+    const int nbs = (nr+7)/8;
+    for (int I = 0; I < nbs; I++)
+        for (int J = I; J < nbs; J++)
+            for (int inner = 0; inner < 64; inner++) {
+                const int bi = 8*I+(inner >> 3), bj = 8*J+(inner & 7);
+                if (bi > bj || bj >= nr) continue;
+                ctx->stg_img[fill[ist[img_index(bi, bj)]]++] = ((unsigned)bi << 16) | (unsigned)bj;
+            }
+    for (int u = 0; u < 3; u++) {
+        std::vector<int2> &list = R.uni[u][0];
+        std::vector<int> &off = ctx->stg_uni_off[u];
+        off.assign(K+2, 0);
+        for (const int2 &t : list) off[tst[(size_t)t.x*nb+t.y]+1]++;
+        for (int s = 0; s <= K; s++) off[s+1] += off[s];
+        std::vector<int> at(off.begin(), off.end()-1);
+        std::vector<int2> sorted(list.size());
+        for (const int2 &t : list) sorted[at[tst[(size_t)t.x*nb+t.y]]++] = t;
+        list.swap(sorted);
+    }
+    int rc;
+    if ((rc = upload(ctx, ctx->b_foldimg, ctx->stg_img.data(), ctx->stg_img.size()))) return rc;
+    ctx->stg_K = K;
+    if (pnl_tune("PNL_VERBOSE"))
+        for (int s = 0; s <= K; s++)
+            fprintf(stderr, "[pnl] fold stage %d: %d images, uniform tiles of order 2/3/4: %d / %d / %d\n", s, ioff[s+1]-ioff[s],
+                    ctx->stg_uni_off[0][s+1]-ctx->stg_uni_off[0][s], ctx->stg_uni_off[1][s+1]-ctx->stg_uni_off[1][s],
+                    ctx->stg_uni_off[2][s+1]-ctx->stg_uni_off[2][s]);
     return PNL_OK;
 }
 
@@ -1206,6 +1342,8 @@
     }
     std::vector<int2> all;
     ctx->single_launch = R.p2;
+    const int stages_wanted = fold_stages_wanted();
+    if ((rc = stage_plan(ctx, R, tiles, stages_wanted))) return rc;
     if (!R.p2) tile_lists_per_class(ctx, R, all);
     else if ((rc = tile_lists_single_launch(ctx, R, tiles, all))) return rc;
     if (pnl_tune("PNL_VERBOSE")) {
@@ -1217,6 +1355,7 @@
     ctx->tile_off = 0; ctx->n_mixed = ctx->cls_n_mixed[0]; ctx->n_pure = ctx->cls_n_pure[0];
     ctx->tiles_cached = tiles; ctx->tiles_cb = cell_begin; ctx->tiles_ce = cell_end; ctx->tiles_forms = R.forms;
     ctx->tiles_filter = ctx->tile_cell_filter;
+    ctx->stg_want = stages_wanted;
     return PNL_OK;
 }
 
@@ -1392,15 +1531,60 @@
     return PNL_OK;
 }
 
+int pnl_get_fold_stages(pnl_context *ctx, int64_t *out, int n) {
+    if (!ctx || n < 0 || (n && !out)) return PNL_ERR_INVALID;
+    if (!ctx->b_tiles.p || ctx->cls_n_mixed.empty()) return fail(ctx, PNL_ERR_STATE, "no tile plan yet");
+    const int K = ctx->stg_K;
+    for (int s = 0; s <= K && s < n; s++) {
+        int64_t *o = out+5*(size_t)s;
+        if (K == 0) {
+            const long long nr = (ctx->N+31)/32;
+            o[0] = nr*(nr+1)/2;
+            for (int u = 0; u < 3; u++) { o[1+u] = 0; for (int k : ctx->cls_n_uni[u]) o[1+u] += k; }
+        } else {
+            o[0] = ctx->stg_img_off[s+1]-ctx->stg_img_off[s];
+            for (int u = 0; u < 3; u++) o[1+u] = ctx->stg_uni_off[u][s+1]-ctx->stg_uni_off[u][s];
+        }
+        o[4] = 0;
+        if (s == 0) for (int k : ctx->cls_n_mixed) o[4] += k;
+    }
+    return K+1;
+}
+
+int pnl_get_fold_plan(pnl_context *ctx, int32_t *images, int64_t nimages, int8_t *tile_stage, int8_t *tile_order, int64_t ntiles) {
+    if (!ctx) return PNL_ERR_INVALID;
+    if (ctx->stg_K <= 0) return fail(ctx, PNL_ERR_STATE, "the resident tile plan has no fold stages");
+    const int K = ctx->stg_K;
+    const size_t nb2 = (size_t)ctx->nblocks*ctx->nblocks;
+    if (images) {
+        if (nimages != ctx->stg_img_off[K+1]) return fail(ctx, PNL_ERR_INVALID, "the plan has %d images", ctx->stg_img_off[K+1]);
+        for (int s = 0; s <= K; s++)
+            for (int i = ctx->stg_img_off[s]; i < ctx->stg_img_off[s+1]; i++) {
+                images[3*(size_t)i] = (int32_t)(ctx->stg_img[i] >> 16); images[3*(size_t)i+1] = (int32_t)(ctx->stg_img[i] & 0xffffu);
+                images[3*(size_t)i+2] = s;
+            }
+    }
+    if (tile_stage || tile_order) {
+        if ((size_t)ntiles != nb2) return fail(ctx, PNL_ERR_INVALID, "the tile tables have %zu entries", nb2);
+        if (tile_stage) std::memcpy(tile_stage, ctx->stg_tile_stage.data(), nb2);
+        if (tile_order) std::memcpy(tile_order, ctx->stg_tile_q.data(), nb2);
+    }
+    return PNL_OK;
+}
+
 int pnl_get_kernel_ms(pnl_context *ctx, float *out, int n) {
     if (!ctx || !out || n <= 0) return PNL_ERR_INVALID;
     if (!ctx->ev_valid) return fail(ctx, PNL_ERR_STATE, "nothing assembled yet");
     HIPCHK(ctx, hipEventSynchronize(ctx->ev[5]));
     for (int s = 0; s < n && s < PNL_NUM_KERNEL_SLOTS; s++) {
         out[s] = 0.f;
-        if (ctx->kev_set[s]) HIPCHK(ctx, hipEventElapsedTime(&out[s], ctx->kev[s][0], ctx->kev[s][1]));
-    }
-    return PNL_OK;
-}
-
-}
+        for (int k = 0; k < ctx->kev_n[s]; k++) {
+            float t = 0.f;
+            HIPCHK(ctx, hipEventElapsedTime(&t, ctx->kev[s][2*k], ctx->kev[s][2*k+1]));
+            out[s] += t;
+        }
+    }
+    return PNL_OK;
+}
+
+}
diff --git a/pynucleus_amd/csrc/pnl_tile2.h b/pynucleus_amd/csrc/pnl_tile2.h
--- a/pynucleus_amd/csrc/pnl_tile2.h
+++ b/pynucleus_amd/csrc/pnl_tile2.h
@@ -10,23 +10,29 @@
 template <bool NT>
 __global__ void __launch_bounds__(256)
 k_fold_mirror(const double *__restrict__ A2, const FoldEntry *__restrict__ tab, const int *__restrict__ cpoff, const int2 *__restrict__ cp,
-              const long long *__restrict__ cprow, double *__restrict__ A, long long ldA, int N) {
+              const long long *__restrict__ cprow, double *__restrict__ A, long long ldA, int N, const unsigned *__restrict__ images) {
     __shared__ double t1[32][33], t2[32][33];
     __shared__ FoldEntry s_tab[2][PNL_FOLD_TAB+1];
     const unsigned nb = (unsigned)(N+31)/32;
-    const unsigned nbs = (nb+7)/8;
-    const unsigned sbid = blockIdx.x >> 6, inner = blockIdx.x & 63;
-    unsigned I;
-    {
-        const float t = 2.f*(float)nbs+1.f;
-        const float fb = (t-sqrtf(fmaxf(t*t-8.f*(float)sbid, 0.f)))*0.5f;
-        I = (unsigned)fmaxf(fb, 0.f);
-        if (I >= nbs) I = nbs-1;
-        while (I > 0 && I*nbs-I*(I-1)/2 > sbid) I--;
-        while (I+1 < nbs && (I+1)*nbs-(I+1)*I/2 <= sbid) I++;
-    }
-    const unsigned J = I+(sbid-(I*nbs-I*(I-1)/2));
-    const unsigned bi = 8*I+(inner >> 3), bj = 8*J+(inner & 7);
+    unsigned bi, bj;
+    if (images) {
+        const unsigned im = images[blockIdx.x];
+        bi = im >> 16; bj = im & 0xffffu;
+    } else {
+        const unsigned nbs = (nb+7)/8;
+        const unsigned sbid = blockIdx.x >> 6, inner = blockIdx.x & 63;
+        unsigned I;
+        {
+            const float t = 2.f*(float)nbs+1.f;
+            const float fb = (t-sqrtf(fmaxf(t*t-8.f*(float)sbid, 0.f)))*0.5f;
+            I = (unsigned)fmaxf(fb, 0.f);
+            if (I >= nbs) I = nbs-1;
+            while (I > 0 && I*nbs-I*(I-1)/2 > sbid) I--;
+            while (I+1 < nbs && (I+1)*nbs-(I+1)*I/2 <= sbid) I++;
+        }
+        const unsigned J = I+(sbid-(I*nbs-I*(I-1)/2));
+        bi = 8*I+(inner >> 3); bj = 8*J+(inner & 7);
+    }
     if (bi > bj || bj >= nb) return;
     const int tid = threadIdx.x, tx = tid & 31, ty = tid >> 5;
     if (tid < 2*(PNL_FOLD_TAB+1)) {
@@ -139,7 +145,7 @@
 
 __host__ __device__ constexpr size_t uniform_fixed_lds(int dpe, int np, int tile, int nUe, bool dof_lists = true) {
     return dpe == 3 ? sizeof(double)*(size_t)(2*tile*(np*2+1)+2*tile+2*tile*(np|1)+(dpe*(dpe+1)/2)*np)
-                      +sizeof(int)*(size_t)(2*tile*(dpe|1)+2*tile+(dof_lists ? 4*nUe : 0))
+                      +sizeof(int)*(size_t)(2*tile*(dpe|1)+2*tile+2+(dof_lists ? 4*nUe : 0))
                     : sizeof(double)*(size_t)(tile*np*2+tile*6+2*tile+2*tile*np+(dpe*(dpe+1)/2)*np)
                       +sizeof(int)*(size_t)(2*tile*dpe+2*tile+(dof_lists ? 4*nUe : 0));
 }
@@ -151,7 +157,7 @@
 __global__ void __launch_bounds__(256, (DPE == 3 && NP == 3) ? (KT == 0 ? PNL_U33K0_WAVES : (KT == 2 ? 4 : 2)) : ((DPE == 3 && NP == 6) ? 3 : 2))
 k_tile_uniform(const DevProblem P, const int2 *__restrict__ tiles, const int *__restrict__ tile_cls, const DevKernel *__restrict__ kcls,
                int ntiles, double *__restrict__ A, long long ldA, double *__restrict__ Dglob, int acc_stride, int q_uniform,
-               int flags, const double *__restrict__ rule_g, int nUe, const SlotOut SO) {
+               int flags, const double *__restrict__ rule_g, int nUe, const SlotOut SO, unsigned *__restrict__ tile_ctr) {
     const int flags_in = flags;
     constexpr int DIM = 2, NV = 3, NC = 6, ND = DPE*(DPE+1)/2, NT = 256, NW = NT/64;
     constexpr int TILE = DPE == 6 ? 32 : 64, HALVES = 64/TILE, JW = TILE/NW, ITER = JW/HALVES;
@@ -175,7 +181,8 @@
     int *s_sa = s_slotb+TILE*SS;
     int *s_ha = s_sa+TILE*SS;
     int *s_hb = s_ha+TILE;
-    int *s_dof = s_hb+TILE;
+    int *s_next = s_hb+TILE;
+    int *s_dof = s_next+(DPE == 3 ? 2 : 0);
     const bool dof_lists = SO.A2 == nullptr;
     double *s_acc = (double*)(s_dof+(dof_lists ? 4*nUe : 0));
     const bool have_pow = KT == 0 && (flags_in & 8) != 0;
@@ -243,6 +250,9 @@
     if (have_pow && !tile_cls) { cur_ptab = P.k.ptab; pnl_pow_tab_fill(s_pow, cur_ptab, tid, NT); }
     for (int t = tid; t < (nUe+1)*acc_stride; t += NT) s_acc[t] = 0.;
     for (int t = tid; t < 2*TILE*RS; t += NT) s_Ra[t] = 0.;
+    constexpr bool TICKET = DPE == 3;
+    unsigned pending = 0;
+    if (TICKET && tid == 0) pending = atomicAdd(tile_ctr, 1u);
     stage(tile_idx, 0);
     lds_barrier();
 #pragma unroll 1
@@ -430,8 +440,12 @@
             for (int ip = 0; ip < (NP == 3 ? 3 : 1); ip++) lds_add_f64(&Ra[li*RS+ip], racc[ip]);
         }
         });
+        if (TICKET && tid == 0) {
+            s_next[0] = (int)min(gridDim.x+pending, (unsigned)ntiles);
+            if (gridDim.x+pending < (unsigned)ntiles) pending = atomicAdd(tile_ctr, 1u);
+        }
         lds_barrier();
-        const int nxt = tile_idx+(int)gridDim.x;
+        const int nxt = TICKET ? __builtin_amdgcn_readfirstlane(s_next[0]) : tile_idx+(int)gridDim.x;
         const bool more = nxt < ntiles;
         if (more) stage(nxt, buf^1);
         const int *__restrict__ dA = s_dof+(buf*2+0)*nUe, *__restrict__ dB = s_dof+(buf*2+1)*nUe;
diff --git a/pynucleus_amd/csrc/pnl_tile2.hip b/pynucleus_amd/csrc/pnl_tile2.hip
--- a/pynucleus_amd/csrc/pnl_tile2.hip
+++ b/pynucleus_amd/csrc/pnl_tile2.hip
@@ -5,7 +5,7 @@
 
 template <int DPE, int NP, int KT, bool STRUCT = false>
 int launch_uniform_t(pnl_context *ctx, const DevProblem &Pt, const int2 *tiles, const int *tile_cls, int ntiles, int q, double *A,
-                     int64_t ldA, double *Dglob, const SlotOut &SO) {
+                     int64_t ldA, double *Dglob, const SlotOut &SO, int spare) {
     constexpr int TILE = DPE == 6 ? 32 : 64;
     const int nUe = (ctx->nU+1) & ~1;
     const size_t fixed = uniform_fixed_lds(DPE, NP, TILE, nUe, SO.A2 == nullptr);
@@ -39,7 +39,17 @@
     }
     HIPCHK(ctx, hipFuncSetAttribute((const void*)kfun, hipFuncAttributeMaxDynamicSharedMemorySize, (int)lds));
     const int per_cu = resident(lds);
-    const int grid = pnl_grid_cap(std::min(ntiles, 256*per_cu));
+    const int grid = pnl_grid_cap(std::min(ntiles, 256*std::max(1, per_cu-(DPE == 3 ? std::max(spare, 0) : 0))));
+    unsigned *ctr = nullptr;
+    if (DPE == 3) {
+        constexpr int NCTR = pnl_context::UNI_CTRS;
+        int rc = ensure(ctx, ctx->b_unictr, sizeof(unsigned)*NCTR);
+        if (rc) return rc;
+        ctr = (unsigned*)ctx->b_unictr.p+ctx->uni_ctr_next;
+        ctx->uni_ctr_next = (ctx->uni_ctr_next+1)%NCTR;
+        if (ctx->uni_ctr_fresh > 0) ctx->uni_ctr_fresh--;
+        else HIPCHK(ctx, hipMemsetAsync(ctr, 0, sizeof(unsigned), ctx->stream));
+    }
     if (pnl_tune("PNL_VERBOSE"))
         fprintf(stderr, "[pnl] uniform tiles of order %d: %d, dpe=%d np=%d kt=%d struct=%d lds=%zu bytes (%d per CU), acc_stride=%d\n", q, ntiles, DPE,
                 NP, KT, (int)STRUCT, lds, per_cu, acc_stride);
@@ -50,7 +60,7 @@
     kt_begin(ctx, PNL_K_TILE_UNIFORM2+(q-2));
     hipLaunchKernelGGL(kfun, dim3(grid), dim3(256), lds, ctx->stream, Pt, tiles, tile_cls, (const DevKernel*)ctx->b_kcls.p, ntiles, A,
                        (long long)ldA, Dglob, acc_stride, q, (ctx->symflush ? 1 : 0) | uni_abl | pow_flag, (const double*)ctx->b_uni.p+ctx->uni_off[q],
-                       nUe, SO);
+                       nUe, SO, ctr);
     kt_end(ctx, PNL_K_TILE_UNIFORM2+(q-2));
     HIPCHK(ctx, hipGetLastError());
     return PNL_OK;
@@ -58,17 +68,17 @@
 
 template <int DPE, int NP>
 int launch_uniform_kt(pnl_context *ctx, int kt, const DevProblem &Pt, const int2 *tiles, const int *tile_cls, int ntiles, int q,
-                      double *A, int64_t ldA, double *Dglob, const SlotOut &SO) {
+                      double *A, int64_t ldA, double *Dglob, const SlotOut &SO, int spare) {
     if constexpr (DPE == 3) {
         if (ctx->uni_struct[q] && !pnl_tune("PNL_UNI_GENERIC")) {
-            if (kt == 2) return launch_uniform_t<DPE, NP, 2, true>(ctx, Pt, tiles, tile_cls, ntiles, q, A, ldA, Dglob, SO);
-            if (kt == 1) return launch_uniform_t<DPE, NP, 1, true>(ctx, Pt, tiles, tile_cls, ntiles, q, A, ldA, Dglob, SO);
-            return launch_uniform_t<DPE, NP, 0, true>(ctx, Pt, tiles, tile_cls, ntiles, q, A, ldA, Dglob, SO);
+            if (kt == 2) return launch_uniform_t<DPE, NP, 2, true>(ctx, Pt, tiles, tile_cls, ntiles, q, A, ldA, Dglob, SO, spare);
+            if (kt == 1) return launch_uniform_t<DPE, NP, 1, true>(ctx, Pt, tiles, tile_cls, ntiles, q, A, ldA, Dglob, SO, spare);
+            return launch_uniform_t<DPE, NP, 0, true>(ctx, Pt, tiles, tile_cls, ntiles, q, A, ldA, Dglob, SO, spare);
         }
     }
-    if (kt == 2) return launch_uniform_t<DPE, NP, 2>(ctx, Pt, tiles, tile_cls, ntiles, q, A, ldA, Dglob, SO);
-    if (kt == 1) return launch_uniform_t<DPE, NP, 1>(ctx, Pt, tiles, tile_cls, ntiles, q, A, ldA, Dglob, SO);
-    return launch_uniform_t<DPE, NP, 0>(ctx, Pt, tiles, tile_cls, ntiles, q, A, ldA, Dglob, SO);
+    if (kt == 2) return launch_uniform_t<DPE, NP, 2>(ctx, Pt, tiles, tile_cls, ntiles, q, A, ldA, Dglob, SO, spare);
+    if (kt == 1) return launch_uniform_t<DPE, NP, 1>(ctx, Pt, tiles, tile_cls, ntiles, q, A, ldA, Dglob, SO, spare);
+    return launch_uniform_t<DPE, NP, 0>(ctx, Pt, tiles, tile_cls, ntiles, q, A, ldA, Dglob, SO, spare);
 }
 
 template <int KT>
@@ -100,14 +110,14 @@
 }
 
 int pnl2_launch_uniform(pnl_context *ctx, int kt, const DevProblem &Pt, const int2 *tiles, const int *tile_cls, int ntiles, int q,
-                        double *A, int64_t ldA, double *Dglob, const SlotOut &SO) {
+                        double *A, int64_t ldA, double *Dglob, const SlotOut &SO, int spare) {
     if (ntiles <= 0) return PNL_OK;
     if (q < 2 || q > 4 || ctx->uni_off[q] < 0) return fail(ctx, PNL_ERR_STATE, "no uniform-tile rule for order %d", q);
     const int np = ctx->uni_np[q];
-    if (ctx->dpe == 6 && np == 3) return launch_uniform_kt<6, 3>(ctx, kt, Pt, tiles, tile_cls, ntiles, q, A, ldA, Dglob, SO);
-    if (ctx->dpe == 6 && np == 6) return launch_uniform_kt<6, 6>(ctx, kt, Pt, tiles, tile_cls, ntiles, q, A, ldA, Dglob, SO);
-    if (ctx->dpe == 3 && np == 6) return launch_uniform_kt<3, 6>(ctx, kt, Pt, tiles, tile_cls, ntiles, q, A, ldA, Dglob, SO);
-    if (ctx->dpe == 3 && np == 3) return launch_uniform_kt<3, 3>(ctx, kt, Pt, tiles, tile_cls, ntiles, q, A, ldA, Dglob, SO);
+    if (ctx->dpe == 6 && np == 3) return launch_uniform_kt<6, 3>(ctx, kt, Pt, tiles, tile_cls, ntiles, q, A, ldA, Dglob, SO, spare);
+    if (ctx->dpe == 6 && np == 6) return launch_uniform_kt<6, 6>(ctx, kt, Pt, tiles, tile_cls, ntiles, q, A, ldA, Dglob, SO, spare);
+    if (ctx->dpe == 3 && np == 6) return launch_uniform_kt<3, 6>(ctx, kt, Pt, tiles, tile_cls, ntiles, q, A, ldA, Dglob, SO, spare);
+    if (ctx->dpe == 3 && np == 3) return launch_uniform_kt<3, 3>(ctx, kt, Pt, tiles, tile_cls, ntiles, q, A, ldA, Dglob, SO, spare);
     return fail(ctx, PNL_ERR_UNSUPPORTED, "uniform tiles: dpe=%d with %d points", ctx->dpe, np);
 }
 
@@ -127,12 +137,14 @@
     return PNL_OK;
 }
 
-int pnl2_fold_mirror(pnl_context *ctx, const SlotOut &SO, double *A, int64_t ldA) {
+int pnl2_fold_mirror(pnl_context *ctx, const SlotOut &SO, double *A, int64_t ldA, const unsigned *images, int nimages) {
     const long long nb = (ctx->N+31)/32, nbs = (nb+7)/8;
     if (nbs*(nbs+1)/2*64 >= (1ll << 31)) return fail(ctx, PNL_ERR_UNSUPPORTED, "fold pass: %d DoFs exceed the grid size", ctx->N);
+    if (images && nimages <= 0) return PNL_OK;
+    const unsigned grid = images ? (unsigned)nimages : (unsigned)(nbs*(nbs+1)/2*64);
     kt_begin(ctx, PNL_K_FOLD_MIRROR);
-    hipLaunchKernelGGL(k_fold_mirror<true>, dim3((unsigned)(nbs*(nbs+1)/2*64)), dim3(256), 0, ctx->stream, (const double*)SO.A2, (const FoldEntry*)ctx->b_foldtab.p, (const int*)ctx->b_cpoff.p,
-                       (const int2*)ctx->b_cpslot.p, (const long long*)ctx->b_cprow.p, A, (long long)ldA, ctx->N);
+    hipLaunchKernelGGL(k_fold_mirror<true>, dim3(grid), dim3(256), 0, ctx->stream, (const double*)SO.A2, (const FoldEntry*)ctx->b_foldtab.p, (const int*)ctx->b_cpoff.p,
+                       (const int2*)ctx->b_cpslot.p, (const long long*)ctx->b_cprow.p, A, (long long)ldA, ctx->N, images);
     kt_end(ctx, PNL_K_FOLD_MIRROR);
     HIPCHK(ctx, hipGetLastError());
     return PNL_OK;
```

Measured after the change: 59.41 billion element-pairs/s, median of 6. 1.08x the previous value.
